# ashawkey/torch-ngp

Hardware: AMD Instinct MI355X
Metric: training samples/s (rays x steps), lego-shaped synthetic, fp16 autocast, full step incl. Adam (higher is better)
Workload: dtype f16

## Files before the change

### include/ngp_hip.h

```cpp
#ifndef NGP_HIP_H
#define NGP_HIP_H

#include <stddef.h>
#include <stdint.h>

#ifdef __cplusplus
extern "C" {
#endif

typedef void* ngp_stream_t;

enum {
    NGP_OK = 0,
    NGP_ERR_INVALID = 1,
    NGP_ERR_LAUNCH = 2,
    NGP_ERR_DEVICE = 3
};

enum { NGP_F32 = 0, NGP_F16 = 1, NGP_F64 = 2 };

#define NGP_MAX_LEVELS 32

const char* ngp_last_error(void);
int ngp_abi_version(void);
// ... 91 lines not shown
                                          const double* rgbs, const double* deltas, const int32_t* rays, const double* weights_sum,
                                          const double* image, uint32_t M, uint32_t N, float T_thresh, double* grad_sigmas,
                                          double* grad_rgbs, ngp_stream_t stream);
int ngp_composite_rays_f64(uint32_t n_alive, uint32_t n_step, float T_thresh, int32_t* rays_alive, double* rays_t,
                           const double* sigmas, const double* rgbs, const double* deltas, double* weights_sum, double* depth,
                           double* image, ngp_stream_t stream);

size_t ngp_compact_rays_workspace_bytes(uint32_t n_alive);
int ngp_compact_rays(const int32_t* rays_alive, uint32_t n_alive, int32_t* out_alive, int32_t* out_count,
                     void* workspace, ngp_stream_t stream);


int ngp_ffmlp_forward(const void* inputs, const void* weights, uint32_t B, uint32_t input_dim, uint32_t output_dim,
                      uint32_t hidden_dim, uint32_t num_layers, uint32_t activation, uint32_t output_activation,
                      void* forward_buffer, void* outputs, ngp_stream_t stream);
int ngp_ffmlp_inference(const void* inputs, const void* weights, uint32_t B, uint32_t input_dim,
                        uint32_t output_dim, uint32_t hidden_dim, uint32_t num_layers, uint32_t activation,
                        uint32_t output_activation, void* inference_buffer, void* outputs, ngp_stream_t stream);
int ngp_ffmlp_backward(const void* grad, const void* inputs, const void* weights, const void* forward_buffer,
                       uint32_t B, uint32_t input_dim, uint32_t output_dim, uint32_t hidden_dim, uint32_t num_layers,
                       uint32_t activation, uint32_t output_activation, int calc_grad_inputs, void* backward_buffer,
                       void* grad_inputs, void* grad_weights, ngp_stream_t stream);
int ngp_allocate_splitk(size_t size);
int ngp_free_splitk(void);

int ngp_grid_encode_forward_ex(const float* inputs, const void* embeddings, const int32_t* offsets, void* outputs,
                               uint32_t B, uint32_t D, uint32_t C, uint32_t L, float S, uint32_t H, void* dy_dx,
                               uint32_t gridtype, int align_corners, uint32_t interp, int dtype, float bound,
                               ngp_stream_t stream);
int ngp_grid_encode_backward_ex(const void* grad, const float* inputs, const void* embeddings, const int32_t* offsets,
                                void* grad_embeddings, uint32_t B, uint32_t D, uint32_t C, uint32_t L, float S,
                                uint32_t H, const void* dy_dx, void* grad_inputs, uint32_t gridtype, int align_corners,
                                uint32_t interp, int dtype, float bound, ngp_stream_t stream);
int ngp_grid_encode_forward_sched(const float* inputs, const void* embeddings, const int32_t* offsets, void* outputs,
                                  uint32_t B, uint32_t D, uint32_t C, uint32_t L, float S, uint32_t H, void* dy_dx,
                                  uint32_t gridtype, int align_corners, uint32_t interp, int dtype, float bound,
                                  const float* level_cost_host, ngp_stream_t stream);

int ngp_grid_encode_forward_sel(const float* inputs, const void* embeddings, const void* embeddings_alt, const float* parity,
                                const uint32_t* rows_dev, const int32_t* offsets, void* outputs, uint32_t B, uint32_t D, uint32_t C, uint32_t L,
                                float S, uint32_t H, uint32_t gridtype, int align_corners, uint32_t interp, int dtype, float bound,
                                const float* level_cost_host, ngp_stream_t stream);

uint32_t ngp_grid_forward_work_lists(uint32_t L, uint32_t tiles, const float* level_cost_host, uint16_t* level_out, uint32_t* tile0_out,
                                     uint32_t* end_out);

size_t ngp_grid_backward_workspace_bytes(const int32_t* offsets_host, uint32_t B, uint32_t D, uint32_t C, uint32_t L, float S, uint32_t H,
                                         uint32_t gridtype, int align_corners, int dtype);
int ngp_grid_encode_backward_checked(const void* grad, const float* inputs, const void* embeddings, const int32_t* offsets,
                                     void* grad_embeddings, uint32_t B, uint32_t D, uint32_t C, uint32_t L, float S, uint32_t H,
                                     const void* dy_dx, void* grad_inputs, uint32_t gridtype, int align_corners, uint32_t interp,
                                     int dtype, float bound, const int32_t* offsets_host, void* workspace, size_t workspace_bytes,
                                     float* found_inf, ngp_stream_t stream);

typedef struct ngp_table_adam {
    float* param[2]; float* exp_avg[2]; float* exp_avg_sq[2]; void* param_fp16[2];
    const float* state;
    float lr, beta1, beta2, eps;
} ngp_table_adam_t;
uint32_t ngp_grid_table_adam_prefix(const int32_t* offsets_host, uint32_t B, uint32_t D, uint32_t C, uint32_t L, float S, uint32_t H,
                                    uint32_t gridtype, int align_corners, int dtype);
typedef struct ngp_slab_sets {
    const void* slabs_a; uint32_t n_slabs_a, n_params_a; void* grad_weights_a;
    const void* slabs_b; uint32_t n_slabs_b, n_params_b; void* grad_weights_b;
    const float* ray_err; uint32_t n_rays; float* loss;
    uint32_t overwrite_table;
    const ngp_table_adam_t* table_adam;
} ngp_slab_sets_t;
int ngp_grid_encode_backward_checked_slabs(const void* grad, const float* inputs, const void* embeddings, const int32_t* offsets,
                                           void* grad_embeddings, uint32_t B, uint32_t D, uint32_t C, uint32_t L, float S, uint32_t H,
                                           const void* dy_dx, void* grad_inputs, uint32_t gridtype, int align_corners, uint32_t interp,
                                           int dtype, float bound, const int32_t* offsets_host, void* workspace, size_t workspace_bytes,
                                           float* found_inf, const ngp_slab_sets_t* slab_sets, ngp_stream_t stream);
int ngp_grid_encode_backward_ws(const void* grad, const float* inputs, const void* embeddings, const int32_t* offsets,
                                void* grad_embeddings, uint32_t B, uint32_t D, uint32_t C, uint32_t L, float S, uint32_t H,
                                const void* dy_dx, void* grad_inputs, uint32_t gridtype, int align_corners, uint32_t interp,
                                int dtype, float bound, const int32_t* offsets_host, void* workspace, size_t workspace_bytes,
                                ngp_stream_t stream);

size_t ngp_density_grid_update_workspace_bytes(uint32_t n_cells);
int ngp_density_grid_update(const float* sigmas, const int64_t* cells, uint32_t n, float density_scale, float decay, float* density_grid,
                            uint32_t n_cells, float* scratch, float density_thresh, float* mean_out, uint8_t* bitfield, void* workspace,
                            ngp_stream_t stream);

#define NGP_FF_INPUT_PLANAR 1u
#define NGP_FF_DX_PLANAR 2u
#define NGP_FF_LAYERED 4u
#define NGP_FF_SINGLE_WAVE 8u
#define NGP_FF_DEFER_REDUCE 16u
#define NGP_FF_RECOMPUTE 32u
#define NGP_FF_SERIAL_FLUSH 64u
int ngp_ffmlp_forward_ex(const void* inputs, const void* weights, uint32_t B, uint32_t input_dim, uint32_t output_dim,
                         uint32_t hidden_dim, uint32_t num_layers, uint32_t activation, uint32_t output_activation,
                         void* forward_buffer, void* outputs, uint32_t flags, ngp_stream_t stream);
int ngp_ffmlp_inference_ex(const void* inputs, const void* weights, uint32_t B, uint32_t input_dim,
                           uint32_t output_dim, uint32_t hidden_dim, uint32_t num_layers, uint32_t activation,
                           uint32_t output_activation, void* inference_buffer, void* outputs, uint32_t flags,
                           ngp_stream_t stream);
int ngp_ffmlp_backward_ex(const void* grad, const void* inputs, const void* weights, const void* forward_buffer,
                          uint32_t B, uint32_t input_dim, uint32_t output_dim, uint32_t hidden_dim, uint32_t num_layers,
                          uint32_t activation, uint32_t output_activation, int calc_grad_inputs, void* backward_buffer,
                          void* grad_inputs, void* grad_weights, uint32_t flags, ngp_stream_t stream);

size_t ngp_ffmlp_backward_workspace_bytes(uint32_t B, uint32_t input_dim, uint32_t hidden_dim, uint32_t num_layers);
int ngp_ffmlp_backward_ws(const void* grad, const void* inputs, const void* weights, const void* forward_buffer, uint32_t B,
                          uint32_t input_dim, uint32_t output_dim, uint32_t hidden_dim, uint32_t num_layers, uint32_t activation,
                          uint32_t output_activation, int calc_grad_inputs, void* backward_buffer, void* grad_inputs, void* grad_weights,
                          uint32_t flags, void* workspace, size_t workspace_bytes, ngp_stream_t stream);

size_t ngp_ffmlp_backward_backward_workspace_bytes(uint32_t B, uint32_t input_dim, uint32_t hidden_dim, uint32_t num_layers,
                                                   uint32_t activation);
int ngp_ffmlp_backward_backward(const void* grad, const void* inputs, const void* weights, const void* forward_buffer, const void* u,
                                uint32_t B, uint32_t input_dim, uint32_t output_dim, uint32_t hidden_dim, uint32_t num_layers,
                                uint32_t activation, void* grad_grad, void* grad_weights2, void* grad_inputs2, void* workspace,
                                size_t workspace_bytes, ngp_stream_t stream);

int ngp_network_forward(const void* enc, const float* dirs, uint32_t M, uint32_t M_valid, const void* w_sigma, const void* w_color,
                        uint32_t num_layers_sigma, uint32_t num_layers_color, float density_scale, int training,
                        void* forward_buffer_sigma, void* h16, float* sigma, void* color_in, void* forward_buffer_color, float* rgb,
                        uint32_t flags, ngp_stream_t stream);

int ngp_network_forward_rows(const void* enc, const float* dirs, uint32_t M, uint32_t M_valid, const void* w_sigma, const void* w_color,
                             uint32_t num_layers_sigma, uint32_t num_layers_color, float density_scale, int training,
                             void* forward_buffer_sigma, void* h16, float* sigma, void* color_in, void* forward_buffer_color, float* rgb,
                             uint32_t flags, const uint32_t* rows_dev, ngp_stream_t stream);

int ngp_network_backward_color(const void* grad_out16, const void* color_in, const void* w_color, const void* forward_buffer_color, uint32_t M,
                               uint32_t num_layers_color, void* backward_buffer, const float* grad_sigma, const void* h16,
                               float density_scale, void* grad_h16, void* grad_w_color, uint32_t flags, ngp_stream_t stream);
uint32_t ngp_ffmlp_backward_slab_count(uint32_t B, uint32_t input_dim, uint32_t hidden_dim, uint32_t num_layers);
int ngp_ffmlp_reduce_slabs_pair(const void* slabs_a, uint32_t n_slabs_a, uint32_t n_params_a, void* grad_weights_a, const void* slabs_b,
                                uint32_t n_slabs_b, uint32_t n_params_b, void* grad_weights_b, float* found_inf, ngp_stream_t stream);

int ngp_training_row_bound(const uint32_t* rows_dev);

int ngp_pipeline_mid_forward(const void* h16, const float* dirs, float* sigma, void* color_in, uint32_t M, uint32_t M_valid,
                             float density_scale, ngp_stream_t stream);
int ngp_pipeline_rgb_forward(const void* out16, float* rgb, uint32_t M, ngp_stream_t stream);
int ngp_pipeline_rgb_backward(const float* grad_rgb, const float* rgb, void* grad_out16, uint32_t M, ngp_stream_t stream);
int ngp_pipeline_mid_backward(const float* grad_sigma, const void* h16, const void* grad_color_in, void* grad_h16, uint32_t M,
                              float density_scale, ngp_stream_t stream);

int ngp_pipeline_mse_loss(const float* image, const float* target, uint32_t n, const float* loss_scale, float* loss,
                          float* grad_image, ngp_stream_t stream);

#define NGP_LINEAR_STACK_MAX 8
uint32_t ngp_linear_stack_flat_size(uint32_t depth, uint32_t n_in, uint32_t hidden, uint32_t n_out, int identity);
int ngp_linear_stack_pack(const float* const* weights, uint32_t depth, uint32_t n_in, uint32_t hidden, uint32_t n_out, int identity,
                          void* flat_fp16, ngp_stream_t stream);
int ngp_linear_stack_unpack_grad(const void* grad_flat_fp16, uint32_t depth, uint32_t n_in, uint32_t hidden, uint32_t n_out, int identity,
                                 float* const* grads, ngp_stream_t stream);

int ngp_pad_2d_fp16(const void* src, uint32_t src_rows, uint32_t src_cols, uint32_t src_row_stride, void* dst, uint32_t dst_rows,
                    uint32_t dst_cols, ngp_stream_t stream);

int ngp_rays_from_pixels(const float* poses, uint32_t B, float fx, float fy, float cx, float cy, uint32_t W, const int64_t* inds,
                         uint32_t inds_batch_stride, uint32_t N, float* rays_o, float* rays_d, ngp_stream_t stream);

#define NGP_MARCH_RESET_COUNTER 1u
#define NGP_MARCH_ZERO_TAIL 2u
#define NGP_MARCH_SCAN_LAUNCH 8u
#define NGP_MARCH_NOISE_FROM_SEED 4u
int ngp_march_rays_train_ex(const float* rays_o, const float* rays_d, const uint8_t* grid, float bound, float dt_gamma,
                            uint32_t max_steps, uint32_t N, uint32_t C, uint32_t H, uint32_t M, const float* nears,
                            const float* fars, float* xyzs, float* dirs, float* deltas, int32_t* rays, int32_t* counter,
                            const float* noises, void* workspace, uint32_t flags, ngp_stream_t stream);
int ngp_march_rays_train_aabb(const float* rays_o, const float* rays_d, const uint8_t* grid, float bound, float dt_gamma,
                              uint32_t max_steps, uint32_t N, uint32_t C, uint32_t H, uint32_t M, const float* aabb, float min_near,
                              float* nears, float* fars, float* xyzs, float* dirs, float* deltas, int32_t* rays, int32_t* counter,
                              const float* noises, void* workspace, uint32_t flags, ngp_stream_t stream);

int ngp_march_rays_ex(uint32_t n_alive, uint32_t n_step, const int32_t* rays_alive, const float* rays_t, const float* rays_o,
                      const float* rays_d, float bound, float dt_gamma, uint32_t max_steps, uint32_t C, uint32_t H,
                      const uint8_t* grid, const float* nears, const float* fars, float* xyzs, float* dirs, float* deltas,
                      const float* noises, uint32_t zero_rows, ngp_stream_t stream);

int ngp_march_rays_dev(const int32_t* state, uint32_t alive_bound, uint32_t n_total, uint32_t n_step_cap, const int32_t* rays_alive, const float* rays_t,
                       const float* rays_o, const float* rays_d, float bound, float dt_gamma, uint32_t max_steps, uint32_t C, uint32_t H,
                       const uint8_t* grid, const float* nears, const float* fars, float* xyzs, float* dirs, float* deltas,
                       const float* noises, uint32_t rows, ngp_stream_t stream);
int ngp_march_rays_dev_rows(const int32_t* state, uint32_t alive_bound, uint32_t n_total, uint32_t n_step_cap, const int32_t* rays_alive, const float* rays_t,
// ... 176 lines not shown
```

### torch-ngp_amd/_ngp_capi.py

```python
import ctypes
import os

import torch

_HERE = os.path.dirname(os.path.abspath(__file__))
LIB_PATH = os.environ.get('NGP_HIP_LIBRARY') or os.path.join(_HERE, 'libngp_hip.so')

NGP_F32, NGP_F16, NGP_F64 = 0, 1, 2
NGP_FF_INPUT_PLANAR, NGP_FF_DX_PLANAR, NGP_FF_LAYERED, NGP_FF_SINGLE_WAVE, NGP_FF_DEFER_REDUCE, NGP_FF_RECOMPUTE = 1, 2, 4, 8, 16, 32
NGP_FF_SERIAL_FLUSH = 64
NGP_MARCH_RESET_COUNTER, NGP_MARCH_ZERO_TAIL, NGP_MARCH_NOISE_FROM_SEED, NGP_MARCH_SCAN_LAUNCH = 1, 2, 4, 8
NGP_OPT_PHASE_CHECK, NGP_OPT_PHASE_UPDATE, NGP_OPT_PHASE_COMMIT, NGP_OPT_PHASE_FLIP = 1, 2, 4, 8
ABI_VERSION = 11

if not os.path.exists(LIB_PATH):
    raise ImportError(
        f"{LIB_PATH} is missing: build the HIP extension first (python __graft_entry__.py, or "
        f"make -C {os.path.join(_HERE, 'csrc')}).  There is no CPU fallback for these operators.")

lib = ctypes.CDLL(LIB_PATH)

_vp, _u32, _f32, _i32, _sz = ctypes.c_void_p, ctypes.c_uint32, ctypes.c_float, ctypes.c_int, ctypes.c_size_t

_SIGNATURES = {
    'ngp_grid_encode_forward': [_vp, _vp, _vp, _vp, _u32, _u32, _u32, _u32, _f32, _u32, _vp, _u32, _i32, _u32, _i32, _vp],
    'ngp_grid_encode_backward': [_vp, _vp, _vp, _vp, _vp, _u32, _u32, _u32, _u32, _f32, _u32, _vp, _vp, _u32, _i32, _u32, _i32, _vp],
    'ngp_grad_total_variation': [_vp, _vp, _vp, _vp, _f32, _u32, _u32, _u32, _u32, _f32, _u32, _u32, _i32, _i32, _vp],
    'ngp_grid_corner_indices': [_vp, _vp, _vp, _u32, _u32, _u32, _f32, _u32, _u32, _i32, _vp],
    'ngp_grid_level_table': [_u32, _f32, _u32, _vp, _vp],
    'ngp_grid_encode_backward_backward': [_vp, _vp, _vp, _vp, _vp, _vp, _vp, _vp, _u32, _u32, _u32, _u32, _f32, _u32, _u32, _i32, _u32, _i32, _vp,
                                          _sz, _vp],
    'ngp_grid_encode_backward_ordered': [_vp, _vp, _vp, _vp, _vp, _u32, _u32, _u32, _u32, _f32, _u32, _vp, _vp, _u32, _i32, _u32, _i32, _f32, _vp,
                                         _sz, _vp],
    'ngp_grid_encode_backward_backward_ordered': [_vp, _vp, _vp, _vp, _vp, _vp, _vp, _vp, _u32, _u32, _u32, _u32, _f32, _u32, _u32, _i32, _u32, _i32,
                                                  _vp, _sz, _vp],
    'ngp_grid_backward_is_reproducible': [_vp, _u32, _u32, _u32, _u32, _f32, _u32, _u32, _i32, _i32],
    'ngp_sh_encode_forward': [_vp, _vp, _u32, _u32, _u32, _vp, _i32, _vp],
    'ngp_sh_encode_backward': [_vp, _vp, _u32, _u32, _u32, _vp, _vp, _i32, _vp],
    'ngp_freq_encode_forward': [_vp, _u32, _u32, _u32, _u32, _vp, _vp],
    'ngp_freq_encode_backward': [_vp, _vp, _u32, _u32, _u32, _u32, _vp, _vp],
    'ngp_freq_encode_forward_f64': [_vp, _u32, _u32, _u32, _u32, _vp, _vp],
    'ngp_freq_encode_backward_f64': [_vp, _vp, _u32, _u32, _u32, _u32, _vp, _vp],
    'ngp_freq_encode_backward_backward': [_vp, _vp, _vp, _u32, _u32, _u32, _u32, _vp, _vp, _i32, _vp],
    'ngp_sh_encode_backward_backward': [_vp, _vp, _vp, _vp, _u32, _u32, _u32, _vp, _vp, _i32, _vp],
    'ngp_near_far_from_aabb': [_vp, _vp, _vp, _u32, _f32, _vp, _vp, _vp],
    'ngp_sph_from_ray': [_vp, _vp, _f32, _u32, _vp, _vp],
    'ngp_morton3D': [_vp, _u32, _vp, _vp],
    'ngp_morton3D_invert': [_vp, _u32, _vp, _vp],
    'ngp_packbits': [_vp, _u32, _f32, _vp, _vp],
    'ngp_packbits_ex': [_vp, _u32, _f32, _vp, _vp, _vp],
    'ngp_march_rays_train': [_vp, _vp, _vp, _f32, _f32, _u32, _u32, _u32, _u32, _u32, _vp, _vp, _vp, _vp, _vp, _vp, _vp, _vp, _vp, _vp],
    'ngp_composite_rays_train_forward': [_vp, _vp, _vp, _vp, _u32, _u32, _f32, _vp, _vp, _vp, _vp],
    'ngp_composite_rays_train_backward': [_vp, _vp, _vp, _vp, _vp, _vp, _vp, _vp, _u32, _u32, _f32, _vp, _vp, _vp],
    'ngp_march_rays': [_u32, _u32, _vp, _vp, _vp, _vp, _f32, _f32, _u32, _u32, _u32, _vp, _vp, _vp, _vp, _vp, _vp, _vp, _vp],
    'ngp_march_rays_ex': [_u32, _u32, _vp, _vp, _vp, _vp, _f32, _f32, _u32, _u32, _u32, _vp, _vp, _vp, _vp, _vp, _vp, _vp, _u32, _vp],
    'ngp_composite_rays': [_u32, _u32, _f32, _vp, _vp, _vp, _vp, _vp, _vp, _vp, _vp, _vp],
    'ngp_near_far_from_aabb_f64': [_vp, _vp, _vp, _u32, _f32, _vp, _vp, _vp],
    'ngp_sph_from_ray_f64': [_vp, _vp, _f32, _u32, _vp, _vp],
    'ngp_packbits_f64': [_vp, _u32, _f32, _vp, _vp],
    'ngp_composite_rays_train_forward_f64': [_vp, _vp, _vp, _vp, _u32, _u32, _f32, _vp, _vp, _vp, _vp],
    'ngp_composite_rays_train_backward_f64': [_vp, _vp, _vp, _vp, _vp, _vp, _vp, _vp, _u32, _u32, _f32, _vp, _vp, _vp],
    'ngp_composite_rays_f64': [_u32, _u32, _f32, _vp, _vp, _vp, _vp, _vp, _vp, _vp, _vp, _vp],
    'ngp_compact_rays': [_vp, _u32, _vp, _vp, _vp, _vp],
    'ngp_coarse_occupancy': [_vp, _u32, _u32, _vp, _vp],
    'ngp_cull_rays': [_vp, _vp, _vp, _vp, _u32, _f32, _u32, _u32, _vp, _vp, _vp],
    'ngp_march_rays_dev': [_vp, _u32, _u32, _u32, _vp, _vp, _vp, _vp, _f32, _f32, _u32, _u32, _u32, _vp, _vp, _vp, _vp, _vp, _vp, _vp, _u32, _vp],
    'ngp_composite_rays_dev': [_vp, _u32, _u32, _u32, _f32, _vp, _vp, _vp, _vp, _vp, _vp, _vp, _vp, _vp],
    'ngp_compact_rays_dev': [_vp, _u32, _u32, _u32, _u32, _vp, _vp, _vp, _vp, _vp],
    'ngp_render_iterations_dev': [_vp, _u32, _u32, _vp],
    'ngp_ffmlp_forward': [_vp, _vp, _u32, _u32, _u32, _u32, _u32, _u32, _u32, _vp, _vp, _vp],
    'ngp_ffmlp_inference': [_vp, _vp, _u32, _u32, _u32, _u32, _u32, _u32, _u32, _vp, _vp, _vp],
    'ngp_ffmlp_backward': [_vp, _vp, _vp, _vp, _u32, _u32, _u32, _u32, _u32, _u32, _u32, _i32, _vp, _vp, _vp, _vp],
    'ngp_grid_encode_forward_ex': [_vp, _vp, _vp, _vp, _u32, _u32, _u32, _u32, _f32, _u32, _vp, _u32, _i32, _u32, _i32, _f32, _vp],
    'ngp_grid_encode_forward_sched': [_vp, _vp, _vp, _vp, _u32, _u32, _u32, _u32, _f32, _u32, _vp, _u32, _i32, _u32, _i32, _f32, _vp, _vp],
    'ngp_grid_encode_forward_sel': [_vp, _vp, _vp, _vp, _vp, _vp, _vp, _u32, _u32, _u32, _u32, _f32, _u32, _u32, _i32, _u32, _i32, _f32, _vp, _vp],
    'ngp_grid_encode_backward_ex': [_vp, _vp, _vp, _vp, _vp, _u32, _u32, _u32, _u32, _f32, _u32, _vp, _vp, _u32, _i32, _u32, _i32, _f32, _vp],
    'ngp_grid_encode_backward_ws': [_vp, _vp, _vp, _vp, _vp, _u32, _u32, _u32, _u32, _f32, _u32, _vp, _vp, _u32, _i32, _u32, _i32, _f32, _vp, _vp,
                                    _sz, _vp],
    'ngp_grid_encode_backward_checked': [_vp, _vp, _vp, _vp, _vp, _u32, _u32, _u32, _u32, _f32, _u32, _vp, _vp, _u32, _i32, _u32, _i32, _f32, _vp,
                                         _vp, _sz, _vp, _vp],
    'ngp_grid_encode_backward_checked_slabs': [_vp, _vp, _vp, _vp, _vp, _u32, _u32, _u32, _u32, _f32, _u32, _vp, _vp, _u32, _i32, _u32, _i32, _f32,
                                               _vp, _vp, _sz, _vp, _vp, _vp],
    'ngp_density_grid_update': [_vp, _vp, _u32, _f32, _f32, _vp, _u32, _vp, _f32, _vp, _vp, _vp, _vp],
    'ngp_ffmlp_forward_ex': [_vp, _vp, _u32, _u32, _u32, _u32, _u32, _u32, _u32, _vp, _vp, _u32, _vp],
    'ngp_ffmlp_inference_ex': [_vp, _vp, _u32, _u32, _u32, _u32, _u32, _u32, _u32, _vp, _vp, _u32, _vp],
    'ngp_ffmlp_backward_ex': [_vp, _vp, _vp, _vp, _u32, _u32, _u32, _u32, _u32, _u32, _u32, _i32, _vp, _vp, _vp, _u32, _vp],
    'ngp_ffmlp_backward_ws': [_vp, _vp, _vp, _vp, _u32, _u32, _u32, _u32, _u32, _u32, _u32, _i32, _vp, _vp, _vp, _u32, _vp, _sz, _vp],
    'ngp_ffmlp_backward_backward': [_vp, _vp, _vp, _vp, _vp, _u32, _u32, _u32, _u32, _u32, _u32, _vp, _vp, _vp, _vp, _sz, _vp],
    'ngp_network_forward': [_vp, _vp, _u32, _u32, _vp, _vp, _u32, _u32, _f32, _i32, _vp, _vp, _vp, _vp, _vp, _vp, _u32, _vp],
    'ngp_network_forward_rows': [_vp, _vp, _u32, _u32, _vp, _vp, _u32, _u32, _f32, _i32, _vp, _vp, _vp, _vp, _vp, _vp, _u32, _vp, _vp],
    'ngp_march_rays_dev_rows': [_vp, _u32, _u32, _u32, _vp, _vp, _vp, _vp, _f32, _f32, _u32, _u32, _u32, _vp, _vp, _vp, _vp, _vp, _vp, _vp, _u32, _vp, _vp],
    'ngp_training_row_bound': [_vp],
    'ngp_pipeline_mid_forward': [_vp, _vp, _vp, _vp, _u32, _u32, _f32, _vp],
    'ngp_pipeline_rgb_forward': [_vp, _vp, _u32, _vp],
    'ngp_pipeline_rgb_backward': [_vp, _vp, _vp, _u32, _vp],
    'ngp_pipeline_mid_backward': [_vp, _vp, _vp, _vp, _u32, _f32, _vp],
    'ngp_pipeline_mse_loss': [_vp, _vp, _u32, _vp, _vp, _vp, _vp],
    'ngp_rays_from_pixels': [_vp, _u32, _f32, _f32, _f32, _f32, _u32, _vp, _u32, _u32, _vp, _vp, _vp],
    'ngp_march_rays_train_ex': [_vp, _vp, _vp, _f32, _f32, _u32, _u32, _u32, _u32, _u32, _vp, _vp, _vp, _vp, _vp, _vp, _vp, _vp, _vp, _u32, _vp],
    'ngp_march_rays_train_aabb': [_vp, _vp, _vp, _f32, _f32, _u32, _u32, _u32, _u32, _u32, _vp, _f32, _vp, _vp, _vp, _vp, _vp, _vp, _vp, _vp, _vp, _u32,
                                  _vp],
    'ngp_composite_rays_train_forward_ex': [_vp, _vp, _vp, _vp, _u32, _u32, _f32, _vp, _vp, _vp, _i32, _f32, _vp, _vp, _vp, _vp, _vp, _vp],
    'ngp_composite_rays_train_backward_ex': [_vp, _vp, _vp, _vp, _vp, _vp, _vp, _vp, _u32, _u32, _f32, _vp, _vp, _i32, _f32, _vp, _vp, _vp],
    'ngp_composite_rays_train_geo_forward': [_vp, _vp, _vp, _vp, _u32, _u32, _f32, _vp, _vp, _vp, _vp, _vp],
    'ngp_composite_rays_train_geo_backward': [_vp, _vp, _vp, _vp, _vp, _vp, _vp, _vp, _vp, _vp, _vp, _vp, _u32, _u32, _f32, _vp, _vp, _vp],
    'ngp_composite_rays_train_geo_forward_f64': [_vp, _vp, _vp, _vp, _u32, _u32, _f32, _vp, _vp, _vp, _vp, _vp],
    'ngp_composite_rays_train_geo_backward_f64': [_vp, _vp, _vp, _vp, _vp, _vp, _vp, _vp, _vp, _vp, _vp, _vp, _u32, _u32, _f32, _vp, _vp, _vp],
    'ngp_composite_rays_train_features_forward': [_vp, _vp, _vp, _vp, _u32, _u32, _u32, _f32, _i32, _vp, _vp],
    'ngp_composite_rays_train_features_backward': [_vp, _vp, _vp, _vp, _vp, _vp, _u32, _u32, _u32, _f32, _i32, _vp, _vp, _vp],
    'ngp_composite_rays_train_features_forward_f64': [_vp, _vp, _vp, _vp, _u32, _u32, _u32, _f32, _vp, _vp],
    'ngp_composite_rays_train_features_backward_f64': [_vp, _vp, _vp, _vp, _vp, _vp, _u32, _u32, _u32, _f32, _vp, _vp, _vp],
    'ngp_composite_rays_features': [_u32, _u32, _f32, _vp, _vp, _vp, _vp, _vp, _u32, _i32, _vp, _vp],
    'ngp_composite_rays_features_dev': [_vp, _u32, _u32, _u32, _f32, _vp, _vp, _vp, _vp, _vp, _u32, _i32, _vp, _vp],
    'ngp_composite_train_loss_backward': [_vp, _vp, _vp, _vp, _u32, _u32, _f32, _i32, _f32, _vp, _vp, _vp, _vp, _vp, _vp, _vp, _vp, _vp, _vp, _vp,
                                          _vp, _vp, _sz, _vp],
    'ngp_composite_train_geo_loss_backward': [_vp, _vp, _vp, _vp, _u32, _u32, _f32, _i32, _f32, _vp, _vp, _vp, _vp, _f32, _f32, _vp, _vp, _vp, _vp,
                                              _vp, _vp, _vp, _vp, _vp, _vp, _vp, _vp, _vp, _sz, _vp],
    'ngp_network_backward_color': [_vp, _vp, _vp, _vp, _u32, _u32, _vp, _vp, _vp, _f32, _vp, _vp, _u32, _vp],
    'ngp_ffmlp_reduce_slabs_pair': [_vp, _u32, _u32, _vp, _vp, _u32, _u32, _vp, _vp, _vp],
    'ngp_optim_adam_step': [_i32, _vp, _vp, _vp, _vp, _vp, _vp, _vp, _vp, _f32, _f32, _f32, _f32, _f32, _f32, _f32, _vp, _vp],
    'ngp_optim_adam_step_ex': [_i32, _vp, _vp, _vp, _vp, _vp, _vp, _vp, _vp, _f32, _f32, _f32, _f32, _f32, _f32, _f32, _vp, _vp, _f32, _u32, _vp],
    'ngp_optim_adam_small_commit': [_i32, _vp, _vp, _vp, _vp, _vp, _vp, _vp, _vp, _f32, _f32, _f32, _f32, _f32, _f32, _f32, _vp, _i32, _vp, _vp,
                                    ctypes.c_uint64, _vp],
    'ngp_optim_ema_update': [_i32, _vp, _vp, _vp, _f32, _vp],
    'ngp_optim_poison_shards': [_vp, _u32, ctypes.c_uint64, _vp, _vp],
    'ngp_optim_shard_verdict': [_vp, _vp, _vp, _u32, ctypes.c_uint64, _vp],
    'ngp_linear_stack_pack': [_vp, _u32, _u32, _u32, _u32, _i32, _vp, _vp],
    'ngp_linear_stack_unpack_grad': [_vp, _u32, _u32, _u32, _u32, _i32, _vp, _vp],
    'ngp_pad_2d_fp16': [_vp, _u32, _u32, _u32, _vp, _u32, _u32, _vp],
    'ngp_allocate_splitk': [_sz],
    'ngp_free_splitk': [],
    'ngp_cmdlist_create': [_vp],
    'ngp_cmdlist_begin': [_vp],
    'ngp_cmdlist_mark': [_vp, _u32, _i32],
    'ngp_cmdlist_end': [_vp],
    'ngp_cmdlist_count': [_vp, _vp],
    'ngp_cmdlist_entry_name': [_vp, _u32, _vp, _u32],
    'ngp_cmdlist_replay': [_vp, _vp],
    'ngp_cmdlist_wait_mark': [_vp, _u32, _vp],
    'ngp_cmdlist_destroy': [_vp],
    'ngp_ray_sample_ts': [_vp, _vp, _vp, _vp, _u32, _u32, _f32, _vp, _vp],
    'ngp_ray_sample_ts_f64': [_vp, _vp, _vp, _vp, _u32, _u32, _f32, _vp, _vp],
    'ngp_ray_points_forward': [_vp, _vp, _vp, _vp, _u32, _u32, _f32, _vp, _vp, _vp],
    'ngp_ray_points_forward_f64': [_vp, _vp, _vp, _vp, _u32, _u32, _f32, _vp, _vp, _vp],
    'ngp_ray_points_backward': [_vp, _vp, _vp, _vp, _vp, _vp, _vp, _u32, _u32, _f32, _vp, _vp, _vp],
    'ngp_ray_points_backward_f64': [_vp, _vp, _vp, _vp, _vp, _vp, _u32, _u32, _f32, _vp, _vp, _vp],
    'ngp_grid_input_gradient': [_vp, _vp, _vp, _vp, _u32, _u32, _u32, _u32, _f32, _u32, _u32, _i32, _u32, _i32, _f32, _vp, _vp],
    'ngp_rays_from_pixels_backward': [_vp, _vp, _u32, _f32, _f32, _f32, _f32, _u32, _vp, _u32, _u32, _vp, _vp],
    'ngp_error_map_draw': [_vp, _u32, _u32, _u32, _u32, _u32, _u32, _vp, _vp, _vp, _vp, _vp, _vp],
    'ngp_error_map_update': [_vp, _vp, _vp, _vp, _u32, _u32, _f32, _f32, _vp],
    'ngp_sdf_sigmas_forward': [_vp, _vp, _vp, _vp, _vp, _u32, _f32, _vp, _vp],
    'ngp_sdf_sigmas_backward': [_vp, _vp, _vp, _vp, _vp, _vp, _u32, _f32, _vp, _vp, _vp, _vp, _vp, _sz, _vp],
    'ngp_sdf_sigmas_forward_f64': [_vp, _vp, _vp, _vp, _vp, _u32, _f32, _vp, _vp],
    'ngp_sdf_sigmas_backward_f64': [_vp, _vp, _vp, _vp, _vp, _vp, _u32, _f32, _vp, _vp, _vp, _vp, _vp, _sz, _vp],
}
for _name, _args in _SIGNATURES.items():
    _fn = getattr(lib, _name)
    _fn.argtypes = _args
    _fn.restype = ctypes.c_int
lib.ngp_last_error.restype = ctypes.c_char_p
lib.ngp_target_arch.restype = ctypes.c_char_p
lib.ngp_abi_version.restype = ctypes.c_int
lib.ngp_ffmlp_backward_slab_count.argtypes = [_u32, _u32, _u32, _u32]
lib.ngp_ffmlp_backward_slab_count.restype = _u32
lib.ngp_march_rays_train_workspace_bytes.argtypes = [_u32]
lib.ngp_march_rays_train_workspace_bytes.restype = _sz
lib.ngp_compact_rays_workspace_bytes.argtypes = [_u32]
lib.ngp_ffmlp_backward_workspace_bytes.argtypes = [_u32, _u32, _u32, _u32]
lib.ngp_ffmlp_backward_workspace_bytes.restype = _sz
lib.ngp_ffmlp_backward_backward_workspace_bytes.argtypes = [_u32, _u32, _u32, _u32, _u32]
lib.ngp_ffmlp_backward_backward_workspace_bytes.restype = _sz
lib.ngp_grid_backward_workspace_bytes.argtypes = [_vp, _u32, _u32, _u32, _u32, _f32, _u32, _u32, _i32, _i32]
lib.ngp_grid_backward_workspace_bytes.restype = _sz
lib.ngp_grid_backward_backward_workspace_bytes.argtypes = [_vp, _u32, _u32, _u32, _u32, _i32]
lib.ngp_grid_backward_backward_workspace_bytes.restype = _sz
lib.ngp_compact_rays_workspace_bytes.restype = _sz
lib.ngp_grid_ordered_workspace_bytes.argtypes = [_u32, _u32, _u32, _i32]
lib.ngp_grid_ordered_workspace_bytes.restype = _sz
lib.ngp_grid_table_adam_prefix.argtypes = [_vp, _u32, _u32, _u32, _u32, _f32, _u32, _u32, _i32, _i32]
lib.ngp_grid_table_adam_prefix.restype = _u32
lib.ngp_coarse_occupancy_bytes.argtypes = [_u32, _u32]
lib.ngp_coarse_occupancy_bytes.restype = _sz
lib.ngp_grid_forward_work_lists.argtypes = [_u32, _u32, _vp, _vp, _vp, _vp]
lib.ngp_grid_forward_work_lists.restype = _u32
lib.ngp_density_grid_update_workspace_bytes.argtypes = [_u32]
lib.ngp_linear_stack_flat_size.argtypes = [_u32, _u32, _u32, _u32, _i32]
lib.ngp_linear_stack_flat_size.restype = _u32
lib.ngp_density_grid_update_workspace_bytes.restype = _sz
lib.ngp_sdf_sigmas_workspace_bytes.argtypes = [_u32]
lib.ngp_sdf_sigmas_workspace_bytes.restype = _sz

if lib.ngp_abi_version() != ABI_VERSION:
    raise ImportError(f"{LIB_PATH}: ABI version {lib.ngp_abi_version()} != expected {ABI_VERSION}; rebuild the extension")

EXPORTED = sorted(list(_SIGNATURES) + ['ngp_last_error', 'ngp_target_arch', 'ngp_abi_version',
                                       'ngp_march_rays_train_workspace_bytes', 'ngp_compact_rays_workspace_bytes',
                                       'ngp_grid_backward_workspace_bytes', 'ngp_ffmlp_backward_workspace_bytes',
                                       'ngp_ffmlp_backward_slab_count', 'ngp_density_grid_update_workspace_bytes', 'ngp_grid_forward_work_lists', 'ngp_coarse_occupancy_bytes',
                                       'ngp_grid_table_adam_prefix', 'ngp_linear_stack_flat_size',
                                       'ngp_grid_backward_backward_workspace_bytes', 'ngp_ffmlp_backward_backward_workspace_bytes',
                                       'ngp_grid_ordered_workspace_bytes', 'ngp_sdf_sigmas_workspace_bytes'])


def check(rc):
    if rc != 0:
        raise RuntimeError(lib.ngp_last_error().decode('utf-8', 'replace'))


class row_bound:

    def __init__(self, ws):
        self.ws = ws

    def __enter__(self):
        if self.ws is not None:
            check(lib.ngp_training_row_bound(self.ws.data_ptr()))
        return self

    def __exit__(self, *exc):
        if self.ws is not None:
            lib.ngp_training_row_bound(None)
        return False


class SlabSets(ctypes.Structure):
    _fields_ = [('slabs_a', ctypes.c_void_p), ('n_slabs_a', ctypes.c_uint32), ('n_params_a', ctypes.c_uint32), ('grad_weights_a', ctypes.c_void_p),
                ('slabs_b', ctypes.c_void_p), ('n_slabs_b', ctypes.c_uint32), ('n_params_b', ctypes.c_uint32), ('grad_weights_b', ctypes.c_void_p),
                ('ray_err', ctypes.c_void_p), ('n_rays', ctypes.c_uint32), ('loss', ctypes.c_void_p), ('overwrite_table', ctypes.c_uint32),
                ('table_adam', ctypes.c_void_p)]


class RenderLoop(ctypes.Structure):
    _fields_ = ([('state', ctypes.c_void_p), ('alive', ctypes.c_void_p * 2)] +
                [(n, ctypes.c_void_p) for n in ('rays_t', 'rays_o', 'rays_d', 'nears', 'fars', 'grid', 'noises', 'xyzs', 'dirs', 'deltas', 'enc', 'sigmas',
                                                'rgbs', 'embeddings', 'offsets', 'level_cost_host', 'w_sigma', 'w_color', 'weights_sum', 'depth', 'image',
                                                'compact_workspace', 'rows_used')] +
                [(n, ctypes.c_uint32) for n in ('lanes', 'rows', 'n_total', 'n_step_cap', 'max_steps', 'cascade', 'grid_size', 'L', 'H', 'gridtype',
                                                'interp', 'num_layers_sigma', 'num_layers_color')] +
                [('align_corners', ctypes.c_int32)] + [(n, ctypes.c_float) for n in ('bound', 'dt_gamma', 'T_thresh', 'S', 'density_scale')])


class TableAdam(ctypes.Structure):
    _fields_ = [('param', ctypes.c_void_p * 2), ('exp_avg', ctypes.c_void_p * 2), ('exp_avg_sq', ctypes.c_void_p * 2), ('param_fp16', ctypes.c_void_p * 2),
                ('state', ctypes.c_void_p), ('lr', ctypes.c_float), ('beta1', ctypes.c_float), ('beta2', ctypes.c_float), ('eps', ctypes.c_float)]


class CallerTensor:
    __slots__ = ('tensor',)

    def __init__(self, tensor):
        self.tensor = tensor


def ptr(t):
    return None if t is None else t.data_ptr()


def stream():
    return torch.cuda.current_stream().cuda_stream


def require_device(t, name):
    if not t.is_cuda:
        raise RuntimeError(f"{name} must be a CUDA tensor")


def require_contiguous(t, name):
    if not t.is_contiguous():
        raise RuntimeError(f"{name} must be a contiguous tensor")


def require_int32(t, name):
    if t.dtype != torch.int32:
        raise RuntimeError(f"{name} must be an int tensor")


def float_code(t, name):
    if t.dtype == torch.float16:
        return NGP_F16
    if t.dtype == torch.float32:
        return NGP_F32
    if t.dtype == torch.float64:
        return NGP_F64
    raise RuntimeError(f"{name} must be a floating tensor")
# ... 60 lines not shown
```

### torch-ngp_amd/csrc/ffmlp.hip

```cpp
#include "common.h"
#include "sh_poly.inc"

namespace ngp {

constexpr int FF_WAVES = 4;
constexpr int FF_THREADS = FF_WAVES * 64;
constexpr int FF_TILE = 32;

enum Act : uint32_t { ACT_RELU = 0, ACT_EXP = 1, ACT_SINE = 2, ACT_SIGMOID = 3, ACT_SQUAREPLUS = 4, ACT_SOFTPLUS = 5, ACT_NONE = 6 };
constexpr float K_ACT = 10.0f;

__device__ __forceinline__ float act_forward(uint32_t a, float x) {
    switch (a) {
        case ACT_RELU: return x > 0.0f ? x : 0.0f;
        case ACT_EXP: return __expf(x);
        case ACT_SINE: return __sinf(x);
        case ACT_SIGMOID: return 1.0f / (1.0f + __expf(-x));
        case ACT_SQUAREPLUS: { const float s = x * K_ACT; return 0.5f * (s + sqrtf(s * s + 4.0f)) / K_ACT; }
        case ACT_SOFTPLUS: return __logf(__expf(x * K_ACT) + 1.0f) / K_ACT;
        default: return x;
    }
}
__device__ __forceinline__ float act_backward_factor(uint32_t a, float y) {
    switch (a) {
// ... 123 lines not shown
template <int WIDTH>
__device__ void build_forward_image(half8_t* img, const half_t* __restrict__ w, uint32_t in_dim, uint32_t num_layers, uint32_t first_frag = 0,
                                    uint32_t n_frags = 0xFFFFFFFFu) {
    if (first_frag == 0u && n_frags == 0xFFFFFFFFu && (in_dim & 15u) == 0u) {
        build_forward_image_coalesced<WIDTH>(img, w, in_dim, num_layers);
        return;
    }
    const uint32_t all = fwd_frag_count<WIDTH>(in_dim, num_layers);
    const uint32_t total = (n_frags == 0xFFFFFFFFu ? all : n_frags) * 64;
    const uint32_t shift = first_frag * 64;
    for (uint32_t e0 = threadIdx.x; e0 < total; e0 += IMG_BATCH * blockDim.x) {
        half4_t lo[IMG_BATCH], hi[IMG_BATCH];
        bool real[IMG_BATCH];
#pragma unroll
        for (int b = 0; b < IMG_BATCH; b++) {
            const uint32_t e = e0 + b * blockDim.x;
            const half_t *pl = nullptr, *ph = nullptr;
            if (e < total) forward_fragment_source<WIDTH>(e + shift, w, in_dim, num_layers, pl, ph);
            real[b] = pl != nullptr;
            lo[b] = *reinterpret_cast<const half4_t*>(pl ? pl : w);
            hi[b] = *reinterpret_cast<const half4_t*>(ph ? ph : w);
        }
#pragma unroll
        for (int b = 0; b < IMG_BATCH; b++) {
            const uint32_t e = e0 + b * blockDim.x;
            if (e < total) {
                const half4_t z = {(half_t)0.0f, (half_t)0.0f, (half_t)0.0f, (half_t)0.0f};
                const half4_t l4 = real[b] ? lo[b] : z, h4 = real[b] ? hi[b] : z;
                img[e] = half8_t{l4.x, l4.y, l4.z, l4.w, h4.x, h4.y, h4.z, h4.w};
            }
        }
    }
}

template <int WIDTH>
__device__ __forceinline__ void pack_hidden(const float16_t (&acc)[Shape<WIDTH>::NIB], half8_t (&frag)[Shape<WIDTH>::NKB]) {
#pragma unroll
    for (int kb = 0; kb < Shape<WIDTH>::NKB; kb++) {
#pragma unroll
        for (int j = 0; j < 8; j++) frag[kb][j] = (half_t)acc[kb >> 1][(kb & 1) * 8 + j];
    }
}

__device__ __forceinline__ uint32_t relu_pack2(float a, float b) {
    typedef float f32x2 __attribute__((ext_vector_type(2)));
    typedef short i16x2 __attribute__((ext_vector_type(2)));
    const half2_t hv = __builtin_convertvector(f32x2{a, b}, half2_t);
    return __builtin_bit_cast(uint32_t, __builtin_elementwise_max(__builtin_bit_cast(i16x2, hv), i16x2{0, 0}));
}
template <int WIDTH>
__device__ __forceinline__ void pack_hidden_relu(const float16_t (&acc)[Shape<WIDTH>::NIB], half8_t (&frag)[Shape<WIDTH>::NKB]) {
    typedef uint32_t u32x4 __attribute__((ext_vector_type(4)));
#pragma unroll
    for (int kb = 0; kb < Shape<WIDTH>::NKB; kb++) {
        u32x4 w;
#pragma unroll
        for (int q = 0; q < 4; q++) w[q] = relu_pack2(acc[kb >> 1][(kb & 1) * 8 + 2 * q], acc[kb >> 1][(kb & 1) * 8 + 2 * q + 1]);
        frag[kb] = __builtin_bit_cast(half8_t, w);
    }
}


__device__ __forceinline__ half8_t load_features8(const half_t* __restrict__ inputs, bool planar, size_t rows, size_t s, uint32_t in_dim,
                                                  uint32_t f0) {
    if (!planar) return *reinterpret_cast<const half8_t*>(inputs + s * in_dim + f0);
    half8_t v;
#pragma unroll
    for (int q = 0; q < 4; q++) {
        const half2_t t = *reinterpret_cast<const half2_t*>(inputs + ((size_t)(f0 / 2 + q) * rows + s) * 2);
        v[2 * q] = t.x;
        v[2 * q + 1] = t.y;
    }
    return v;
}

template <typename V>
__device__ __forceinline__ void stream_store(V* dst, V v) {
    __builtin_nontemporal_store(v, dst);
}

template <int WIDTH, bool TRAIN, bool PLAIN >
__device__ __forceinline__ void ffmlp_forward_body(const half_t* __restrict__ inputs, const half_t* __restrict__ weights,
                                                   half_t* __restrict__ forward_buffer, half_t* __restrict__ outputs, uint32_t n_tiles,
                                                   uint32_t in_dim, uint32_t num_layers, uint32_t act, uint32_t out_act, bool in_planar) {
    constexpr int NIB = Shape<WIDTH>::NIB, NKB = Shape<WIDTH>::NKB;
    extern __shared__ __attribute__((aligned(16))) unsigned char smem[];
    half8_t* img = reinterpret_cast<half8_t*>(smem);
    build_forward_image<WIDTH>(img, weights, in_dim, num_layers);
    const size_t rows = (size_t)n_tiles * FF_TILE;
    __syncthreads();

    const int lane = threadIdx.x & 63, wid = threadIdx.x >> 6;
    const int n = lane & 31, h = lane >> 5;
    const uint32_t in_kb = in_dim / 16;
    const half8_t* img_l0 = img + lane;
    const half8_t* img_hid = img_l0 + (size_t)NIB * in_kb * 64;
    const half8_t* img_out = img_hid + (size_t)(num_layers - 1) * NIB * NKB * 64;
    const size_t layer_stride = (size_t)n_tiles * NKB * 64;

    for (uint32_t tile = blockIdx.x * FF_WAVES + wid; tile < n_tiles; tile += gridDim.x * FF_WAVES) {
        const size_t srow = (size_t)tile * FF_TILE + n;
        float16_t acc[NIB];
#pragma unroll
        for (int ib = 0; ib < NIB; ib++) acc[ib] = zero16();
        for (uint32_t kb = 0; kb < in_kb; kb++) {
            const half8_t x = load_features8(inputs, in_planar, rows, srow, in_dim, 16 * kb + 8 * h);
#pragma unroll
            for (int ib = 0; ib < NIB; ib++) acc[ib] = mfma(img_l0[(ib * in_kb + kb) * 64], x, acc[ib]);
        }
        half8_t hid[NKB];
        for (uint32_t l = 0;; l++) {
            if (PLAIN || act == ACT_RELU) {
                pack_hidden_relu<WIDTH>(acc, hid);
            } else {
                if (act != ACT_NONE) {
#pragma unroll
                    for (int ib = 0; ib < NIB; ib++)
#pragma unroll
                        for (int r = 0; r < 16; r++) acc[ib][r] = act_forward(act, acc[ib][r]);
                }
                pack_hidden<WIDTH>(acc, hid);
            }
            if (TRAIN) {
                half8_t* dst = reinterpret_cast<half8_t*>(forward_buffer) + l * layer_stride + (size_t)tile * NKB * 64 + lane;
#pragma unroll
                for (int kb = 0; kb < NKB; kb++) stream_store(dst + kb * 64, hid[kb]);
            }
            if (l + 1 == num_layers) break;
            const half8_t* wl = img_hid + (size_t)l * NIB * NKB * 64;
#pragma unroll
            for (int ib = 0; ib < NIB; ib++) {
                acc[ib] = zero16();
#pragma unroll
                for (int kb = 0; kb < NKB; kb++) acc[ib] = mfma(wl[(ib * NKB + kb) * 64], hid[kb], acc[ib]);
            }
        }
        float16_t o = zero16();
#pragma unroll
        for (int kb = 0; kb < NKB; kb++) o = mfma(img_out[kb * 64], hid[kb], o);
        half4_t lo, hi;
#pragma unroll
        for (int c = 0; c < 4; c++) {
            lo[c] = (half_t)(PLAIN ? o[c] : act_forward(out_act, o[c]));
            hi[c] = (half_t)(PLAIN ? o[4 + c] : act_forward(out_act, o[4 + c]));
        }
        half_t* orow = outputs + ((size_t)tile * FF_TILE + n) * 16 + 4 * h;
        *reinterpret_cast<half4_t*>(orow) = lo;
        *reinterpret_cast<half4_t*>(orow + 8) = hi;
    }
}

template <int WIDTH, bool TRAIN, bool PLAIN>
__global__ __launch_bounds__(FF_THREADS) __attribute__((amdgpu_waves_per_eu(4, 4))) void k_ffmlp_forward(
    const half_t* __restrict__ inputs, const half_t* __restrict__ weights, half_t* __restrict__ forward_buffer, half_t* __restrict__ outputs,
    uint32_t n_tiles, uint32_t in_dim, uint32_t num_layers, uint32_t act, uint32_t out_act, bool in_planar) {
    ffmlp_forward_body<WIDTH, TRAIN, PLAIN>(inputs, weights, forward_buffer, outputs, n_tiles, in_dim, num_layers, act, out_act, in_planar);
}
template <int WIDTH, bool TRAIN, bool PLAIN>
__global__ __launch_bounds__(FF_THREADS) __attribute__((amdgpu_waves_per_eu(2, 2))) void k_ffmlp_forward_wide(
    const half_t* __restrict__ inputs, const half_t* __restrict__ weights, half_t* __restrict__ forward_buffer, half_t* __restrict__ outputs,
    uint32_t n_tiles, uint32_t in_dim, uint32_t num_layers, uint32_t act, uint32_t out_act, bool in_planar) {
    ffmlp_forward_body<WIDTH, TRAIN, PLAIN>(inputs, weights, forward_buffer, outputs, n_tiles, in_dim, num_layers, act, out_act, in_planar);
}


template <bool TRAIN, int NT>
__device__ __forceinline__ void relu_network_tail(float16_t (&acc)[NT][2], float16_t (&o)[NT], const half8_t* __restrict__ hid_img,
                                                  const half8_t* __restrict__ out_img, uint32_t nl, half_t* __restrict__ fb, size_t layer_stride,
                                                  const uint32_t (&tile)[NT], const bool (&live)[NT], int lane) {
    constexpr int WIDTH = 64, NIB = 2, NKB = 4;
    half8_t hid[NT][NKB];
    for (uint32_t l = 0;; l++) {
#pragma unroll
        for (int t = 0; t < NT; t++) {
            pack_hidden_relu<WIDTH>(acc[t], hid[t]);
            if (TRAIN && fb && live[t]) {
                half8_t* dst = reinterpret_cast<half8_t*>(fb) + l * layer_stride + (size_t)tile[t] * NKB * 64 + lane;
#pragma unroll
                for (int kb = 0; kb < NKB; kb++) stream_store(dst + kb * 64, hid[t][kb]);
            }
        }
        if (l + 1 == nl) break;
        const half8_t* wl = hid_img + (size_t)l * NIB * NKB * 64;
#pragma unroll
        for (int ib = 0; ib < NIB; ib++) {
#pragma unroll
            for (int t = 0; t < NT; t++) acc[t][ib] = zero16();
#pragma unroll
            for (int kb = 0; kb < NKB; kb++) {
                const half8_t a = wl[(ib * NKB + kb) * 64];
#pragma unroll
                for (int t = 0; t < NT; t++) acc[t][ib] = mfma(a, hid[t][kb], acc[t][ib]);
            }
        }
    }
#pragma unroll
    for (int t = 0; t < NT; t++) o[t] = zero16();
#pragma unroll
    for (int kb = 0; kb < NKB; kb++) {
        const half8_t a = out_img[kb * 64];
#pragma unroll
        for (int t = 0; t < NT; t++) o[t] = mfma(a, hid[t][kb], o[t]);
    }
}

template <bool TRAIN, int WAVES , int NT >
__global__ __launch_bounds__(WAVES * 64) __attribute__((amdgpu_waves_per_eu(NT == 1 ? 4 : 2, NT == 1 ? 4 : 3))) void k_network_forward(
    const half_t* __restrict__ enc, bool enc_planar, const float* __restrict__ dirs, uint32_t M_valid, const half_t* __restrict__ w_sigma,
    const half_t* __restrict__ w_color, half_t* __restrict__ fb_s, half_t* __restrict__ h16, float* __restrict__ sigma,
    half_t* __restrict__ color_in, half_t* __restrict__ fb_c, float* __restrict__ rgb, uint32_t n_tiles_cap, uint32_t nl_s, uint32_t nl_c,
    float density_scale, const uint32_t* __restrict__ rows_dev, bool rows_live) {
    constexpr int WIDTH = 64, NIB = 2, NKB = 4;
    constexpr uint32_t in_kb = 2;
    const uint32_t n_tiles = !rows_dev ? n_tiles_cap
                             : rows_live ? live_rows(n_tiles_cap * (uint32_t)FF_TILE, rows_dev[0]) / (uint32_t)FF_TILE
                                         : min(n_tiles_cap, (rows_dev[0] + (uint32_t)FF_TILE - 1u) / (uint32_t)FF_TILE);
    extern __shared__ __attribute__((aligned(16))) unsigned char smem[];
    half8_t* img_s = reinterpret_cast<half8_t*>(smem);
    const uint32_t frags_s = NIB * in_kb + (nl_s - 1) * NIB * NKB + NKB;
    half8_t* img_c = img_s + (size_t)frags_s * 64;
    const size_t rows = (size_t)n_tiles_cap * FF_TILE;
    const int lane = threadIdx.x & 63, wid = threadIdx.x >> 6;
    const int n = lane & 31, h = lane >> 5;
    const uint32_t n_groups = (n_tiles + NT - 1) / NT;
    half8_t x_next[NT][in_kb];
    float dir_next[NT][3];
#pragma unroll
    for (int t = 0; t < NT; t++) dir_next[t][0] = dir_next[t][1] = dir_next[t][2] = 0.0f;
    auto request = [&](uint32_t group) {
        if (group < n_groups) {
#pragma unroll
            for (int t = 0; t < NT; t++) {
                const uint32_t tl = group * NT + t < n_tiles ? group * NT + t : n_tiles - 1;
                const size_t srow = (size_t)tl * FF_TILE + n;
#pragma unroll
                for (uint32_t kb = 0; kb < in_kb; kb++) x_next[t][kb] = load_features8(enc, enc_planar, rows, srow, 32, 16 * kb + 8 * h);
                dir_next[t][0] = dir_next[t][1] = dir_next[t][2] = 0.0f;
                if (srow < M_valid) { dir_next[t][0] = dirs[srow * 3]; dir_next[t][1] = dirs[srow * 3 + 1]; dir_next[t][2] = dirs[srow * 3 + 2]; }
            }
        }
    };
    request(blockIdx.x * WAVES + wid);
    build_forward_image<WIDTH>(img_s, w_sigma, 32, nl_s);
    build_forward_image<WIDTH>(img_c, w_color, 32, nl_c);
    __syncthreads();
// ... 1214 lines not shown
        }
    }
}

__global__ __launch_bounds__(RS_PARAMS * RS_GROUPS) void k_ffmlp_reduce_slabs_pair(SlabSets sets, float* __restrict__ found_inf) {
    __shared__ float part[RS_GROUPS][RS_PARAMS];
    slab_reduce_block(sets, blockIdx.x, part, found_inf);
}

struct DeviceInfo {
    int cus = 0;
    bool ok = false;
};
static DeviceInfo device_info() {
    static thread_local DeviceInfo info;
    if (!info.ok) {
        int dev = 0;
        if (hipGetDevice(&dev) == hipSuccess) {
            hipDeviceProp_t p;
            if (hipGetDeviceProperties(&p, dev) == hipSuccess) {
                info.cus = p.multiProcessorCount;
                info.ok = true;
            }
        }
        if (!info.ok) info.cus = 256;
    }
    return info;
}

static int check_ff_args(const char* fn, uint32_t B, uint32_t in_dim, uint32_t out_dim, uint32_t hidden, uint32_t num_layers) {
    NGP_REQUIRE(hidden == 16 || hidden == 32 || hidden == 64 || hidden == 128 || hidden == 256, NGP_ERR_INVALID,
                "%s: hidden_dim should in [16, 32, 64, 128, 256], but got %u", fn, hidden);
    NGP_REQUIRE(in_dim > 0 && in_dim % 16 == 0, NGP_ERR_INVALID, "%s: input_dim should be 16 * m (m > 0), but got %u", fn, in_dim);
    NGP_REQUIRE(out_dim == 16, NGP_ERR_INVALID, "%s: output_dim must be padded to 16 by the caller (got %u)", fn, out_dim);
    NGP_REQUIRE(num_layers >= 2, NGP_ERR_INVALID, "%s: num_layers should be larger than 2 (3 matmuls), but got %u", fn, num_layers);
    NGP_REQUIRE(B % 128 == 0, NGP_ERR_INVALID, "%s: batch size must be 128 * m, but got %u", fn, B);
    return NGP_OK;
}

static int raise_lds(const void* kern, size_t lds, const char* what) {
    if (lds > 64 * 1024) {
        hipError_t e = hipFuncSetAttribute(kern, hipFuncAttributeMaxDynamicSharedMemorySize, (int)lds);
        NGP_REQUIRE(e == hipSuccess, NGP_ERR_LAUNCH, "%s: cannot raise the dynamic LDS limit: %s", what, hipGetErrorString(e));
    }
    return NGP_OK;
}

static int reduce_slabs(const void* slabs, uint32_t n_slabs, uint32_t n_params, void* grad_weights, hipStream_t st, const char* what) {
    SlabSets sets = {};
    const uint32_t blocks = slab_set(sets, 0, slabs, n_slabs, n_params, grad_weights, false);
    NGP_LAUNCH(k_ffmlp_reduce_slabs_pair, dim3(blocks), dim3(RS_PARAMS * RS_GROUPS), 0, st, sets, (float*)nullptr);
    return check_launch(what);
}

template <int WIDTH>
static size_t forward_image_bytes(uint32_t in_dim, uint32_t num_layers) {
    return (size_t)fwd_frag_count<WIDTH>(in_dim, num_layers) * 1024;
}

template <int WIDTH, bool TRAIN>
static int launch_forward_layered(const void* inputs, const void* weights, uint32_t B, uint32_t in_dim, uint32_t num_layers, uint32_t act,
                                  uint32_t out_act, void* buffer, void* outputs, uint32_t flags, hipStream_t st) {
    constexpr int NIB = Shape<WIDTH>::NIB, NKB = Shape<WIDTH>::NKB;
    const uint32_t n_tiles = B / FF_TILE;
    uint32_t frags = NIB * (in_dim / 16);
    if (frags < (uint32_t)(NIB * NKB)) frags = NIB * NKB;
    const size_t lds = (size_t)frags * 1024;
    NGP_REQUIRE(lds <= 152 * 1024, NGP_ERR_INVALID, "ffmlp: one %u x %u layer (%zu B) exceeds the LDS of a CU", (unsigned)WIDTH, in_dim, lds);
    NGP_REQUIRE(buffer, NGP_ERR_INVALID, "ffmlp: this network shape needs the %s the reference passes", TRAIN ? "forward_buffer" : "inference_buffer [B, hidden]");
    auto kern = k_ffmlp_forward_layered<WIDTH, TRAIN>;
    int rc = raise_lds(reinterpret_cast<const void*>(kern), lds, "ffmlp");
    if (rc) return rc;
    const uint32_t per_cu = (uint32_t)((160 * 1024) / (lds + 1024));
    uint32_t blocks = (uint32_t)device_info().cus * (per_cu < 1 ? 1 : (per_cu > 2 ? 2 : per_cu));
    const uint32_t need = cdiv(n_tiles, FF_WAVES);
    if (blocks > need) blocks = need;
    NGP_LAUNCH(kern, dim3(blocks), dim3(FF_THREADS), lds, st, (const half_t*)inputs, (const half_t*)weights, (half_t*)buffer,
                       (half_t*)outputs, n_tiles, in_dim, num_layers, act, out_act, (flags & NGP_FF_INPUT_PLANAR) != 0);
    return check_launch(TRAIN ? "ffmlp_forward(layered)" : "ffmlp_inference(layered)");
}

template <int WIDTH, bool TRAIN>
static int launch_forward(const void* inputs, const void* weights, uint32_t B, uint32_t in_dim, uint32_t num_layers, uint32_t act,
                          uint32_t out_act, void* fwd, void* outputs, uint32_t flags, hipStream_t st) {
    const uint32_t n_tiles = B / FF_TILE;
    const size_t lds = forward_image_bytes<WIDTH>(in_dim, num_layers);
    if (WIDTH > 128 || lds > 152 * 1024 || (flags & NGP_FF_LAYERED))
        return launch_forward_layered<WIDTH, TRAIN>(inputs, weights, B, in_dim, num_layers, act, out_act, fwd, outputs, flags, st);
    if constexpr (WIDTH > 128) {
        return NGP_ERR_INVALID;
    } else {
    const bool plain = act == ACT_RELU && out_act == ACT_NONE;
    using forward_kernel_t = void (*)(const half_t*, const half_t*, half_t*, half_t*, uint32_t, uint32_t, uint32_t, uint32_t, uint32_t, bool);
    forward_kernel_t kern;
    if constexpr (WIDTH > 64) kern = plain ? k_ffmlp_forward_wide<WIDTH, TRAIN, true> : k_ffmlp_forward_wide<WIDTH, TRAIN, false>;
    else kern = plain ? k_ffmlp_forward<WIDTH, TRAIN, true> : k_ffmlp_forward<WIDTH, TRAIN, false>;
    int rc = raise_lds(reinterpret_cast<const void*>(kern), lds, "ffmlp");
    if (rc) return rc;
    const uint32_t per_cu = (uint32_t)((160 * 1024) / (lds + 1024));
    uint32_t blocks = (uint32_t)device_info().cus * (per_cu < 1 ? 1 : (per_cu > 4 ? 4 : per_cu));
    const uint32_t need = cdiv(n_tiles, FF_WAVES);
    if (blocks > need) blocks = need;
    const hipError_t e = NGP_LAUNCH_STATUS(kern, dim3(blocks), dim3(FF_THREADS), lds, st, (const half_t*)inputs, (const half_t*)weights, (half_t*)fwd,
                                           (half_t*)outputs, n_tiles, in_dim, num_layers, act, out_act, (flags & NGP_FF_INPUT_PLANAR) != 0);
    NGP_REQUIRE(e == hipSuccess, NGP_ERR_LAUNCH, "ffmlp: kernel launch failed: %s", hipGetErrorString(e));
    return check_launch(TRAIN ? "ffmlp_forward" : "ffmlp_inference");
    }
}

constexpr uint32_t WG_MAX_CHUNKS = 64;

template <int WIDTH>
static int launch_backward_layered(const void* grad, const void* inputs, const void* weights, const void* fwd, uint32_t B, uint32_t in_dim,
                                   uint32_t num_layers, uint32_t act, bool with_dx, void* backward_buffer, void* grad_inputs,
                                   void* grad_weights, uint32_t flags, void* workspace, size_t workspace_bytes, hipStream_t st) {
    constexpr int NIB = Shape<WIDTH>::NIB, NKB = Shape<WIDTH>::NKB;
    const bool in_planar = (flags & NGP_FF_INPUT_PLANAR) != 0, dx_planar = (flags & NGP_FF_DX_PLANAR) != 0;
    const uint32_t n_tiles = B / FF_TILE;
    const uint32_t in_jb = (in_dim + 31) / 32;
    uint32_t frags = NIB * NKB;
    if (with_dx && frags < in_jb * NKB) frags = in_jb * NKB;
    const size_t lds = (size_t)frags * 1024;
    NGP_REQUIRE(lds <= 152 * 1024, NGP_ERR_INVALID, "ffmlp_backward: one %u x %u layer (%zu B) exceeds the LDS of a CU", (unsigned)WIDTH, in_dim, lds);
    const void* dk = act == ACT_RELU ? reinterpret_cast<const void*>(k_ffmlp_dgrad_layered<WIDTH, true>)
                                     : reinterpret_cast<const void*>(k_ffmlp_dgrad_layered<WIDTH, false>);
    int rc = raise_lds(dk, lds, "ffmlp_backward");
    if (rc) return rc;
    const uint32_t per_cu = (uint32_t)((160 * 1024) / (lds + 1024));
    uint32_t blocks = (uint32_t)device_info().cus * (per_cu < 1 ? 1 : (per_cu > 2 ? 2 : per_cu));
    const uint32_t need = cdiv(n_tiles, FF_WAVES);
    if (blocks > need) blocks = need;
    if (act == ACT_RELU)
        NGP_LAUNCH((k_ffmlp_dgrad_layered<WIDTH, true>), dim3(blocks), dim3(FF_THREADS), lds, st, (const half_t*)grad, (const half_t*)weights,
                           (const half_t*)fwd, (half_t*)backward_buffer, n_tiles, in_dim, num_layers, act, with_dx, (half_t*)grad_inputs, dx_planar);
    else
        NGP_LAUNCH((k_ffmlp_dgrad_layered<WIDTH, false>), dim3(blocks), dim3(FF_THREADS), lds, st, (const half_t*)grad, (const half_t*)weights,
                           (const half_t*)fwd, (half_t*)backward_buffer, n_tiles, in_dim, num_layers, act, with_dx, (half_t*)grad_inputs, dx_planar);
    rc = check_launch("ffmlp_backward(dgrad)");
    if (rc) return rc;
    const uint32_t n_params = ff_param_count(in_dim, WIDTH, num_layers);
    const uint32_t jobs = wgrad_jobs_of(NIB, in_jb) + (num_layers - 1) * wgrad_jobs_of(NIB, NIB) + wgrad_jobs_of(1, NIB);
    uint32_t chunks = 1;
    if (workspace) {
        chunks = (uint32_t)(workspace_bytes / ((size_t)n_params * 4));
        const uint32_t want = cdiv((uint32_t)device_info().cus * 4u, jobs);
        if (chunks > want) chunks = want;
        if (chunks > WG_MAX_CHUNKS) chunks = WG_MAX_CHUNKS;
        const uint32_t by_tiles = cdiv(n_tiles, 2 * FF_WAVES);
        if (chunks > by_tiles) chunks = by_tiles;
        if (chunks < 1) chunks = 1;
    }
    const uint32_t tiles_per_chunk = cdiv(n_tiles, chunks);
    chunks = cdiv(n_tiles, tiles_per_chunk);
    const bool direct = chunks == 1;
    NGP_LAUNCH(k_ffmlp_wgrad<WIDTH>, dim3(chunks, jobs), dim3(FF_THREADS), 0, st, (const half_t*)grad, (const half_t*)inputs, (const half_t*)fwd,
                       (const half_t*)backward_buffer, n_tiles, in_dim, num_layers, in_planar, tiles_per_chunk, direct ? (float*)nullptr : (float*)workspace,
                       direct ? (half_t*)grad_weights : (half_t*)nullptr);
    rc = check_launch("ffmlp_backward(wgrad)");
    if (rc || direct) return rc;
    return reduce_slabs(workspace, chunks, n_params, grad_weights, st, "ffmlp_backward(reduce)");
}

static bool ff_register_resident(uint32_t in_dim, uint32_t hidden, uint32_t num_layers) {
    return (hidden == 32 || hidden == 64) && num_layers <= 4 && in_dim <= 64;
}
static bool ff_leaves_slabs(uint32_t in_dim, uint32_t hidden, uint32_t num_layers) {
    return ff_register_resident(in_dim, hidden, num_layers) && num_layers >= 2 && num_layers <= 3;
}

template <int WIDTH>
static uint32_t backward_slab_count(uint32_t B, uint32_t in_dim, uint32_t num_layers) {
    const uint32_t n_params = SlabLayout{WIDTH, in_dim, num_layers}.n_params();
    const size_t buf_bytes = (size_t)num_layers * B * WIDTH * sizeof(half_t);
    uint32_t blocks = (uint32_t)device_info().cus;
    const uint32_t need = cdiv(B / FF_TILE, FF_WAVES);
    if (blocks > need) blocks = need;
    const size_t fit = buf_bytes / ((size_t)n_params * 4);
    if (blocks > fit) blocks = (uint32_t)fit;
    return blocks;
}

struct BackwardLds {
    size_t image, tile;
    uint32_t pf_depth;
    size_t stage, total;
};
template <int WIDTH, int IN_JB, int NHM>
// ... 43 lines not shown
    const bool defer = (flags & NGP_FF_DEFER_REDUCE) != 0, serial = (flags & NGP_FF_SERIAL_FLUSH) != 0;
    const MidEpilogue mid = mid_in ? *mid_in : MidEpilogue{nullptr, nullptr, nullptr, 0.0f};
    const uint32_t n_tiles = B / FF_TILE;
    const uint32_t n_params = SlabLayout{WIDTH, in_dim, num_layers}.n_params();
    const BackwardLds lds = backward_lds_plan<WIDTH, IN_JB, NHM>(in_dim, num_layers, with_dx, flags, false);
    NGP_REQUIRE(lds.total <= 160 * 1024, NGP_ERR_INVALID, "ffmlp_backward: LDS need (%zu B) exceeds 160 KiB", lds.total);
    const uint32_t blocks = backward_slab_count<WIDTH>(B, in_dim, num_layers);
    const half_t *g = (const half_t*)grad, *x = (const half_t*)inputs, *w = (const half_t*)weights;
    if (flags & NGP_FF_RECOMPUTE) {
        if constexpr (WIDTH == 64 && IN_JB == 1 && RELU && (NHM == 1 || NHM == 2)) {
            NGP_REQUIRE(in_dim == 32 && !(flags & NGP_FF_SINGLE_WAVE), NGP_ERR_INVALID, "ffmlp_backward: NGP_FF_RECOMPUTE needs input_dim 32 and the paired kernel");
            const BackwardLds lds_r = backward_lds_plan<WIDTH, IN_JB, NHM>(in_dim, num_layers, with_dx, flags, true);
            NGP_REQUIRE(lds_r.total <= 160 * 1024, NGP_ERR_INVALID, "ffmlp_backward: LDS need (%zu B) exceeds 160 KiB", lds_r.total);
            auto pk = k_ffmlp_backward_paired<WIDTH, IN_JB, NHM, RELU, true>;
            return launch_and_reduce(reinterpret_cast<const void*>(pk), lds_r.total, blocks, defer, backward_buffer, grad_weights, n_params, st,
                                     [&](dim3 grid, float* slabs, half_t* direct) {
                NGP_LAUNCH(pk, grid, dim3(FP_THREADS), lds_r.total, st, g, x, w, (const half_t*)nullptr, n_tiles, in_dim, num_layers, act, with_dx,
                                   (half_t*)grad_inputs, slabs, direct, in_planar, dx_planar, lds_r.pf_depth, mid, (uint32_t)lds_r.total, serial, rows_dev);
            });
        } else {
            NGP_REQUIRE(false, NGP_ERR_INVALID, "ffmlp_backward: NGP_FF_RECOMPUTE serves 64-wide ReLU networks with 32 inputs and 2 or 3 layers");
        }
    }
    if constexpr (NHM == 1 || NHM == 2) {
        if (!(flags & NGP_FF_SINGLE_WAVE)) {
            auto pk = k_ffmlp_backward_paired<WIDTH, IN_JB, NHM, RELU>;
            return launch_and_reduce(reinterpret_cast<const void*>(pk), lds.total, blocks, defer, backward_buffer, grad_weights, n_params, st,
                                     [&](dim3 grid, float* slabs, half_t* direct) {
                NGP_LAUNCH(pk, grid, dim3(FP_THREADS), lds.total, st, g, x, w, (const half_t*)fwd, n_tiles, in_dim, num_layers, act, with_dx,
                                   (half_t*)grad_inputs, slabs, direct, in_planar, dx_planar, lds.pf_depth, mid, (uint32_t)lds.total, serial, rows_dev);
            });
        }
    }
    NGP_REQUIRE(!mid.grad_sigma && !defer && !rows_dev, NGP_ERR_INVALID, "ffmlp_backward: this extension needs the paired kernel (2 or 3 layers)");
    auto kern = k_ffmlp_backward<WIDTH, IN_JB, NHM, RELU>;
    return launch_and_reduce(reinterpret_cast<const void*>(kern), lds.total, blocks, false, backward_buffer, grad_weights, n_params, st,
                             [&](dim3 grid, float* slabs, half_t* direct) {
        NGP_LAUNCH(kern, grid, dim3(FF_THREADS), lds.total, st, g, x, w, (const half_t*)fwd, n_tiles, in_dim, num_layers, act, with_dx,
                           (half_t*)grad_inputs, slabs, direct, in_planar, dx_planar, lds.pf_depth, (uint32_t)lds.total, serial);
    });
}

template <int WIDTH, int IN_JB, int NHM>
static int launch_backward(const void* grad, const void* inputs, const void* weights, const void* fwd, uint32_t B, uint32_t in_dim,
                           uint32_t num_layers, uint32_t act, bool with_dx, void* backward_buffer, void* grad_inputs,
                           void* grad_weights, uint32_t flags, hipStream_t st, const MidEpilogue* mid = nullptr,
                           const uint32_t* rows_dev = nullptr ) {
    if (act == ACT_RELU)
        return launch_backward_t<WIDTH, IN_JB, NHM, true>(grad, inputs, weights, fwd, B, in_dim, num_layers, act, with_dx, backward_buffer,
                                                          grad_inputs, grad_weights, flags, st, mid, rows_dev);
    return launch_backward_t<WIDTH, IN_JB, NHM, false>(grad, inputs, weights, fwd, B, in_dim, num_layers, act, with_dx, backward_buffer,
                                                       grad_inputs, grad_weights, flags, st, mid, rows_dev);
}

}

using namespace ngp;

#define FF_WIDTHS(CALL)                  \
    switch (hidden_dim) {                \
        case 16: return CALL(16);        \
        case 32: return CALL(32);        \
        case 64: return CALL(64);        \
        case 128: return CALL(128);      \
        default: return CALL(256);       \
    }

extern "C" int ngp_ffmlp_forward_ex(const void* inputs, const void* weights, uint32_t B, uint32_t input_dim, uint32_t output_dim,
                                    uint32_t hidden_dim, uint32_t num_layers, uint32_t activation, uint32_t output_activation,
                                    void* forward_buffer, void* outputs, uint32_t flags, ngp_stream_t stream) {
    int rc = check_ff_args("ffmlp_forward", B, input_dim, output_dim, hidden_dim, num_layers);
    if (rc) return rc;
    if (B == 0) return NGP_OK;
    NGP_REQUIRE(inputs && weights && forward_buffer && outputs, NGP_ERR_INVALID, "ffmlp_forward: NULL tensor");
    hipStream_t st = as_stream(stream);
#define FF_FWD(W) launch_forward<W, true>(inputs, weights, B, input_dim, num_layers, activation, output_activation, forward_buffer, outputs, flags, st)
    FF_WIDTHS(FF_FWD)
#undef FF_FWD
}

extern "C" int ngp_ffmlp_inference_ex(const void* inputs, const void* weights, uint32_t B, uint32_t input_dim, uint32_t output_dim,
                                      uint32_t hidden_dim, uint32_t num_layers, uint32_t activation, uint32_t output_activation,
                                      void* inference_buffer, void* outputs, uint32_t flags, ngp_stream_t stream) {
    int rc = check_ff_args("ffmlp_inference", B, input_dim, output_dim, hidden_dim, num_layers);
    if (rc) return rc;
    if (B == 0) return NGP_OK;
    NGP_REQUIRE(inputs && weights && outputs, NGP_ERR_INVALID, "ffmlp_inference: NULL tensor");
    hipStream_t st = as_stream(stream);
#define FF_INF(W) launch_forward<W, false>(inputs, weights, B, input_dim, num_layers, activation, output_activation, inference_buffer, outputs, flags, st)
    FF_WIDTHS(FF_INF)
#undef FF_INF
}

extern "C" size_t ngp_ffmlp_backward_workspace_bytes(uint32_t B, uint32_t input_dim, uint32_t hidden_dim, uint32_t num_layers) {
    if (ff_register_resident(input_dim, hidden_dim, num_layers) || B == 0) return 0;
    return (size_t)WG_MAX_CHUNKS * SlabLayout{hidden_dim, input_dim, num_layers}.n_params() * sizeof(float);
}

static int ffmlp_backward_impl(const void* grad, const void* inputs, const void* weights, const void* forward_buffer, uint32_t B,
                               uint32_t input_dim, uint32_t output_dim, uint32_t hidden_dim, uint32_t num_layers, uint32_t activation,
                               int calc_grad_inputs, void* backward_buffer, void* grad_inputs, void* grad_weights, uint32_t flags, void* workspace,
                               size_t workspace_bytes, const uint32_t* rows_dev, ngp_stream_t stream) {
    int rc = check_ff_args("ffmlp_backward", B, input_dim, output_dim, hidden_dim, num_layers);
    if (rc) return rc;
    NGP_REQUIRE(!rows_dev || (ff_register_resident(input_dim, hidden_dim, num_layers) && num_layers <= 3 &&
                              !(flags & (NGP_FF_LAYERED | NGP_FF_SINGLE_WAVE))),
                NGP_ERR_INVALID, "ffmlp_backward: the row bound needs the paired kernel (a register-resident network of 2 or 3 layers, neither "
                                 "NGP_FF_LAYERED nor NGP_FF_SINGLE_WAVE)");
    if (B == 0) {
        if (grad_weights && !(flags & NGP_FF_DEFER_REDUCE)) {
            const size_t n_w = (size_t)hidden_dim * ((size_t)input_dim + (size_t)hidden_dim * (num_layers - 1) + (size_t)output_dim);
            hipError_t e = ::ngp::memset_async(grad_weights, 0, n_w * sizeof(half_t), as_stream(stream));
            NGP_REQUIRE(e == hipSuccess, NGP_ERR_LAUNCH, "ffmlp_backward: hipMemsetAsync failed: %s", hipGetErrorString(e));
        }
        return NGP_OK;
    }
    NGP_REQUIRE(grad && inputs && weights && (forward_buffer || (flags & NGP_FF_RECOMPUTE)) && backward_buffer && grad_weights, NGP_ERR_INVALID,
                "ffmlp_backward: NULL tensor");
    NGP_REQUIRE(!calc_grad_inputs || grad_inputs, NGP_ERR_INVALID, "ffmlp_backward: grad_inputs is NULL but calc_grad_inputs is set");
    hipStream_t st = as_stream(stream);
    const bool dx = calc_grad_inputs != 0;
    const bool fast = ff_register_resident(input_dim, hidden_dim, num_layers) && !(flags & NGP_FF_LAYERED);
    NGP_REQUIRE(fast || !(flags & NGP_FF_RECOMPUTE), NGP_ERR_INVALID, "ffmlp_backward: NGP_FF_RECOMPUTE serves 64-wide ReLU networks with 32 inputs and 2 or 3 layers");
    NGP_REQUIRE(fast || !(flags & NGP_FF_DEFER_REDUCE), NGP_ERR_INVALID, "ffmlp_backward: NGP_FF_DEFER_REDUCE needs a 2- or 3-layer network of width 32 / 64");
    if (!fast) {
#define FF_LAY(W) launch_backward_layered<W>(grad, inputs, weights, forward_buffer, B, input_dim, num_layers, activation, dx, backward_buffer, grad_inputs, grad_weights, flags, workspace, workspace_bytes, st)
        FF_WIDTHS(FF_LAY)
#undef FF_LAY
    }
    const uint32_t in_jb = (input_dim + 31) / 32;
#define FF_BWD(W, J, N) \
    return launch_backward<W, J, N>(grad, inputs, weights, forward_buffer, B, input_dim, num_layers, activation, dx, backward_buffer, grad_inputs, grad_weights, flags, st, nullptr, rows_dev)
#define FF_BWD_N(W, J)                      \
    switch (num_layers - 1) {               \
        case 1: FF_BWD(W, J, 1);            \
        case 2: FF_BWD(W, J, 2);            \
        default: FF_BWD(W, J, 3);           \
    }
    if (hidden_dim == 64) {
        if (in_jb == 1) { FF_BWD_N(64, 1) }
        FF_BWD_N(64, 2)
    }
    if (in_jb == 1) { FF_BWD_N(32, 1) }
    FF_BWD_N(32, 2)
#undef FF_BWD_N
#undef FF_BWD
}

extern "C" int ngp_ffmlp_backward_ws(const void* grad, const void* inputs, const void* weights, const void* forward_buffer, uint32_t B,
                                     uint32_t input_dim, uint32_t output_dim, uint32_t hidden_dim, uint32_t num_layers, uint32_t activation,
                                     uint32_t output_activation, int calc_grad_inputs, void* backward_buffer, void* grad_inputs,
                                     void* grad_weights, uint32_t flags, void* workspace, size_t workspace_bytes, ngp_stream_t stream) {
    (void)output_activation;
    return ffmlp_backward_impl(grad, inputs, weights, forward_buffer, B, input_dim, output_dim, hidden_dim, num_layers, activation, calc_grad_inputs,
                               backward_buffer, grad_inputs, grad_weights, flags, workspace, workspace_bytes, nullptr, stream);
}

extern "C" int ngp_ffmlp_backward_ex(const void* grad, const void* inputs, const void* weights, const void* forward_buffer, uint32_t B,
                                     uint32_t input_dim, uint32_t output_dim, uint32_t hidden_dim, uint32_t num_layers, uint32_t activation,
                                     uint32_t output_activation, int calc_grad_inputs, void* backward_buffer, void* grad_inputs,
                                     void* grad_weights, uint32_t flags, ngp_stream_t stream) {
    (void)output_activation;
    return ffmlp_backward_impl(grad, inputs, weights, forward_buffer, B, input_dim, output_dim, hidden_dim, num_layers, activation, calc_grad_inputs,
                               backward_buffer, grad_inputs, grad_weights, flags, nullptr, 0, armed_row_bound(), stream);
}


extern "C" uint32_t ngp_ffmlp_backward_slab_count(uint32_t B, uint32_t input_dim, uint32_t hidden_dim, uint32_t num_layers) {
    if (!ff_leaves_slabs(input_dim, hidden_dim, num_layers) || B == 0) return 0;
    const uint32_t blocks = hidden_dim == 64 ? backward_slab_count<64>(B, input_dim, num_layers) : backward_slab_count<32>(B, input_dim, num_layers);
    return blocks <= 1 ? 0u : blocks;
}
// ... 144 lines not shown
```

### torch-ngp_amd/csrc/raymarching.hip

```cpp
#include "common.h"
#include <math.h>
#include <float.h>

namespace ngp {

constexpr int RM_THREADS = 256;

__device__ __forceinline__ void near_far_from_aabb(float ox, float oy, float oz, float dx, float dy, float dz, const float* __restrict__ aabb,
                                                   float min_near, float& near_out, float& far_out) {
    const float rdx = 1.0f / dx, rdy = 1.0f / dy, rdz = 1.0f / dz;
    float near = (aabb[0] - ox) * rdx, far = (aabb[3] - ox) * rdx, t;
    near_out = far_out = FLT_MAX;
    if (near > far) { t = near; near = far; far = t; }
    float ny = (aabb[1] - oy) * rdy, fy = (aabb[4] - oy) * rdy;
    if (ny > fy) { t = ny; ny = fy; fy = t; }
    if (near > fy || ny > far) return;
    if (ny > near) near = ny;
    if (fy < far) far = fy;
    float nz = (aabb[2] - oz) * rdz, fz = (aabb[5] - oz) * rdz;
    if (nz > fz) { t = nz; nz = fz; fz = t; }
    if (near > fz || nz > far) return;
    if (nz > near) near = nz;
    if (fz < far) far = fz;
    if (near < min_near) near = min_near;
// ... 8 lines not shown
    if (n >= N) return;
    float near, far;
    near_far_from_aabb(rays_o[n * 3], rays_o[n * 3 + 1], rays_o[n * 3 + 2], rays_d[n * 3], rays_d[n * 3 + 1], rays_d[n * 3 + 2], aabb, min_near,
                       near, far);
    nears[n] = near;
    fars[n] = far;
}

__global__ void k_sph_from_ray(const float* __restrict__ rays_o, const float* __restrict__ rays_d, float radius, uint32_t N,
                               float* __restrict__ coords) {
    const uint32_t n = blockIdx.x * blockDim.x + threadIdx.x;
    if (n >= N) return;
    const float ox = rays_o[n * 3], oy = rays_o[n * 3 + 1], oz = rays_o[n * 3 + 2];
    const float dx = rays_d[n * 3], dy = rays_d[n * 3 + 1], dz = rays_d[n * 3 + 2];
    const float A = dx * dx + dy * dy + dz * dz;
    const float Bh = ox * dx + oy * dy + oz * dz;
    const float Cc = ox * ox + oy * oy + oz * oz - radius * radius;
    const float t = (-Bh + sqrtf(Bh * Bh - A * Cc)) / A;
    const float x = ox + t * dx, y = oy + t * dy, z = oz + t * dz;
    const float theta = atan2f(sqrtf(x * x + z * z), y);
    const float phi = atan2f(z, x);
    const float RPI = 0.3183098861837907f;
    coords[n * 2] = 2.0f * theta * RPI - 1.0f;
    coords[n * 2 + 1] = phi * RPI;
}

__device__ __forceinline__ uint32_t expand_bits(uint32_t v) {
    v = (v * 0x00010001u) & 0xFF0000FFu;
    v = (v * 0x00000101u) & 0x0F00F00Fu;
    v = (v * 0x00000011u) & 0xC30C30C3u;
    v = (v * 0x00000005u) & 0x49249249u;
    return v;
}
__device__ __forceinline__ uint32_t morton3D_1(uint32_t x, uint32_t y, uint32_t z) {
    return expand_bits(x) | (expand_bits(y) << 1) | (expand_bits(z) << 2);
}
__device__ __forceinline__ uint32_t compact_bits(uint32_t x) {
    x &= 0x49249249u;
    x = (x | (x >> 2)) & 0xc30c30c3u;
    x = (x | (x >> 4)) & 0x0f00f00fu;
    x = (x | (x >> 8)) & 0xff0000ffu;
    x = (x | (x >> 16)) & 0x0000ffffu;
    return x;
}
__global__ void k_morton3D(const int32_t* __restrict__ coords, uint32_t N, int32_t* __restrict__ indices) {
    const uint32_t n = blockIdx.x * blockDim.x + threadIdx.x;
    if (n >= N) return;
    indices[n] = (int32_t)morton3D_1((uint32_t)coords[n * 3], (uint32_t)coords[n * 3 + 1], (uint32_t)coords[n * 3 + 2]);
}
__global__ void k_morton3D_invert(const int32_t* __restrict__ indices, uint32_t N, int32_t* __restrict__ coords) {
    const uint32_t n = blockIdx.x * blockDim.x + threadIdx.x;
    if (n >= N) return;
    const int32_t ind = indices[n];
    coords[n * 3 + 0] = (int32_t)compact_bits((uint32_t)(ind >> 0));
    coords[n * 3 + 1] = (int32_t)compact_bits((uint32_t)(ind >> 1));
    coords[n * 3 + 2] = (int32_t)compact_bits((uint32_t)(ind >> 2));
}

__global__ void k_packbits(const float* __restrict__ grid, uint32_t N, float thresh, const float* __restrict__ thresh_cap,
                           uint8_t* __restrict__ bitfield) {
    const uint32_t n = blockIdx.x * blockDim.x + threadIdx.x;
    if (n >= N) return;
    if (thresh_cap) thresh = fminf(thresh, thresh_cap[0]);
    const float4_t a = *reinterpret_cast<const float4_t*>(grid + (size_t)n * 8);
    const float4_t b = *reinterpret_cast<const float4_t*>(grid + (size_t)n * 8 + 4);
    uint32_t bits = 0;
    bits |= (a.x > thresh) ? 1u : 0u;
    bits |= (a.y > thresh) ? 2u : 0u;
    bits |= (a.z > thresh) ? 4u : 0u;
    bits |= (a.w > thresh) ? 8u : 0u;
    bits |= (b.x > thresh) ? 16u : 0u;
    bits |= (b.y > thresh) ? 32u : 0u;
    bits |= (b.z > thresh) ? 64u : 0u;
    bits |= (b.w > thresh) ? 128u : 0u;
    bitfield[n] = (uint8_t)bits;
}

__global__ __launch_bounds__(RM_THREADS) void k_density_scatter(const float* __restrict__ sigmas, const int64_t* __restrict__ cells, uint32_t n,
                                                                  float scale, float* __restrict__ scratch, uint32_t n_cells) {
    const uint32_t i = blockIdx.x * RM_THREADS + threadIdx.x;
    if (i >= n) return;
    const uint64_t c = (uint64_t)cells[i];
    if (c < n_cells) scratch[c] = sigmas[i] * scale;
}

constexpr int DM_THREADS = 256, DM_PER_THREAD = 32;
__global__ __launch_bounds__(DM_THREADS) void k_density_apply_mean(float* __restrict__ grid, float* __restrict__ scratch, uint32_t n_cells, float decay,
                                                                     double* __restrict__ partials, uint32_t* __restrict__ ticket,
                                                                     float* __restrict__ mean_out) {
    const uint32_t base = blockIdx.x * (DM_THREADS * DM_PER_THREAD);
    double acc = 0.0;
    auto one = [&](float g, float f, bool& touched) {
        touched = !(f == -1.0f);
        if (f >= 0.0f && g >= 0.0f) g = fmaxf(g * decay, f);
        acc += (double)fmaxf(g, 0.0f);
        return g;
    };
#pragma unroll 2
    for (int k = 0; k < DM_PER_THREAD / 4; k++) {
        const uint32_t i = base + (uint32_t)(k * DM_THREADS + threadIdx.x) * 4u;
        if (i < n_cells) {
            float4_t g = *reinterpret_cast<const float4_t*>(grid + i);
            const float4_t f = *reinterpret_cast<const float4_t*>(scratch + i);
            bool t0, t1, t2, t3;
            g.x = one(g.x, f.x, t0); g.y = one(g.y, f.y, t1); g.z = one(g.z, f.z, t2); g.w = one(g.w, f.w, t3);
            if (t0 || t1 || t2 || t3) {
                *reinterpret_cast<float4_t*>(grid + i) = g;
                *reinterpret_cast<float4_t*>(scratch + i) = float4_t{-1.0f, -1.0f, -1.0f, -1.0f};
            }
        }
    }
    __shared__ double part[DM_THREADS / 64];
    __shared__ bool last;
#pragma unroll
    for (int o = 32; o > 0; o >>= 1) acc += __shfl_xor(acc, o, 64);
    if ((threadIdx.x & 63) == 0) part[threadIdx.x >> 6] = acc;
    __syncthreads();
    if (threadIdx.x == 0) {
        double b = 0.0;
#pragma unroll
        for (int w = 0; w < DM_THREADS / 64; w++) b += part[w];
        __hip_atomic_store(&partials[blockIdx.x], b, __ATOMIC_RELAXED, __HIP_MEMORY_SCOPE_AGENT);
        asm volatile("s_waitcnt vmcnt(0)" ::: "memory");
        last = __hip_atomic_fetch_add(ticket, 1u, __ATOMIC_RELAXED, __HIP_MEMORY_SCOPE_AGENT) == gridDim.x - 1u;
    }
    __syncthreads();
    if (!last) return;
    double t = 0.0;
    for (uint32_t b = threadIdx.x; b < gridDim.x; b += DM_THREADS) t += __hip_atomic_load(&partials[b], __ATOMIC_RELAXED, __HIP_MEMORY_SCOPE_AGENT);
#pragma unroll
    for (int o = 32; o > 0; o >>= 1) t += __shfl_xor(t, o, 64);
    __syncthreads();
    if ((threadIdx.x & 63) == 0) part[threadIdx.x >> 6] = t;
    __syncthreads();
    if (threadIdx.x == 0) {
        double sum = 0.0;
#pragma unroll
        for (int w = 0; w < DM_THREADS / 64; w++) sum += part[w];
        mean_out[0] = (float)(sum / (double)n_cells);
        __hip_atomic_store(ticket, 0u, __ATOMIC_RELAXED, __HIP_MEMORY_SCOPE_AGENT);
    }
}

struct Ray {
    float ox, oy, oz, dx, dy, dz, rdx, rdy, rdz;
};
struct MarchParams {
    float bound, rbound, dt_gamma, dt_min, dt_max, Hf, rH, H3f, Hm1, Cm1;
    uint32_t H3;
    const uint8_t* grid;
};

__device__ __forceinline__ MarchParams make_params(float bound, float dt_gamma, uint32_t max_steps, uint32_t C, uint32_t H,
                                                   const uint8_t* grid) {
    MarchParams p;
    const float SQRT3 = 1.7320508075688772f;
    p.bound = bound;
    p.dt_gamma = dt_gamma;
    p.Hf = (float)H;
    p.rH = 1.0f / p.Hf;
    p.H3f = (float)(H * H * H);
    p.H3 = H * H * H;
    p.rbound = 1.0f / bound;
    p.Hm1 = (float)(H - 1);
    p.Cm1 = (float)C - 1.0f;
    p.dt_min = 2.0f * SQRT3 / (float)max_steps;
// ... 1317 lines not shown
                }
            }
        } else {
            const uint32_t npass = (nl + spp - 1u) >> (6u - lp);
            for (uint32_t p0 = 0; p0 < npass; p0 += CF_UNROLL) {
                float f[CF_UNROLL];
#pragma unroll
                for (int u = 0; u < CF_UNROLL; u++) {
                    const uint32_t i = (p0 + u) * spp + j;
                    f[u] = (c < C && i < nl) ? (float)row[i * C + c] : 0.0f;
                }
#pragma unroll
                for (int u = 0; u < CF_UNROLL; u++) {
                    const uint32_t p = p0 + u, i = p * spp + j;
                    const float wi = __shfl(w, (int)(i & 63u), 64);
                    if (c < C && i < nl) store_feat(grow + i * C + c, wi * g[0]);
                    const float qs = seg_sum(g[0] * f[u], lp, lane);
                    const float got = __shfl(qs, (int)(((uint32_t)lane & (spp - 1u)) << lp), 64);
                    q = ((uint32_t)lane >> (6u - lp)) == p ? got : q;
                }
            }
        }
        const float sa = carry + wave_incl_sum(w * q, lane);
        if (live) grad_sigmas[offset + s] = d0 * (T_after * q - (Q - sa));
        T = T * lane63(pin);
        carry = lane63(sa);
        if (T < T_thresh) break;
    }
}

}

using namespace ngp;

#define RM_LAUNCH_1D(kernel, count, st, ...) NGP_LAUNCH(kernel, dim3(cdiv((count), RM_THREADS)), dim3(RM_THREADS), 0, st, __VA_ARGS__)

extern "C" int ngp_near_far_from_aabb(const float* rays_o, const float* rays_d, const float* aabb, uint32_t N, float min_near,
                                      float* nears, float* fars, ngp_stream_t stream) {
    if (N == 0) return NGP_OK;
    NGP_REQUIRE(rays_o && rays_d && aabb && nears && fars, NGP_ERR_INVALID, "near_far_from_aabb: NULL tensor");
    RM_LAUNCH_1D(k_near_far_from_aabb, N, as_stream(stream), rays_o, rays_d, aabb, N, min_near, nears, fars);
    return check_launch("near_far_from_aabb");
}

extern "C" int ngp_sph_from_ray(const float* rays_o, const float* rays_d, float radius, uint32_t N, float* coords,
                                ngp_stream_t stream) {
    if (N == 0) return NGP_OK;
    NGP_REQUIRE(rays_o && rays_d && coords, NGP_ERR_INVALID, "sph_from_ray: NULL tensor");
    RM_LAUNCH_1D(k_sph_from_ray, N, as_stream(stream), rays_o, rays_d, radius, N, coords);
    return check_launch("sph_from_ray");
}

extern "C" int ngp_morton3D(const int32_t* coords, uint32_t N, int32_t* indices, ngp_stream_t stream) {
    if (N == 0) return NGP_OK;
    NGP_REQUIRE(coords && indices, NGP_ERR_INVALID, "morton3D: NULL tensor");
    RM_LAUNCH_1D(k_morton3D, N, as_stream(stream), coords, N, indices);
    return check_launch("morton3D");
}

extern "C" int ngp_morton3D_invert(const int32_t* indices, uint32_t N, int32_t* coords, ngp_stream_t stream) {
    if (N == 0) return NGP_OK;
    NGP_REQUIRE(coords && indices, NGP_ERR_INVALID, "morton3D_invert: NULL tensor");
    RM_LAUNCH_1D(k_morton3D_invert, N, as_stream(stream), indices, N, coords);
    return check_launch("morton3D_invert");
}

extern "C" int ngp_packbits_ex(const float* grid, uint32_t N, float density_thresh, const float* thresh_cap, uint8_t* bitfield,
                               ngp_stream_t stream) {
    if (N == 0) return NGP_OK;
    NGP_REQUIRE(grid && bitfield, NGP_ERR_INVALID, "packbits: NULL tensor");
    NGP_REQUIRE((reinterpret_cast<uintptr_t>(grid) & 15) == 0, NGP_ERR_INVALID, "packbits: grid must be 16-byte aligned");
    RM_LAUNCH_1D(k_packbits, N, as_stream(stream), grid, N, density_thresh, thresh_cap, bitfield);
    return check_launch("packbits");
}

extern "C" int ngp_packbits(const float* grid, uint32_t N, float density_thresh, uint8_t* bitfield, ngp_stream_t stream) {
    return ngp_packbits_ex(grid, N, density_thresh, nullptr, bitfield, stream);
}

extern "C" size_t ngp_density_grid_update_workspace_bytes(uint32_t n_cells) {
    return sizeof(double) * (size_t)cdiv(n_cells, DM_THREADS * DM_PER_THREAD) + 64;
}

extern "C" int ngp_density_grid_update(const float* sigmas, const int64_t* cells, uint32_t n, float density_scale, float decay, float* density_grid,
                                       uint32_t n_cells, float* scratch, float density_thresh, float* mean_out, uint8_t* bitfield, void* workspace,
                                       ngp_stream_t stream) {
    NGP_REQUIRE(density_grid && scratch && mean_out && bitfield && workspace, NGP_ERR_INVALID, "density_grid_update: NULL tensor");
    NGP_REQUIRE(n_cells >= 8 && n_cells % 8 == 0, NGP_ERR_INVALID, "density_grid_update: the grid must hold a multiple of 8 cells (got %u)", n_cells);
    NGP_REQUIRE(((reinterpret_cast<uintptr_t>(density_grid) | reinterpret_cast<uintptr_t>(scratch)) & 15) == 0, NGP_ERR_INVALID,
                "density_grid_update: grid and scratch must be 16-byte aligned");
    hipStream_t st = as_stream(stream);
    if (n) {
        NGP_REQUIRE(sigmas && cells, NGP_ERR_INVALID, "density_grid_update: NULL tensor");
        RM_LAUNCH_1D(k_density_scatter, n, st, sigmas, cells, n, density_scale, scratch, n_cells);
    }
    const uint32_t blocks = cdiv(n_cells, DM_THREADS * DM_PER_THREAD);
    double* partials = reinterpret_cast<double*>(workspace);
    uint32_t* ticket = reinterpret_cast<uint32_t*>(partials + blocks);
    NGP_LAUNCH(k_density_apply_mean, dim3(blocks), dim3(DM_THREADS), 0, st, density_grid, scratch, n_cells, decay, partials, ticket, mean_out);
    RM_LAUNCH_1D(k_packbits, n_cells / 8, st, (const float*)density_grid, n_cells / 8, density_thresh, (const float*)mean_out, bitfield);
    return check_launch("density_grid_update");
}

extern "C" size_t ngp_march_rays_train_workspace_bytes(uint32_t N) {
    return sizeof(uint32_t) * (march_ws_ticket_word(N) + (size_t)CT_GROUPS * CT_GROUP_STRIDE);
}

static int check_march_args(const char* fn, uint32_t C, uint32_t H, uint32_t max_steps) {
    NGP_REQUIRE(C >= 1 && C <= 8, NGP_ERR_INVALID, "%s: cascade count C must be in [1, 8] (got %u)", fn, C);
    NGP_REQUIRE(H >= 2 && H <= 1024, NGP_ERR_INVALID, "%s: grid size H must be in [2, 1024] (got %u)", fn, H);
    NGP_REQUIRE(max_steps >= 1, NGP_ERR_INVALID, "%s: max_steps must be positive", fn);
    return NGP_OK;
}

static int march_rays_train_impl(const float* rays_o, const float* rays_d, const uint8_t* grid_in, float bound, float dt_gamma,
                                 uint32_t max_steps, uint32_t N, uint32_t C, uint32_t H, uint32_t M, const float* aabb, float min_near,
                                 float* nears, float* fars, float* xyzs, float* dirs, float* deltas, int32_t* rays, int32_t* counter,
                                 const float* noises, void* workspace, uint32_t flags, ngp_stream_t stream) {
    int rc = check_march_args("march_rays_train", C, H, max_steps);
    if (rc) return rc;
    if (N == 0) return NGP_OK;
    NGP_REQUIRE(rays_o && rays_d && grid_in && nears && fars && xyzs && dirs && deltas && rays && counter && noises && workspace,
                NGP_ERR_INVALID, "march_rays_train: NULL tensor");
    hipStream_t st = as_stream(stream);
    uint32_t* ws = reinterpret_cast<uint32_t*>(workspace);
    const uint32_t ray_blocks = cdiv(N, MW_WAVES);
    const bool zero_tail = (flags & NGP_MARCH_ZERO_TAIL) && M > 0;
    const bool self_scan = (flags & NGP_MARCH_RESET_COUNTER) && !(flags & NGP_MARCH_SCAN_LAUNCH) && N <= 8192u;
    const uint32_t extra = zero_tail ? 16u : (self_scan ? 1u : 0u);
    const dim3 block(MW_WAVES * 64);
    const bool const_dt = dt_gamma == 0.0f;
#define MARCH_WAVE(WRITE, CDT)                                                                                                              \
    NGP_LAUNCH((k_march_train_wave<WRITE, CDT>), dim3(ray_blocks + ((WRITE) ? extra : 0u)), block, 0, st, rays_o, rays_d, grid_bits,   \
                       bound, dt_gamma, max_steps, N, C, H, M, nears, fars, xyzs, dirs, deltas, rays, noises, ws_windows, ws_masks,              \
                       (flags & NGP_MARCH_NOISE_FROM_SEED) != 0, aabb, min_near, ws, ray_blocks, self_scan ? counter : (int32_t*)nullptr,       \
                       zero_tail)
    const uint8_t* grid_bits = grid_in;
    uint32_t* ws_windows = ws + 2;
    uint64_t* ws_masks = reinterpret_cast<uint64_t*>(ws + 2 + ((N + 1u) & ~1u));
    if (const_dt) MARCH_WAVE(false, true); else MARCH_WAVE(false, false);
    rc = check_launch("march_rays_train(count)");
    if (rc) return rc;
    if (!self_scan) {
        NGP_LAUNCH(k_march_train_scan, dim3(1), dim3(SCAN_THREADS), 0, st, rays, counter, N, M, (int)((flags & NGP_MARCH_RESET_COUNTER) != 0), ws);
        rc = check_launch("march_rays_train(scan)");
        if (rc) return rc;
    }
    if (const_dt) MARCH_WAVE(true, true); else MARCH_WAVE(true, false);
#undef MARCH_WAVE
    return check_launch("march_rays_train(write)");
}

extern "C" int ngp_march_rays_train_ex(const float* rays_o, const float* rays_d, const uint8_t* grid_in, float bound, float dt_gamma,
                                       uint32_t max_steps, uint32_t N, uint32_t C, uint32_t H, uint32_t M, const float* nears,
                                       const float* fars, float* xyzs, float* dirs, float* deltas, int32_t* rays, int32_t* counter,
                                       const float* noises, void* workspace, uint32_t flags, ngp_stream_t stream) {
    return march_rays_train_impl(rays_o, rays_d, grid_in, bound, dt_gamma, max_steps, N, C, H, M, nullptr, 0.0f, const_cast<float*>(nears),
                                 const_cast<float*>(fars), xyzs, dirs, deltas, rays, counter, noises, workspace, flags, stream);
}

extern "C" int ngp_march_rays_train_aabb(const float* rays_o, const float* rays_d, const uint8_t* grid_in, float bound, float dt_gamma,
                                         uint32_t max_steps, uint32_t N, uint32_t C, uint32_t H, uint32_t M, const float* aabb, float min_near,
                                         float* nears, float* fars, float* xyzs, float* dirs, float* deltas, int32_t* rays, int32_t* counter,
                                         const float* noises, void* workspace, uint32_t flags, ngp_stream_t stream) {
    NGP_REQUIRE(aabb || N == 0, NGP_ERR_INVALID, "march_rays_train_aabb: NULL box");
    return march_rays_train_impl(rays_o, rays_d, grid_in, bound, dt_gamma, max_steps, N, C, H, M, aabb, min_near, nears, fars, xyzs, dirs, deltas,
                                 rays, counter, noises, workspace, flags, stream);
}

extern "C" int ngp_march_rays_train(const float* rays_o, const float* rays_d, const uint8_t* grid_in, float bound, float dt_gamma,
                                    uint32_t max_steps, uint32_t N, uint32_t C, uint32_t H, uint32_t M, const float* nears,
                                    const float* fars, float* xyzs, float* dirs, float* deltas, int32_t* rays, int32_t* counter,
                                    const float* noises, void* workspace, ngp_stream_t stream) {
    return ngp_march_rays_train_ex(rays_o, rays_d, grid_in, bound, dt_gamma, max_steps, N, C, H, M, nears, fars, xyzs, dirs, deltas, rays,
                                   counter, noises, workspace, 0u, stream);
}

static int make_finish(const char* fn, int bg_mode, float bg_scalar, const float* bg, const float* nears, const float* fars, float* image_out,
                       float* depth_out, bool forward, Finish* fin) {
    NGP_REQUIRE(bg_mode >= 0 && bg_mode <= 2, NGP_ERR_INVALID, "%s: bg_mode must be 0, 1 or 2", fn);
    NGP_REQUIRE(bg_mode != 2 || bg, NGP_ERR_INVALID, "%s: bg_mode 2 needs a per-ray background tensor", fn);
    NGP_REQUIRE(bg_mode == 0 || !forward || (nears && fars && image_out && depth_out), NGP_ERR_INVALID, "%s: NULL finishing tensor", fn);
    *fin = Finish{bg_mode, bg_scalar, bg, nears, fars, image_out, depth_out};
    return NGP_OK;
// ... 353 lines not shown
```

### torch-ngp_amd/fused.py

```python
import ctypes
import os
from collections import namedtuple

import numpy as np
import torch
from torch.autograd import Function

import _ngp_capi as capi
from optim import announce_overwrite, clean_deposits, resync_stale_shadows

_PLANAR_IN = capi.NGP_FF_INPUT_PLANAR
_PLANAR_DX = capi.NGP_FF_DX_PLANAR

NetCfg = namedtuple('NetCfg', 'bound L S H gridtype align interp nl_sigma nl_color training')
RenderCfg = namedtuple('RenderCfg', 'cascade grid_size min_near capacity perturb dt_gamma max_steps T_thresh density_scale bg_scalar')
Marched = namedtuple('Marched', 'xyzs dirs deltas rays nears fars ws')
Saved = namedtuple('Saved', 'xyzs offsets enc ws16 wc16 fb_s fb_c h16 color_in rgb sigma deltas rays weights_sum image_raw bg march_ws')
Bufs = namedtuple('Bufs', 'emb16 ws16 wc16 g_emb g_ws g_wc')


class GeoLoss(namedtuple('GeoLoss', 'lambda_distortion lambda_depth target_depth depth_weight', defaults=(0.0, 0.0, None, None))):
    __slots__ = ()

    def __new__(cls, lambda_distortion=0.0, lambda_depth=0.0, target_depth=None, depth_weight=None):
        lams = []
        for name, v in (('lambda_distortion', lambda_distortion), ('lambda_depth', lambda_depth)):
            if isinstance(v, bool) or not isinstance(v, (int, float)):
                raise TypeError(f'GeoLoss: {name} must be a host float, got {type(v).__name__}')
            v = float(v)
            if not (0.0 <= v < float('inf')):
                raise ValueError(f'GeoLoss: {name} must be finite and >= 0, got {v}')
            lams.append(v)
        if lams[1] > 0 and target_depth is None:
            raise ValueError('GeoLoss: lambda_depth > 0 needs target_depth')
        for name, t in (('target_depth', target_depth), ('depth_weight', depth_weight)):
            if t is not None and not (torch.is_tensor(t) and t.dtype == torch.float32 and t.dim() == 1 and t.is_contiguous()):
                raise ValueError(f'GeoLoss: {name} must be a contiguous [N] float32 tensor')
        return super().__new__(cls, lams[0], lams[1], target_depth, depth_weight)


def _grid_forward(x, emb16, offsets, enc, M, L, S, H, gridtype, align, interp, bound, costs, st):
    sel = getattr(emb16, '_ngp_sel', None)
    if sel is not None:
        capi.check(capi.lib.ngp_grid_encode_forward_sel(x.data_ptr(), emb16.data_ptr(), sel[0].data_ptr(), sel[1].data_ptr(), None, offsets.data_ptr(),
                                                         enc.data_ptr(), M, 3, 2, L, S, H, gridtype, align, interp, capi.NGP_F16, float(bound), costs, st))
    else:
        capi.check(capi.lib.ngp_grid_encode_forward_sched(x.data_ptr(), emb16.data_ptr(), offsets.data_ptr(), enc.data_ptr(), M, 3, 2, L, S, H,
                                                           None, gridtype, align, interp, capi.NGP_F16, float(bound), costs, st))


class _fused_ngp(Function):
    @staticmethod
    def forward(ctx, x, d, embeddings, w_sigma, w_color, offsets, cfg, bufs, density_scale=1.0):
        M = x.shape[0]
        dev = x.device
        st = capi.stream()
        x = x.contiguous()
        d = d.contiguous()
        half = dict(device=dev, dtype=torch.half)

        enc = torch.empty(cfg.L, M, 2, **half)
        costs = capi.ray_level_costs(cfg.L, cfg.S, cfg.H, 3.0 ** 0.5 / (1024.0 * max(float(cfg.bound), 1e-6))) if USE_BALANCED_FORWARD else None
        _grid_forward(x, bufs.emb16, offsets, enc, M, cfg.L, cfg.S, cfg.H, cfg.gridtype, cfg.align, cfg.interp, cfg.bound, costs, st)
        h16 = torch.empty(M, 16, **half)
        color_in = torch.empty(M, 32, **half)
        out16 = torch.empty(M, 16, **half)
        sigma = torch.empty(M, device=dev, dtype=torch.float32)
        rgb = torch.empty(M, 3, device=dev, dtype=torch.float32)
        d_valid = d.shape[0]
        if cfg.training:
            fb_s = torch.empty(cfg.nl_sigma, M, 64, **half)
            fb_c = torch.empty(cfg.nl_color, M, 64, **half)
        else:
            fb_s = fb_c = None
        assert not cfg.training or density_scale == 1.0, 'the backward of _fused_ngp knows no density scale (the fused training render folds it itself)'
        _network_forward(enc, d, d_valid, bufs.ws16, bufs.wc16, cfg.nl_sigma, cfg.nl_color, float(density_scale), cfg.training, fb_s, h16, sigma,
                         color_in, fb_c, out16, rgb, M, st)
        if cfg.training:
            ctx.save_for_backward(x, offsets, enc, bufs.ws16, bufs.wc16, fb_s, fb_c, h16, color_in, rgb)
            ctx.cfg = cfg
            ctx.n_emb = embeddings.shape[0]
            ctx.bufs = bufs
        return sigma, rgb

    @staticmethod
    def backward(ctx, grad_sigma, grad_rgb):
        x, offsets, enc, ws16, wc16, fb_s, fb_c, h16, color_in, rgb = ctx.saved_tensors
        cfg = ctx.cfg
        nl_sigma, nl_color = cfg.nl_sigma, cfg.nl_color
        M = x.shape[0]
        dev = x.device
        st = capi.stream()
        half = dict(device=dev, dtype=torch.half)
        grad_sigma = torch.zeros(M, device=dev) if grad_sigma is None else grad_sigma.contiguous().float()
        grad_rgb = torch.zeros(M, 3, device=dev) if grad_rgb is None else grad_rgb.contiguous().float()

        g_out16 = torch.empty(M, 16, **half)
        capi.check(capi.lib.ngp_pipeline_rgb_backward(grad_rgb.data_ptr(), rgb.data_ptr(), g_out16.data_ptr(), M, st))
        g_color_in = torch.empty(M, 32, **half)
        g_emb, g_ws, g_wc, deposited = _grad_targets(ctx.bufs, ctx.n_emb, dev)
        scratch_c = torch.empty(nl_color, M, 64, **half)
        capi.check(capi.lib.ngp_ffmlp_backward_ex(g_out16.data_ptr(), color_in.data_ptr(), wc16.data_ptr(), fb_c.data_ptr(), M, 32, 16, 64,
                                                   nl_color, 0, 6, 1, scratch_c.data_ptr(), g_color_in.data_ptr(), g_wc.data_ptr(), 0, st))
        g_h16 = g_out16
        capi.check(capi.lib.ngp_pipeline_mid_backward(grad_sigma.data_ptr(), h16.data_ptr(), g_color_in.data_ptr(), g_h16.data_ptr(), M, 1.0, st))
        g_enc = torch.empty(cfg.L, M, 2, **half)
        scratch_s = scratch_c[:nl_sigma]
        capi.check(capi.lib.ngp_ffmlp_backward_ex(g_h16.data_ptr(), enc.data_ptr(), ws16.data_ptr(), fb_s.data_ptr(), M, 32, 16, 64, nl_sigma,
                                                   0, 6, 1, scratch_s.data_ptr(), g_enc.data_ptr(), g_ws.data_ptr(), _PLANAR_IN | _PLANAR_DX, st))
        _grid_backward(g_enc, x, offsets, g_emb, M, cfg.L, cfg.S, cfg.H, cfg.gridtype, cfg.align, cfg.interp, cfg.bound, st)
        if deposited:
            return None, None, None, None, None, None, None, None, None
        return None, None, g_emb, g_ws, g_wc, None, None, None, None


USE_FUSED_NETWORK = True


def _network_forward(enc, dirs, d_valid, ws16, wc16, nl_sigma, nl_color, density_scale, training, fb_s, h16, sigma, color_in, fb_c, out16, rgb, M, st):
    if USE_FUSED_NETWORK:
        capi.check(capi.lib.ngp_network_forward(enc.data_ptr(), dirs.data_ptr(), M, d_valid, ws16.data_ptr(), wc16.data_ptr(), nl_sigma, nl_color,
                                                 float(density_scale), 1 if training else 0, capi.ptr(fb_s), capi.ptr(h16) if training else None,
                                                 sigma.data_ptr(), capi.ptr(color_in) if training else None, capi.ptr(fb_c), rgb.data_ptr(), _PLANAR_IN, st))
        return
    if training:
        capi.check(capi.lib.ngp_ffmlp_forward_ex(enc.data_ptr(), ws16.data_ptr(), M, 32, 16, 64, nl_sigma, 0, 6, fb_s.data_ptr(), h16.data_ptr(),
                                                  _PLANAR_IN, st))
# ... 343 lines not shown
        image, depth, weights_sum, saved = _render_train_network(marched, bufs, bg_t, offsets, cfg, rcfg)
        loss = torch.empty(1, device=image.device, dtype=torch.float32)
        grad_image = torch.empty_like(image)
        capi.check(capi.lib.ngp_pipeline_mse_loss(image.data_ptr(), target.data_ptr(), image.numel(), capi.ptr(loss_scale), loss.data_ptr(),
                                                   grad_image.data_ptr(), capi.stream()))
        _render_train_backward(saved, cfg, rcfg, grad_image, None, g_emb, g_ws, g_wc, found_inf, overwrite)
        return loss, image, depth, weights_sum
    s = _render_train_network(marched, bufs, bg_t, offsets, cfg, rcfg, composite=False)
    N, M, dev = s.rays.shape[0], s.xyzs.shape[0], s.xyzs.device
    f32 = dict(device=dev, dtype=torch.float32)
    weights_sum, image, depth = torch.empty(N, **f32), torch.empty(N, 3, **f32), torch.empty(N, **f32)
    loss, ray_err = torch.empty(1, **f32), torch.empty(N, **f32)
    g_sigma = torch.empty(M, **f32)
    g_out16 = torch.empty(M, 16, device=dev, dtype=torch.half)
    defer = _carries_reductions(cfg.nl_sigma, cfg.nl_color)
    if geo_loss is not None:
        for name in ('target_depth', 'depth_weight'):
            t = getattr(geo_loss, name)
            if t is not None and (t.shape[0] != N or t.device != dev):
                raise RuntimeError(f'fused: geo_loss.{name} must be [{N}] float32 on {dev}')
        depth_raw, distortion = torch.empty(N, **f32), torch.empty(N, **f32)
        capi.check(capi.lib.ngp_composite_train_geo_loss_backward(s.sigma.data_ptr(), s.rgb.data_ptr(), s.deltas.data_ptr(), s.rays.data_ptr(), M, N,
                                                                   float(rcfg.T_thresh), 2 if s.bg is not None else 1, float(rcfg.bg_scalar),
                                                                   capi.ptr(s.bg), marched.nears.data_ptr(), marched.fars.data_ptr(),
                                                                   target.data_ptr(), geo_loss.lambda_distortion, geo_loss.lambda_depth,
                                                                   capi.ptr(geo_loss.target_depth), capi.ptr(geo_loss.depth_weight),
                                                                   capi.ptr(loss_scale), weights_sum.data_ptr(), image.data_ptr(), depth.data_ptr(),
                                                                   depth_raw.data_ptr(), distortion.data_ptr(),
                                                                   None if defer else loss.data_ptr(), ray_err.data_ptr(), g_sigma.data_ptr(),
                                                                   g_out16.data_ptr(), s.march_ws.data_ptr(),
                                                                   s.march_ws.numel() * s.march_ws.element_size(), capi.stream()))
        _network_backward(s, cfg, rcfg, g_sigma, g_out16, g_emb, g_ws, g_wc, found_inf, loss_job=(ray_err, loss) if defer else None,
                          overwrite=overwrite, table_adam=table_adam)
        return loss, image, depth, weights_sum, depth_raw, distortion
    capi.check(capi.lib.ngp_composite_train_loss_backward(s.sigma.data_ptr(), s.rgb.data_ptr(), s.deltas.data_ptr(), s.rays.data_ptr(), M, N,
                                                           float(rcfg.T_thresh), 2 if s.bg is not None else 1, float(rcfg.bg_scalar), capi.ptr(s.bg),
                                                           marched.nears.data_ptr(), marched.fars.data_ptr(), target.data_ptr(),
                                                           capi.ptr(loss_scale), weights_sum.data_ptr(), image.data_ptr(), depth.data_ptr(),
                                                           None if defer else loss.data_ptr(), ray_err.data_ptr(), g_sigma.data_ptr(),
                                                           g_out16.data_ptr(), s.march_ws.data_ptr(),
                                                           s.march_ws.numel() * s.march_ws.element_size(), capi.stream()))
    _network_backward(s, cfg, rcfg, g_sigma, g_out16, g_emb, g_ws, g_wc, found_inf, loss_job=(ray_err, loss) if defer else None,
                      overwrite=overwrite, table_adam=table_adam)
    return loss, image, depth, weights_sum


@torch.no_grad()
def fused_train_iteration_split(model, rays_o, rays_d, target, box, counter, capacity, loss_scale, bg_color=1, perturb=False, dt_gamma=0,
                                max_steps=1024, T_thresh=1e-4, noise_seed=None, found_inf=None, overwrite_table=False, table_adam=None,
                                geo_loss=None):
    cfg = network_cfg(model.encoder, model.sigma_net, model.color_net, model.bound, True)
    bg_t, rcfg = _render_cfg(model, capacity, bg_color, perturb, dt_gamma, max_steps, T_thresh)
    bufs = _operands((model.encoder.embeddings, model.sigma_net.weights, model.color_net.weights), True, overwrite_table)
    if bufs.g_emb is None:
        raise RuntimeError('fused_train_iteration: the parameters are not managed by optim.NGPAdam(deposit=True)')
    rays_o = rays_o.contiguous().view(-1, 3)
    rays_d = rays_d.contiguous().view(-1, 3)
    target = target.contiguous().view(-1, 3)
    if target.shape[0] != rays_o.shape[0] or target.dtype != torch.float32:
        raise RuntimeError('fused_train_iteration: target must be [N,3] float32')
    if geo_loss is not None and not isinstance(geo_loss, GeoLoss):
        raise TypeError('fused_train_iteration: geo_loss must be a fused.GeoLoss')
    box_ = {}

    def march():
        box_['m'] = _render_train_march(rays_o, rays_d, model.density_bitfield, box, counter, cfg, rcfg, noise_seed, into=box_.get('m'))

    def rest():
        ta = _table_adam_of(table_adam, model)
        with capi.row_bound(_row_bound(box_['m'], cfg)):
            out = _train_iteration_rest(box_['m'], bufs, bg_t, model.encoder.offsets, target, loss_scale, cfg, rcfg, found_inf, overwrite_table, ta,
                                        geo_loss)
        if overwrite_table:
            announce_overwrite(model.encoder.embeddings, None if ta is None else _table_adam_prefix(model, cfg, capacity))
        return out
    return march, rest


density_point_spacing = None


@torch.no_grad()
def fused_density(x, encoder, sigma_net, bound):
    M = x.shape[0]
    dev = x.device
    st = capi.stream()
    emb16, w16 = _half_weights((encoder.embeddings, sigma_net.weights))
    L = int(encoder.num_levels)
    enc = torch.empty(L, M, 2, device=dev, dtype=torch.half)
    S, H = float(np.log2(encoder.per_level_scale)), int(encoder.base_resolution)
    costs = None if density_point_spacing is None else capi.ray_level_costs(L, S, H, float(density_point_spacing))
    _grid_forward(x.contiguous(), emb16, encoder.offsets, enc, M, L, S, H, int(encoder.gridtype_id), int(bool(encoder.align_corners)),
                  int(encoder.interp_id), bound, costs, st)
    h16 = torch.empty(M, 16, device=dev, dtype=torch.half)
    capi.check(capi.lib.ngp_ffmlp_inference_ex(enc.data_ptr(), w16.data_ptr(), M, 32, 16, 64, int(sigma_net.num_layers), 0, 6, None, h16.data_ptr(),
                                                _PLANAR_IN, st))
    return torch.exp(h16[:, 0].float()), h16[:, 1:]


def inference_weights(model, x):
    enc, sn, cn = getattr(model, 'encoder', None), getattr(model, 'sigma_net', None), getattr(model, 'color_net', None)
    if enc is None or sn is None or cn is None or torch.is_grad_enabled():
        return None
    probe = torch.empty(128, 3, device=x.device, dtype=torch.float32)
    if not getattr(model, '_fused_ok', lambda *_: False)(probe, probe):
        return None
    emb16, ws16, wc16 = _half_weights((enc.embeddings, sn.weights, cn.weights), cast=False)
    if emb16 is None or ws16 is None or wc16 is None or getattr(emb16, '_ngp_sel', None) is not None:
        return None
    return emb16, ws16, wc16, network_cfg(enc, sn, cn, model.bound, False)


class pinned_half_weights:

    def __init__(self, model):
        enc, sn, cn = getattr(model, 'encoder', None), getattr(model, 'sigma_net', None), getattr(model, 'color_net', None)
        self.params = [getattr(enc, 'embeddings', None), getattr(sn, 'weights', None), getattr(cn, 'weights', None)]

    def __enter__(self):
        if all(p is not None and p.is_cuda for p in self.params) and not torch.is_grad_enabled():
            for p in self.params:
                fn = getattr(p, '_ngp_materialize', None)
                if fn is not None:
                    fn()
                buf = getattr(p, '_ngp_fp16_pinbuf', None)
                if buf is None or buf.shape != p.shape or buf.device != p.device:
                    buf = torch.empty_like(p, dtype=torch.half)
                    p._ngp_fp16_pinbuf = buf
                buf.copy_(p.detach())
                p._ngp_fp16_pin = buf
        return self

    def __exit__(self, *exc):
        for p in self.params:
            if p is not None and hasattr(p, '_ngp_fp16_pin'):
                del p._ngp_fp16_pin
        return False
```

### torch-ngp_amd/graph.py

```python
import contextlib
import dataclasses
import operator
import os
import typing
from collections import namedtuple

import torch


def _capture_into(g, **kw):
    import torch.distributed as dist
    if dist.is_available() and dist.is_initialized():
        kw.setdefault('capture_error_mode', 'thread_local')
    return torch.cuda.graph(g, **kw)


MARCH_MARKS = {'boundary': None, 'net': ('k_network_forward', 1), 'composite': ('k_composite_train', 1), 'sigma': ('k_grid_backward_bin', 0),
               'sort': ('k_grid_backward_accumulate', 0)}
MARCH_MARK_ID = 1


_LaSet = namedtuple('_LaSet', 'march_graph rest_graph loss image march rest', defaults=(None, None))

_Refresh = namedtuple('_Refresh', 'graph mean sampling samples', defaults=(None, None))
# ... 515 lines not shown
            kernel, behind = MARCH_MARKS[self.march_at]
            for cl in rec.lists:
                at = [i for i, n in enumerate(cl.names()) if kernel in n]
                if not at:
                    raise RuntimeError(f'GraphedTrainStep: NGP_STEP_MARCH_AT={self.march_at}: no {kernel} launch in the recorded chain')
                cl.mark(MARCH_MARK_ID, max(at) + behind)
        rec.used_direct, rec.replay = True, GraphedTrainStep._replay_lookahead

    def _replay_lookahead(self, rays_o, rays_d, target, next_rays):
        m, rec = self.model, self.active
        p = self.la_cur
        q = 1 - p
        cur = rec.la[p]
        self.image = cur.image
        main = torch.cuda.current_stream()
        ready, self.la_ready[p] = self.la_ready[p], None
        if ready is not None:
            main.wait_event(self.la_event[p])
        if ready is not None and ready.holds_rays(rays_o, rays_d, self.occupancy_epoch):
            if not ready.holds_target(target):
                self.la_target[p].copy_(target, non_blocking=True)
            self.la_hits += 1
        else:
            torch._foreach_copy_([self.la_rays_o[p], self.la_rays_d[p], self.la_target[p]],
                                 [rays_o.view_as(self.la_rays_o[p]), rays_d.view_as(self.la_rays_d[p]), target], non_blocking=True)
            self.la_seed[p:p + 1].fill_(self.global_step)
            cur.march_graph.replay()
            self._count_to_ring(p)
            if self.la_slot_event is None:
                self.la_slot_event = torch.cuda.Event()
            self.la_slot_event.record(main)
        ahead = next_rays is not None and (self.global_step + 1) % self.update_interval != 0
        cl = rec.lists[p] if rec.lists else None
        early = ahead and cl is not None and MARCH_MARKS[self.march_at] is not None
        if early:
            self._replay_rest(cur.rest_graph, cl)
        if ahead:
            side = self.la_side
            if early:
                cl.wait_mark(MARCH_MARK_ID, side.cuda_stream)
            else:
                side.wait_stream(main)
            with torch.cuda.stream(side):
                no, nd, *nt = next_rays
                dst, src = [self.la_rays_o[q], self.la_rays_d[q]], [no.view_as(self.la_rays_o[q]), nd.view_as(self.la_rays_d[q])]
                torch._foreach_copy_(dst + [self.la_target[q]] * len(nt), src + nt, non_blocking=True)
                self.la_seed[q:q + 1].fill_(self.global_step + 1)
                rec.la[q].march_graph.replay()
                self._count_to_ring(q, ahead=1)
                self.la_event[q].record(side)
            self.la_ready[q] = _Announced.of(no, nd, *nt, epoch=self.occupancy_epoch)
        elif (self.global_step + 1) % self.update_interval == 0 and self.graph_updates and self.update_capture_error is None:
            full = m.iter_density < 16
            entry = self.update_graphs.get(full)
            if entry is not None and entry.sampling is not None:
                side = self.la_side
                side.wait_stream(main)
                with torch.cuda.stream(side):
                    entry.sampling.replay()
                    self.la_sample_event.record(side)
                self.la_presampled = full
        if rec.la_apply is not None:
            opt = self.optimizer
            opt.wait_shadows()
            cur.rest_graph.replay()
            opt.reduce_gradients()
            rec.la_apply.replay()
            opt.gather_shadows()
        elif not early:
            self._replay_rest(cur.rest_graph, cl)
        self.la_cur = q
        return cur.loss

    def _capture_update(self, full):
        if full in self.update_graphs:
            return True
        if self.update_capture_error is not None or self.graphs is None:
            return False
        try:
            import gc
            gc.collect()
            torch.cuda.synchronize()
            m = self.model
            if getattr(m, 'fused_refresh', True) and getattr(m, 'density_grid', None) is not None and m.density_grid.is_cuda:
                import raymarching
                raymarching.density_grid_state(m.density_grid, m.__dict__.setdefault('_refresh_state', {}))
            if self.la is not None and hasattr(m, 'refresh_sample'):
                gs, ga = torch.cuda.CUDAGraph(), torch.cuda.CUDAGraph()
                if self._sample_pool is None:
                    self._sample_pool = torch.cuda.graph_pool_handle()
                with _capture_into(gs, pool=self._sample_pool):
                    samples = m.refresh_sample(full=full)
                with _capture_into(ga, pool=self.active.rest_pool):
                    with torch.autocast('cuda', dtype=self.autocast_dtype):
                        mean = m.refresh_apply(samples)
                self.update_graphs[full] = _Refresh(ga, mean, gs, samples)
            else:
                g = torch.cuda.CUDAGraph()
                first, *_ = self.graphs
                with _capture_into(g, pool=first.pool()):
                    with torch.autocast('cuda', dtype=self.autocast_dtype):
                        mean = m.refresh_occupancy(full=full)
                self.update_graphs[full] = _Refresh(g, mean)
            self.n_update_captures += 1
            return True
        except Exception as e:
            self.update_capture_error = repr(e)
            torch.cuda.synchronize()
            return False

    def _update_extra_state(self):
        m = self.model
        refresh = getattr(m, 'refresh_occupancy', None)
        if refresh is None or not getattr(m, 'cuda_ray', False):
            with torch.autocast('cuda', dtype=self.autocast_dtype):
                m.update_extra_state()
            return
        full = m.iter_density < 16
        use_graph = self.graph_updates and self.graphs is not None and self.update_capture_error is None
        if use_graph and full not in self.update_graphs:
            use_graph = self._capture_update(full)
        mean_count = None
        if use_graph and self.la is not None and m.local_step > 0:
            used = min(16, m.local_step)
            with torch.cuda.stream(self.la_side):
                if self.la_slot_event is not None:
                    self.la_side.wait_event(self.la_slot_event)
                mean_count = int(m.step_counter[:used, 0].sum().item() / used)
        if use_graph:
            entry = self.update_graphs[full]
            mean = entry.mean
            if entry.sampling is not None:
                if self.la_presampled == full:
                    torch.cuda.current_stream().wait_event(self.la_sample_event)
                    self.la_presample_hits += 1
                else:
                    entry.sampling.replay()
                self.la_presampled = None
            entry.graph.replay()
        else:
            with torch.autocast('cuda', dtype=self.autocast_dtype):
                mean = refresh(full=full)
        m.finish_update(mean, mean_count=mean_count)

    def _eager(self, rays_o, rays_d, target):
        self.optimizer.zero_grad(set_to_none=True)
        geo = self.geo_loss
        with torch.autocast('cuda', dtype=self.autocast_dtype):
            if geo is None:
                out = self.model.render(rays_o, rays_d, **self.render_kwargs)
                loss = self.loss_fn(out, target)
            else:
                out = self.model.render(rays_o, rays_d, **dict(self.render_kwargs, geo=True))
                loss = self.loss_fn(out, target) + geo.lambda_distortion * out['distortion'].float().mean()
        self.image = self._image_of(out)
        self._scaled(loss).backward()
        if self.averager is not None and not getattr(self.optimizer, 'shard', False):
            self.averager.all_reduce()
        self._iteration_back()
        return loss.detach()

    def _ready_for(self, cap):
        if self._fits(cap):
            return True
        pick = self._pick_captured(cap)
        if pick is None:
            return self._try_capture(cap)
        if pick != self.captured_capacity:
            self._activate(pick)
# ... 25 lines not shown
```

### torch-ngp_amd/nerf/network_ff.py

```python
import torch

from activation import trunc_exp
from encoding import get_encoder
from ffmlp import FFMLP
from fused import fused_density, fused_ngp
from gridencoder import GridEncoder
from shencoder import SHEncoder

from .renderer import NeRFRenderer


class NeRFNetwork(NeRFRenderer):
    def __init__(self, encoding="hashgrid", encoding_dir="sphere_harmonics", num_layers=2, hidden_dim=64, geo_feat_dim=15,
                 num_layers_color=3, hidden_dim_color=64, bound=1, **kwargs):
        super().__init__(bound, **kwargs)
        self.num_layers = num_layers
        self.hidden_dim = hidden_dim
        self.geo_feat_dim = geo_feat_dim
        self.encoder, self.in_dim = get_encoder(encoding, desired_resolution=2048 * bound)
        self.sigma_net = FFMLP(input_dim=self.in_dim, output_dim=1 + geo_feat_dim, hidden_dim=hidden_dim, num_layers=num_layers)

        self.num_layers_color = num_layers_color
        self.hidden_dim_color = hidden_dim_color
        self.encoder_dir, dir_dim = get_encoder(encoding_dir)
        self.in_dim_color = dir_dim + geo_feat_dim + 1
        self.color_net = FFMLP(input_dim=self.in_dim_color, output_dim=3, hidden_dim=hidden_dim_color, num_layers=num_layers_color)
        self.fused = True

    def _fused_ok(self, x, d):
        return (self.fused and x.is_cuda and x.dtype == torch.float32 and d.dtype == torch.float32 and x.dim() == 2
                and x.shape[0] > 0 and x.shape[0] % 128 == 0 and d.shape[0] == x.shape[0]
                and torch.is_autocast_enabled('cuda') and torch.get_autocast_dtype('cuda') == torch.float16
                and isinstance(self.encoder, GridEncoder) and self.encoder.input_dim == 3 and self.encoder.level_dim == 2
                and self.encoder.output_dim == 32 and isinstance(self.encoder_dir, SHEncoder) and self.encoder_dir.degree == 4
                and self.hidden_dim == 64 and self.hidden_dim_color == 64 and self.geo_feat_dim == 15
                and 2 <= self.num_layers <= 4 and 2 <= self.num_layers_color <= 4
                and not (x.requires_grad or d.requires_grad))

    def _density_head(self, x):
        h = self.sigma_net(self.encoder(x, bound=self.bound))
        return trunc_exp(h[..., 0]), h[..., 1:]

    def _color_head(self, d, geo_feat):
        code = self.encoder_dir(d)
        pad = torch.zeros_like(geo_feat[..., :1])
        return torch.sigmoid(self.color_net(torch.cat([code, geo_feat, pad], dim=-1)))

    def forward(self, x, d):
        if self._fused_ok(x, d):
            return fused_ngp(x, d, self.encoder, self.sigma_net, self.color_net, self.bound, self.training and torch.is_grad_enabled())
        sigma, geo_feat = self._density_head(x)
        return sigma, self._color_head(d, geo_feat)

    def forward_scaled(self, x, d, density_scale):
        if not torch.is_grad_enabled() and self._fused_ok(x, d):
            return fused_ngp(x, d, self.encoder, self.sigma_net, self.color_net, self.bound, False, density_scale)
        sigma, rgb = self(x, d)
        return density_scale * sigma, rgb

    def density(self, x):
        if not torch.is_grad_enabled() and x.dim() == 2 and self._fused_ok(x, x):
            sigma, geo_feat = fused_density(x, self.encoder, self.sigma_net, self.bound)
            return {'sigma': sigma, 'geo_feat': geo_feat}
        sigma, geo_feat = self._density_head(x)
        return {'sigma': sigma, 'geo_feat': geo_feat}

    def color(self, x, d, mask=None, geo_feat=None, **kwargs):
        if mask is None:
            return self._color_head(d, geo_feat)
        rgbs = torch.zeros(mask.shape[0], 3, dtype=x.dtype, device=x.device)
        if mask.any():
            rgbs[mask] = self._color_head(d[mask], geo_feat[mask]).to(rgbs.dtype)
        return rgbs

    def get_params(self, lr):
        groups = [{'params': m.parameters(), 'lr': lr} for m in (self.encoder, self.sigma_net, self.encoder_dir, self.color_net)]
        if self.bg_radius > 0:
            groups += [{'params': self.encoder_bg.parameters(), 'lr': lr}, {'params': self.bg_net.parameters(), 'lr': lr}]
        return groups
```

### torch-ngp_amd/nerf/renderer.py

```python
import math

import numpy as np
import torch
import torch.nn as nn

import raymarching


def _meshgrid(*axes):
    return torch.meshgrid(*axes, indexing='ij')


def sample_pdf(bins, weights, n_samples, det=False):
    pdf = weights + 1e-5
    pdf = pdf / pdf.sum(-1, keepdim=True)
    cdf = torch.cat([torch.zeros_like(pdf[..., :1]), torch.cumsum(pdf, -1)], -1)
    if det:
        u = torch.linspace(0.5 / n_samples, 1.0 - 0.5 / n_samples, steps=n_samples, device=weights.device)
        u = u.expand(*cdf.shape[:-1], n_samples)
    else:
        u = torch.rand(*cdf.shape[:-1], n_samples, device=weights.device)
    u = u.contiguous()
    hi = torch.searchsorted(cdf, u, right=True)
    lo = (hi - 1).clamp(min=0)
    hi = hi.clamp(max=cdf.shape[-1] - 1)
    cdf_lo, cdf_hi = torch.gather(cdf, -1, lo), torch.gather(cdf, -1, hi)
    bin_lo, bin_hi = torch.gather(bins, -1, lo), torch.gather(bins, -1, hi)
    width = cdf_hi - cdf_lo
    width = torch.where(width < 1e-5, torch.ones_like(width), width)
    return bin_lo + (u - cdf_lo) / width * (bin_hi - bin_lo)


def _alpha_weights(z_vals, sample_dist, sigma, density_scale):
    deltas = torch.cat([z_vals[..., 1:] - z_vals[..., :-1], sample_dist * torch.ones_like(z_vals[..., :1])], -1)
    alphas = 1 - torch.exp(-deltas * density_scale * sigma)
    trans = torch.cumprod(torch.cat([torch.ones_like(alphas[..., :1]), 1 - alphas + 1e-15], -1), -1)[..., :-1]
    return deltas, alphas * trans


class NeRFRenderer(nn.Module):
    def __init__(self, bound=1, cuda_ray=False, density_scale=1, min_near=0.2, density_thresh=0.01, bg_radius=-1):
        super().__init__()
        self.bound = bound
        self.cascade = 1 + math.ceil(math.log2(bound))
        self.grid_size = 128
        self.density_scale = density_scale
        self.min_near = min_near
        self.density_thresh = density_thresh
        self.bg_radius = bg_radius

        box = torch.FloatTensor([-bound, -bound, -bound, bound, bound, bound])
        self.register_buffer('aabb_train', box)
        self.register_buffer('aabb_infer', box.clone())

        self.cuda_ray = cuda_ray
        if cuda_ray:
            cells = self.grid_size ** 3
            self.register_buffer('density_grid', torch.zeros(self.cascade, cells))
            self.register_buffer('density_bitfield', torch.zeros(self.cascade * cells // 8, dtype=torch.uint8))
            self.register_buffer('step_counter', torch.zeros(16, 2, dtype=torch.int32))
            self._mean_density, self._mean_density_dev = 0.0, None
            self.iter_density = 0
            self.mean_count = 0
            self.local_step = 0

    def forward(self, x, d):
        raise NotImplementedError()

    def density(self, x):
        raise NotImplementedError()

    def color(self, x, d, mask=None, **kwargs):
        raise NotImplementedError()

    def reset_extra_state(self):
        if not self.cuda_ray:
            return
        self.density_grid.zero_()
        self.step_counter.zero_()
        self.mean_density = 0
        self.iter_density = 0
        self.mean_count = 0
        self.local_step = 0

    def run(self, rays_o, rays_d, num_steps=128, upsample_steps=128, bg_color=None, perturb=False, **kwargs):
        lead = rays_o.shape[:-1]
        rays_o = rays_o.contiguous().view(-1, 3)
        rays_d = rays_d.contiguous().view(-1, 3)
        n_rays, dev = rays_o.shape[0], rays_o.device
        box = self.aabb_train if self.training else self.aabb_infer
        nears, fars = raymarching.near_far_from_aabb(rays_o, rays_d, box, self.min_near)
        nears, fars = nears.unsqueeze(-1), fars.unsqueeze(-1)
        span = fars - nears
        z_vals = nears + span * torch.linspace(0.0, 1.0, num_steps, device=dev).unsqueeze(0).expand(n_rays, num_steps)
        sample_dist = span / num_steps
        if perturb:
            z_vals = z_vals + (torch.rand(z_vals.shape, device=dev) - 0.5) * sample_dist

        def points(z):
            p = rays_o.unsqueeze(-2) + rays_d.unsqueeze(-2) * z.unsqueeze(-1)
            return torch.min(torch.max(p, box[:3]), box[3:])

        xyzs = points(z_vals)
        dens = {k: v.view(n_rays, num_steps, -1) for k, v in self.density(xyzs.reshape(-1, 3)).items()}
        if upsample_steps > 0:
            with torch.no_grad():
                deltas, weights = _alpha_weights(z_vals, sample_dist, dens['sigma'].squeeze(-1), self.density_scale)
                mids = z_vals[..., :-1] + 0.5 * deltas[..., :-1]
                new_z = sample_pdf(mids, weights[:, 1:-1], upsample_steps, det=not self.training).detach()
                new_xyzs = points(new_z)
            new_dens = {k: v.view(n_rays, upsample_steps, -1) for k, v in self.density(new_xyzs.reshape(-1, 3)).items()}
            z_vals, order = torch.sort(torch.cat([z_vals, new_z], 1), dim=1)
            xyzs = torch.cat([xyzs, new_xyzs], 1)
            xyzs = torch.gather(xyzs, 1, order.unsqueeze(-1).expand_as(xyzs))
            for k in dens:
                both = torch.cat([dens[k], new_dens[k]], 1)
                dens[k] = torch.gather(both, 1, order.unsqueeze(-1).expand_as(both))
        _, weights = _alpha_weights(z_vals, sample_dist, dens['sigma'].squeeze(-1), self.density_scale)
        dirs = rays_d.view(-1, 1, 3).expand_as(xyzs)
        flat = {k: v.reshape(-1, v.shape[-1]) for k, v in dens.items()}
# ... 145 lines not shown

        results['depth'] = depth
        results['image'] = image
        return results

    @staticmethod
    def _aux_infer_feats(fn, frame, xyzs, dirs, sigmas, rgbs, n_rays):
        with torch.no_grad():
            feats = fn(xyzs, dirs, sigmas, rgbs)
        if not torch.is_tensor(feats) or feats.dim() != 2 or feats.shape[0] != xyzs.shape[0] or not 1 <= feats.shape[1] <= 256:
            raise ValueError(f"render(aux_infer=...): the callable must return a [{xyzs.shape[0]}, C] tensor with 1 <= C <= 256 (got "
                             f"{tuple(feats.shape) if torch.is_tensor(feats) else type(feats).__name__})")
        if feats.dtype not in (torch.float32, torch.float16):
            raise ValueError(f"render(aux_infer=...): the callable must return float32 or float16 (got {feats.dtype})")
        if frame['out'] is None:
            frame['out'] = torch.zeros(n_rays, feats.shape[1], dtype=torch.float32, device=xyzs.device)
            frame['dtype'] = feats.dtype
        elif feats.shape[1] != frame['out'].shape[1] or feats.dtype != frame['dtype']:
            raise ValueError(f"render(aux_infer=...): every call of a frame must return the same C and dtype (first call: C = "
                             f"{frame['out'].shape[1]}, {frame['dtype']}; this call: C = {feats.shape[1]}, {feats.dtype})")
        return feats.detach().contiguous()

    def _render_loop_on_device(self, rays_o, rays_d, nears, fars, rays_t, weights_sum, depth, image, perturb, dt_gamma, max_steps, T_thresh,
                               sync_every=8, aux_infer=None, aux_frame=None):
        from .render_loop import FrameLoop
        FrameLoop(self, (rays_o, rays_d, nears, fars, rays_t, weights_sum, depth, image), perturb, dt_gamma, max_steps, T_thresh, sync_every,
                  aux_infer, aux_frame).run()

    def _cascade_points(self, coords, cas):
        unit = 2 * coords.float() / (self.grid_size - 1) - 1
        bound = min(2 ** cas, self.bound)
        half_cell = bound / self.grid_size
        pts = unit * (bound - half_cell)
        pts += (torch.rand_like(pts) * 2 - 1) * half_cell
        return pts

    def _query_sigma(self, pts):
        return self.density(pts)['sigma'].reshape(-1).detach() * self.density_scale

    @torch.no_grad()
    def mark_untrained_grid(self, poses, intrinsic, S=64):
        if not self.cuda_ray:
            return
        if isinstance(poses, np.ndarray):
            poses = torch.from_numpy(poses)
        dev = self.density_bitfield.device
        poses = poses.to(dev)
        fx, fy, cx, cy = intrinsic
        n_views = poses.shape[0]
        axis = torch.arange(self.grid_size, dtype=torch.int32, device=dev).split(S)
        count = torch.zeros_like(self.density_grid)
        for xs in axis:
            for ys in axis:
                for zs in axis:
                    xx, yy, zz = _meshgrid(xs, ys, zs)
                    coords = torch.stack([xx.reshape(-1), yy.reshape(-1), zz.reshape(-1)], -1)
                    cell_ids = raymarching.morton3D(coords).long()
                    unit = (2 * coords.float() / (self.grid_size - 1) - 1).unsqueeze(0)
                    for cas in range(self.cascade):
                        bound = min(2 ** cas, self.bound)
                        half_cell = bound / self.grid_size
                        world = unit * (bound - half_cell)
                        for head in range(0, n_views, S):
                            cam = poses[head:head + S]
                            local = (world - cam[:, :3, 3].unsqueeze(1)) @ cam[:, :3, :3]
                            z = local[:, :, 2]
                            seen = (z > 0) & (local[:, :, 0].abs() < cx / fx * z + half_cell * 2) \
                                & (local[:, :, 1].abs() < cy / fy * z + half_cell * 2)
                            count[cas, cell_ids] += seen.sum(0).reshape(-1)
        self.density_grid[count == 0] = -1

    @property
    def mean_density(self):
        if self._mean_density_dev is not None:
            self._mean_density = float(self._mean_density_dev.item())
            self._mean_density_dev = None
        return self._mean_density

    @mean_density.setter
    def mean_density(self, value):
        self._mean_density, self._mean_density_dev = float(value), None

    @torch.no_grad()
    def refresh_sample(self, S=128, full=None):
        dev = self.density_bitfield.device
        full = (self.iter_density < 16) if full is None else full
        samples = []
        if full:
            axis = torch.arange(self.grid_size, dtype=torch.int32, device=dev).split(S)
            for xs in axis:
                for ys in axis:
                    for zs in axis:
                        xx, yy, zz = _meshgrid(xs, ys, zs)
                        coords = torch.stack([xx.reshape(-1), yy.reshape(-1), zz.reshape(-1)], -1)
                        cell_ids = raymarching.morton3D(coords).long()
                        for cas in range(self.cascade):
                            samples.append((cas, cell_ids, self._cascade_points(coords, cas)))
        else:
            n = self.grid_size ** 3 // 4
            cells = self.grid_size ** 3

            def sorted_uniform(count):
                e = -torch.log(torch.rand(count + 1, device=dev, dtype=torch.float64).clamp_(min=1e-300))
                c = torch.cumsum(e, 0)
                return (c[:count] / c[count]).clamp_(max=1.0 - 2.0 ** -40)
            for cas in range(self.cascade):
                rand_ids = (sorted_uniform(n) * cells).long().clamp_(max=cells - 1)
                rand_coords = raymarching.morton3D_invert(rand_ids)
                occupied = torch.cumsum(self.density_grid[cas] > 0, 0, dtype=torch.int32)
                pick = (sorted_uniform(n) * occupied[-1]).to(torch.int32).clamp_(max=occupied[-1] - 1).clamp_(min=0)
                occ_ids = torch.searchsorted(occupied, pick + 1).clamp_(max=occupied.shape[0] - 1)
                occ_coords = raymarching.morton3D_invert(occ_ids)
                cell_ids = torch.cat([rand_ids, occ_ids], 0)
                coords = torch.cat([rand_coords, occ_coords], 0)
                samples.append((cas, cell_ids, self._cascade_points(coords, cas)))
        return samples

    @torch.no_grad()
    def refresh_apply(self, samples, decay=0.95):
        cells = self.grid_size ** 3
        if getattr(self, 'fused_refresh', True) and self.density_grid.is_cuda and self.density_grid.is_contiguous():
            if len(samples) == 1 and samples[0][0] == 0:
                ids, pts = samples[0][1], samples[0][2]
            else:
                ids = torch.cat([cell_ids + cas * cells for cas, cell_ids, _ in samples], 0)
                pts = torch.cat([p for _, _, p in samples], 0)
            import fused as _fused
            _fused.density_point_spacing = 1.6 / self.grid_size if len(samples) == self.cascade and len(samples[0][1]) < cells else None
            try:
                chunk = int(getattr(self, 'refresh_chunk', 1 << 22))
                if pts.shape[0] <= chunk:
                    sigma = self.density(pts)['sigma'].reshape(-1).detach()
                else:
                    sigma = torch.cat([self.density(pts[i:i + chunk])['sigma'].reshape(-1).detach() for i in range(0, pts.shape[0], chunk)], 0)
            finally:
                _fused.density_point_spacing = None
            state = self.__dict__.setdefault('_refresh_state', {})
            return raymarching.update_density_grid(sigma, ids, self.density_scale, decay, self.density_grid, self.density_thresh,
                                                   self.density_bitfield, state).reshape(())
        fresh = -torch.ones_like(self.density_grid)
        for cas, cell_ids, pts in samples:
            fresh[cas, cell_ids] = self._query_sigma(pts)
        both = (self.density_grid >= 0) & (fresh >= 0)
        self.density_grid.copy_(torch.where(both, torch.maximum(self.density_grid * decay, fresh), self.density_grid))
        mean = torch.mean(self.density_grid.clamp(min=0))
        raymarching.packbits_capped(self.density_grid, self.density_thresh, mean, self.density_bitfield)
        return mean

    @torch.no_grad()
    def refresh_occupancy(self, decay=0.95, S=128, full=None):
        return self.refresh_apply(self.refresh_sample(S, full), decay)

    def finish_update(self, mean, mean_count=None):
        self._mean_density_dev = mean.detach().reshape(())
        self.iter_density += 1
        used = min(16, self.local_step)
        if used > 0:
            self.mean_count = int(self.step_counter[:used, 0].sum().item() / used) if mean_count is None else int(mean_count)
        self.local_step = 0

    @torch.no_grad()
    def update_extra_state(self, decay=0.95, S=128):
        if not self.cuda_ray:
            return
        self.finish_update(self.refresh_occupancy(decay, S))

    def render(self, rays_o, rays_d, staged=False, max_ray_batch=4096, **kwargs):
        if kwargs.get('aux') is not None and (staged or not self.cuda_ray):
            raise NotImplementedError("render(aux=...): the 'aux' channels need the cuda_ray training render; the staged / non-cuda_ray path "
                                      "does not composite them")
        if kwargs.get('aux_infer') is not None and not self.cuda_ray:
            raise NotImplementedError("render(aux_infer=...): the 'aux' channels of an eval frame are composited by the cuda_ray inference loop; "
                                      "the non-cuda_ray path does not composite them")
        if self.cuda_ray:
            return self.run_cuda(rays_o, rays_d, **kwargs)
        if not staged:
            return self.run(rays_o, rays_d, **kwargs)
        B, N = rays_o.shape[:2]
        depth = torch.empty(B, N, device=rays_o.device)
        image = torch.empty(B, N, 3, device=rays_o.device)
        for b in range(B):
            for head in range(0, N, max_ray_batch):
                tail = min(head + max_ray_batch, N)
                part = self.run(rays_o[b:b + 1, head:tail], rays_d[b:b + 1, head:tail], **kwargs)
                depth[b:b + 1, head:tail] = part['depth']
                image[b:b + 1, head:tail] = part['image']
        return {'depth': depth, 'image': image}
```

### torch-ngp_amd/raymarching/backend.py

```python
import types

import torch

import _ngp_capi as capi


def _f32(t, name):
    capi.dense(t, name)
    if t.dtype != torch.float32:
        raise RuntimeError(f"{name} must be a float32 tensor (the reference wrappers cast with custom_fwd(cast_inputs=float32))")
    return t


def _f64(pairs):
    if not capi.float64_call(*pairs):
        return False
    for t, n in pairs:
        capi.dense(t, n)
    return True


def _f32_call(pairs, fn):
    for t, n in pairs:
        _f32(t, n)
    return fn


def _i32(t, name):
    capi.dense(t, name)
    capi.require_int32(t, name)
    return t


def near_far_from_aabb(rays_o, rays_d, aabb, N, min_near, nears, fars):
    floats = ((rays_o, 'rays_o'), (rays_d, 'rays_d'), (aabb, 'aabb'), (nears, 'nears'), (fars, 'fars'))
    fn = capi.lib.ngp_near_far_from_aabb_f64 if _f64(floats) else _f32_call(floats, capi.lib.ngp_near_far_from_aabb)
    capi.check(fn(capi.ptr(rays_o), capi.ptr(rays_d), capi.ptr(aabb), N, float(min_near), capi.ptr(nears), capi.ptr(fars), capi.stream()))


def sph_from_ray(rays_o, rays_d, radius, N, coords):
    floats = ((rays_o, 'rays_o'), (rays_d, 'rays_d'), (coords, 'coords'))
    fn = capi.lib.ngp_sph_from_ray_f64 if _f64(floats) else _f32_call(floats, capi.lib.ngp_sph_from_ray)
    capi.check(fn(capi.ptr(rays_o), capi.ptr(rays_d), float(radius), N, capi.ptr(coords), capi.stream()))


def morton3D(coords, N, indices):
    _i32(coords, 'coords'); _i32(indices, 'indices')
    capi.check(capi.lib.ngp_morton3D(capi.ptr(coords), N, capi.ptr(indices), capi.stream()))


def morton3D_invert(indices, N, coords):
    _i32(coords, 'coords'); _i32(indices, 'indices')
    capi.check(capi.lib.ngp_morton3D_invert(capi.ptr(indices), N, capi.ptr(coords), capi.stream()))


def packbits(grid, N, density_thresh, bitfield):
    floats = ((grid, 'grid'),)
    fn = capi.lib.ngp_packbits_f64 if _f64(floats) else _f32_call(floats, capi.lib.ngp_packbits)
    capi.dense(bitfield, 'bitfield')
    if bitfield.dtype != torch.uint8:
        raise RuntimeError("bitfield must be a uint8 tensor")
    capi.check(fn(capi.ptr(grid), N, float(density_thresh), capi.ptr(bitfield), capi.stream()))


def packbits_capped(grid, N, density_thresh, thresh_cap, bitfield):
    capi.check(capi.lib.ngp_packbits_ex(capi.ptr(grid), N, float(density_thresh), capi.ptr(thresh_cap), capi.ptr(bitfield), capi.stream()))


def density_grid_update(sigmas, cells, n, density_scale, decay, density_grid, n_cells, scratch, density_thresh, mean_out, bitfield, workspace):
    _f32(sigmas, 'sigmas'); _f32(density_grid, 'density_grid'); _f32(scratch, 'scratch'); _f32(mean_out, 'mean_out')
    capi.dense(cells, 'cells')
    if cells.dtype != torch.int64:
        raise RuntimeError("cells must be an int64 tensor")
    capi.check(capi.lib.ngp_density_grid_update(capi.ptr(sigmas), capi.ptr(cells), n, float(density_scale), float(decay), capi.ptr(density_grid),
                                                n_cells, capi.ptr(scratch), float(density_thresh), capi.ptr(mean_out), capi.ptr(bitfield),
                                                capi.ptr(workspace), capi.stream()))


def density_grid_update_workspace_bytes(n_cells):
    return int(capi.lib.ngp_density_grid_update_workspace_bytes(n_cells))


def march_rays_train(rays_o, rays_d, grid, bound, dt_gamma, max_steps, N, C, H, M, nears, fars, xyzs, dirs, deltas, rays,
                     counter, noises):
    for t, n in ((rays_o, 'rays_o'), (rays_d, 'rays_d'), (nears, 'nears'), (fars, 'fars'), (xyzs, 'xyzs'), (dirs, 'dirs'),
                 (deltas, 'deltas'), (noises, 'noises')):
        _f32(t, n)
    _i32(rays, 'rays'); _i32(counter, 'counter')
    capi.dense(grid, 'grid')
    ws = torch.empty(capi.lib.ngp_march_rays_train_workspace_bytes(N), dtype=torch.uint8, device=rays_o.device)
    capi.check(capi.lib.ngp_march_rays_train(
        capi.ptr(rays_o), capi.ptr(rays_d), capi.ptr(grid), float(bound), float(dt_gamma), max_steps, N, C, H, M,
        capi.ptr(nears), capi.ptr(fars), capi.ptr(xyzs), capi.ptr(dirs), capi.ptr(deltas), capi.ptr(rays), capi.ptr(counter),
        capi.ptr(noises), capi.ptr(ws), capi.stream()))


def composite_rays_train_forward(sigmas, rgbs, deltas, rays, M, N, T_thresh, weights_sum, depth, image):
    floats = ((sigmas, 'sigmas'), (rgbs, 'rgbs'), (deltas, 'deltas'), (weights_sum, 'weights_sum'), (depth, 'depth'), (image, 'image'))
    fn = capi.lib.ngp_composite_rays_train_forward_f64 if _f64(floats) else _f32_call(floats, capi.lib.ngp_composite_rays_train_forward)
    _i32(rays, 'rays')
    capi.check(fn(capi.ptr(sigmas), capi.ptr(rgbs), capi.ptr(deltas), capi.ptr(rays), M, N, float(T_thresh), capi.ptr(weights_sum), capi.ptr(depth),
                  capi.ptr(image), capi.stream()))


def composite_rays_train_backward(grad_weights_sum, grad_image, sigmas, rgbs, deltas, rays, weights_sum, image, M, N, T_thresh,
                                  grad_sigmas, grad_rgbs):
    floats = ((grad_weights_sum, 'grad_weights_sum'), (grad_image, 'grad_image'), (sigmas, 'sigmas'), (rgbs, 'rgbs'), (deltas, 'deltas'),
              (weights_sum, 'weights_sum'), (image, 'image'), (grad_sigmas, 'grad_sigmas'), (grad_rgbs, 'grad_rgbs'))
    fn = capi.lib.ngp_composite_rays_train_backward_f64 if _f64(floats) else _f32_call(floats, capi.lib.ngp_composite_rays_train_backward)
    _i32(rays, 'rays')
    capi.check(fn(
        capi.ptr(grad_weights_sum), capi.ptr(grad_image), capi.ptr(sigmas), capi.ptr(rgbs), capi.ptr(deltas), capi.ptr(rays),
        capi.ptr(weights_sum), capi.ptr(image), M, N, float(T_thresh), capi.ptr(grad_sigmas), capi.ptr(grad_rgbs), capi.stream()))


def composite_rays_train_geo_forward(sigmas, rgbs, deltas, rays, M, N, T_thresh, weights_sum, depth, image, distortion):
    floats = ((sigmas, 'sigmas'), (rgbs, 'rgbs'), (deltas, 'deltas'), (weights_sum, 'weights_sum'), (depth, 'depth'), (image, 'image'),
              (distortion, 'distortion'))
    fn = capi.lib.ngp_composite_rays_train_geo_forward_f64 if _f64(floats) else _f32_call(floats, capi.lib.ngp_composite_rays_train_geo_forward)
    _i32(rays, 'rays')
    capi.check(fn(capi.ptr(sigmas), capi.ptr(rgbs), capi.ptr(deltas), capi.ptr(rays), M, N, float(T_thresh), capi.ptr(weights_sum), capi.ptr(depth),
                  capi.ptr(image), capi.ptr(distortion), capi.stream()))


def composite_rays_train_geo_backward(grad_weights_sum, grad_depth, grad_image, grad_distortion, sigmas, rgbs, deltas, rays, weights_sum, depth,
                                      image, distortion, M, N, T_thresh, grad_sigmas, grad_rgbs):
    floats = tuple((t, n) for t, n in (
        (grad_weights_sum, 'grad_weights_sum'), (grad_depth, 'grad_depth'), (grad_image, 'grad_image'), (grad_distortion, 'grad_distortion'),
        (sigmas, 'sigmas'), (rgbs, 'rgbs'), (deltas, 'deltas'), (weights_sum, 'weights_sum'), (depth, 'depth'), (image, 'image'),
        (distortion, 'distortion'), (grad_sigmas, 'grad_sigmas'), (grad_rgbs, 'grad_rgbs')) if t is not None)
    fn = capi.lib.ngp_composite_rays_train_geo_backward_f64 if _f64(floats) else _f32_call(floats, capi.lib.ngp_composite_rays_train_geo_backward)
    _i32(rays, 'rays')
    capi.check(fn(
        capi.ptr(grad_weights_sum), capi.ptr(grad_depth), capi.ptr(grad_image), capi.ptr(grad_distortion), capi.ptr(sigmas), capi.ptr(rgbs),
        capi.ptr(deltas), capi.ptr(rays), capi.ptr(weights_sum), capi.ptr(depth), capi.ptr(image), capi.ptr(distortion), M, N, float(T_thresh),
        capi.ptr(grad_sigmas), capi.ptr(grad_rgbs), capi.stream()))


def composite_rays_train_features_forward(sigmas, feats, deltas, rays, M, N, C, T_thresh, out):
    _i32(rays, 'rays')
    if _f64(((sigmas, 'sigmas'), (feats, 'feats'), (deltas, 'deltas'), (out, 'out'))):
        capi.check(capi.lib.ngp_composite_rays_train_features_forward_f64(capi.ptr(sigmas), capi.ptr(feats), capi.ptr(deltas), capi.ptr(rays), M, N, C,
                                                                          float(T_thresh), capi.ptr(out), capi.stream()))
        return
    for t, n in ((sigmas, 'sigmas'), (deltas, 'deltas'), (out, 'out')):
        _f32(t, n)
    capi.check(capi.lib.ngp_composite_rays_train_features_forward(capi.ptr(sigmas), capi.ptr(capi.dense(feats, 'feats')), capi.ptr(deltas),
                                                                  capi.ptr(rays), M, N, C, float(T_thresh), _feat_code(feats, 'feats'), capi.ptr(out),
                                                                  capi.stream()))


def composite_rays_train_features_backward(grad_out, sigmas, feats, deltas, rays, out, M, N, C, T_thresh, grad_sigmas, grad_feats):
    _i32(rays, 'rays')
    if _f64(((grad_out, 'grad_out'), (sigmas, 'sigmas'), (feats, 'feats'), (deltas, 'deltas'), (out, 'out'), (grad_sigmas, 'grad_sigmas'),
             (grad_feats, 'grad_feats'))):
        capi.check(capi.lib.ngp_composite_rays_train_features_backward_f64(
            capi.ptr(grad_out), capi.ptr(sigmas), capi.ptr(feats), capi.ptr(deltas), capi.ptr(rays), capi.ptr(out), M, N, C, float(T_thresh),
            capi.ptr(grad_sigmas), capi.ptr(grad_feats), capi.stream()))
        return
    for t, n in ((grad_out, 'grad_out'), (sigmas, 'sigmas'), (deltas, 'deltas'), (out, 'out'), (grad_sigmas, 'grad_sigmas')):
        _f32(t, n)
    capi.dense(feats, 'feats'); capi.dense(grad_feats, 'grad_feats')
    if grad_feats.dtype != feats.dtype:
# ... 202 lines not shown
```

### torch-ngp_amd/raymarching/raymarching.py

```python
import torch
from torch.autograd import Function
from torch.amp import custom_bwd, custom_fwd

try:
    import os as _os
    if _os.environ.get('NGP_HIP_LIBRARY'):
        raise ImportError('NGP_HIP_LIBRARY is set')
    import _raymarching as _backend
except ImportError:
    from .backend import _backend
from . import backend as _geo

__all__ = ['near_far_from_aabb', 'sph_from_ray', 'morton3D', 'morton3D_invert', 'packbits', 'packbits_capped', 'march_rays_train',
           'composite_rays_train', 'composite_rays_train_geo', 'composite_rays_train_features', 'sample_ts', 'ray_points', 'march_rays', 'composite_rays', 'composite_rays_features', 'compact_rays', 'update_density_grid', 'density_grid_state',
           'sdf_sigmas']

_f32_fwd = custom_fwd(device_type='cuda', cast_inputs=torch.float32)


def _rays(t):
    t = t if t.is_cuda else t.cuda()
    return t.contiguous().view(-1, 3)


def _round_up_strict(count, align):
    return count + (align - count % align) if align > 0 else count


class _near_far_from_aabb(Function):
    @staticmethod
    @_f32_fwd
    def forward(ctx, rays_o, rays_d, aabb, min_near=0.2):
        rays_o, rays_d = _rays(rays_o), _rays(rays_d)
        n_rays = rays_o.shape[0]
        nears = torch.empty(n_rays, dtype=rays_o.dtype, device=rays_o.device)
        fars = torch.empty_like(nears)
        _backend.near_far_from_aabb(rays_o, rays_d, aabb.contiguous(), n_rays, min_near, nears, fars)
        return nears, fars


near_far_from_aabb = _near_far_from_aabb.apply


class _sph_from_ray(Function):
    @staticmethod
    @_f32_fwd
    def forward(ctx, rays_o, rays_d, radius):
        rays_o, rays_d = _rays(rays_o), _rays(rays_d)
        n_rays = rays_o.shape[0]
        coords = torch.empty(n_rays, 2, dtype=rays_o.dtype, device=rays_o.device)
        _backend.sph_from_ray(rays_o, rays_d, radius, n_rays, coords)
        return coords


sph_from_ray = _sph_from_ray.apply


class _morton3D(Function):
    @staticmethod
    def forward(ctx, coords):
        coords = coords if coords.is_cuda else coords.cuda()
        n = coords.shape[0]
        indices = torch.empty(n, dtype=torch.int32, device=coords.device)
        _backend.morton3D(coords.int().contiguous(), n, indices)
        return indices


morton3D = _morton3D.apply


class _morton3D_invert(Function):
    @staticmethod
    def forward(ctx, indices):
        indices = indices if indices.is_cuda else indices.cuda()
        n = indices.shape[0]
        coords = torch.empty(n, 3, dtype=torch.int32, device=indices.device)
        _backend.morton3D_invert(indices.int().contiguous(), n, coords)
        return coords


morton3D_invert = _morton3D_invert.apply


class _packbits(Function):
    @staticmethod
    @_f32_fwd
    def forward(ctx, grid, thresh, bitfield=None):
        grid = (grid if grid.is_cuda else grid.cuda()).contiguous()
        n_bytes = grid.shape[0] * grid.shape[1] // 8
        if bitfield is None:
            bitfield = torch.empty(n_bytes, dtype=torch.uint8, device=grid.device)
        _backend.packbits(grid, n_bytes, thresh, bitfield)
        return bitfield


packbits = _packbits.apply


def packbits_capped(grid, thresh, thresh_cap, bitfield):
    grid = grid.contiguous()
    n_bytes = grid.shape[0] * grid.shape[1] // 8
    _backend.packbits_capped(grid, n_bytes, float(thresh), thresh_cap.reshape(1).float().contiguous(), bitfield)
    return bitfield


def density_grid_state(density_grid, state):
    n_cells, dev = density_grid.numel(), density_grid.device
    if state.get('n_cells') != n_cells or state.get('device') != dev:
        if density_grid.is_cuda and torch.cuda.is_current_stream_capturing():
            raise RuntimeError('density_grid_state: the refresh scratch must be created outside stream capture (call '
                               'raymarching.density_grid_state(model.density_grid, state) -- or run one refresh eagerly -- before capturing)')
        state.update(n_cells=n_cells, device=dev, scratch=torch.full((n_cells,), -1.0, dtype=torch.float32, device=dev),
                     workspace=torch.zeros(int(_backend.density_grid_update_workspace_bytes(n_cells)), dtype=torch.uint8, device=dev),
                     mean=torch.zeros(1, dtype=torch.float32, device=dev))
    return state


def update_density_grid(sigmas, cells, density_scale, decay, density_grid, density_thresh, bitfield, state):
    n_cells = density_grid.numel()
    density_grid_state(density_grid, state)
    sigmas = sigmas.reshape(-1).float().contiguous()
    cells = cells.reshape(-1).contiguous()
    _backend.density_grid_update(sigmas, cells, sigmas.numel(), float(density_scale), float(decay), density_grid, n_cells, state['scratch'],
                                 float(density_thresh), state['mean'], bitfield, state['workspace'])
    return state['mean']


class _march_rays_train(Function):
    @staticmethod
    @_f32_fwd
    def forward(ctx, rays_o, rays_d, bound, density_bitfield, C, H, nears, fars, step_counter=None, mean_count=-1, perturb=False,
                align=-1, force_all_rays=False, dt_gamma=0, max_steps=1024):
        rays_o, rays_d = _rays(rays_o), _rays(rays_d)
        bitfield = (density_bitfield if density_bitfield.is_cuda else density_bitfield.cuda()).contiguous()
        dev, n_rays = rays_o.device, rays_o.shape[0]

        estimated = (not force_all_rays) and mean_count > 0
        capacity = _round_up_strict(mean_count, align) if estimated else n_rays * max_steps

        xyzs = torch.zeros(capacity, 3, dtype=torch.float32, device=dev)
        dirs = torch.zeros(capacity, 3, dtype=torch.float32, device=dev)
        deltas = torch.zeros(capacity, 2, dtype=torch.float32, device=dev)
        rays = torch.empty(n_rays, 3, dtype=torch.int32, device=dev)
        if step_counter is None:
            step_counter = torch.zeros(2, dtype=torch.int32, device=dev)
        noises = torch.rand(n_rays, dtype=torch.float32, device=dev) if perturb else torch.zeros(n_rays, dtype=torch.float32, device=dev)

        _backend.march_rays_train(rays_o, rays_d, bitfield, bound, dt_gamma, max_steps, n_rays, C, H, capacity, nears, fars, xyzs,
                                  dirs, deltas, rays, step_counter, noises)

        if not estimated:
            used = _round_up_strict(int(step_counter[0].item()), align)
            xyzs, dirs, deltas = xyzs[:used], dirs[:used], deltas[:used]
        return xyzs, dirs, deltas, rays


march_rays_train = _march_rays_train.apply


class _composite_rays_train(Function):
    @staticmethod
    @_f32_fwd
    def forward(ctx, sigmas, rgbs, deltas, rays, T_thresh=1e-4):
        sigmas, rgbs, deltas = sigmas.contiguous(), rgbs.contiguous(), deltas.contiguous()
        n_samples, n_rays = sigmas.shape[0], rays.shape[0]
        weights_sum = torch.empty(n_rays, dtype=sigmas.dtype, device=sigmas.device)
        depth = torch.empty_like(weights_sum)
        image = torch.empty(n_rays, 3, dtype=sigmas.dtype, device=sigmas.device)
        _backend.composite_rays_train_forward(sigmas, rgbs, deltas, rays, n_samples, n_rays, T_thresh, weights_sum, depth, image)
        ctx.save_for_backward(sigmas, rgbs, deltas, rays, weights_sum, image)
        ctx.sizes = (n_samples, n_rays, T_thresh)
        return weights_sum, depth, image

    @staticmethod
    @custom_bwd(device_type='cuda')
    def backward(ctx, grad_weights_sum, grad_depth, grad_image):
        sigmas, rgbs, deltas, rays, weights_sum, image = ctx.saved_tensors
        n_samples, n_rays, T_thresh = ctx.sizes
        grad_sigmas = torch.zeros_like(sigmas)
        grad_rgbs = torch.zeros_like(rgbs)
        _backend.composite_rays_train_backward(grad_weights_sum.contiguous(), grad_image.contiguous(), sigmas, rgbs, deltas, rays,
                                               weights_sum, image, n_samples, n_rays, T_thresh, grad_sigmas, grad_rgbs)
        return grad_sigmas, grad_rgbs, None, None, None


composite_rays_train = _composite_rays_train.apply


class _composite_rays_train_geo(Function):

    @staticmethod
    @_f32_fwd
    def forward(ctx, sigmas, rgbs, deltas, rays, T_thresh=1e-4):
        sigmas, rgbs, deltas = sigmas.contiguous(), rgbs.contiguous(), deltas.contiguous()
        n_samples, n_rays = sigmas.shape[0], rays.shape[0]
        weights_sum = torch.empty(n_rays, dtype=sigmas.dtype, device=sigmas.device)
        depth = torch.empty_like(weights_sum)
        distortion = torch.empty_like(weights_sum)
        image = torch.empty(n_rays, 3, dtype=sigmas.dtype, device=sigmas.device)
        _geo.composite_rays_train_geo_forward(sigmas, rgbs, deltas, rays, n_samples, n_rays, T_thresh, weights_sum, depth, image, distortion)
        ctx.save_for_backward(sigmas, rgbs, deltas, rays, weights_sum, depth, image, distortion)
        ctx.sizes = (n_samples, n_rays, T_thresh)
        ctx.set_materialize_grads(False)
        return weights_sum, depth, image, distortion

    @staticmethod
    @custom_bwd(device_type='cuda')
    def backward(ctx, grad_weights_sum, grad_depth, grad_image, grad_distortion):
# ... 209 lines not shown
```

Measured before the change: 673.8 million.

## Deduplicate density-refresh samples on device and bound MLP inference by live row count

Adds a device-side selection pass that drops duplicate cell ids within and across paired runs of refresh samples and compacts them, producing a live-row count held on the device. The MLP inference kernel and the density scatter kernel read this count so they only process live tiles and rows, with no host sync. This is meant to cut redundant density evaluations in the occupancy-grid refresh. It adds an extra selection kernel with a last-block scan, and the row-bounded path only works with the register-resident forward kernel.

```diff
diff --git a/include/ngp_hip.h b/include/ngp_hip.h
--- a/include/ngp_hip.h
+++ b/include/ngp_hip.h
@@ -197,6 +197,14 @@
 int ngp_density_grid_update(const float* sigmas, const int64_t* cells, uint32_t n, float density_scale, float decay, float* density_grid,
                             uint32_t n_cells, float* scratch, float density_thresh, float* mean_out, uint8_t* bitfield, void* workspace,
                             ngp_stream_t stream);
+int ngp_density_grid_update_rows(const float* sigmas, const void* h16, uint32_t h16_stride, const int64_t* cells, uint32_t n,
+                                 const uint32_t* rows_dev, float density_scale, float decay, float* density_grid, uint32_t n_cells,
+                                 float* scratch, float density_thresh, float* mean_out, uint8_t* bitfield, void* workspace,
+                                 ngp_stream_t stream);
+
+size_t ngp_refresh_select_workspace_bytes(uint32_t T);
+int ngp_refresh_select(const int64_t* ids, const float* pts, uint32_t run_len, uint32_t n_runs, int64_t* ids_out, float* pts_out,
+                       uint32_t* live_out, void* workspace, size_t workspace_bytes, ngp_stream_t stream);
 
 #define NGP_FF_INPUT_PLANAR 1u
 #define NGP_FF_DX_PLANAR 2u
@@ -212,6 +220,10 @@
                            uint32_t output_dim, uint32_t hidden_dim, uint32_t num_layers, uint32_t activation,
                            uint32_t output_activation, void* inference_buffer, void* outputs, uint32_t flags,
                            ngp_stream_t stream);
+int ngp_ffmlp_inference_rows(const void* inputs, const void* weights, uint32_t B, uint32_t input_dim,
+                             uint32_t output_dim, uint32_t hidden_dim, uint32_t num_layers, uint32_t activation,
+                             uint32_t output_activation, void* inference_buffer, void* outputs, uint32_t flags,
+                             const uint32_t* rows_dev, ngp_stream_t stream);
 int ngp_ffmlp_backward_ex(const void* grad, const void* inputs, const void* weights, const void* forward_buffer,
                           uint32_t B, uint32_t input_dim, uint32_t output_dim, uint32_t hidden_dim, uint32_t num_layers,
                           uint32_t activation, uint32_t output_activation, int calc_grad_inputs, void* backward_buffer,
diff --git a/torch-ngp_amd/_ngp_capi.py b/torch-ngp_amd/_ngp_capi.py
--- a/torch-ngp_amd/_ngp_capi.py
+++ b/torch-ngp_amd/_ngp_capi.py
@@ -82,6 +82,9 @@
     'ngp_grid_encode_backward_checked_slabs': [_vp, _vp, _vp, _vp, _vp, _u32, _u32, _u32, _u32, _f32, _u32, _vp, _vp, _u32, _i32, _u32, _i32, _f32,
                                                _vp, _vp, _sz, _vp, _vp, _vp],
     'ngp_density_grid_update': [_vp, _vp, _u32, _f32, _f32, _vp, _u32, _vp, _f32, _vp, _vp, _vp, _vp],
+    'ngp_density_grid_update_rows': [_vp, _vp, _u32, _vp, _u32, _vp, _f32, _f32, _vp, _u32, _vp, _f32, _vp, _vp, _vp, _vp],
+    'ngp_refresh_select': [_vp, _vp, _u32, _u32, _vp, _vp, _vp, _vp, _sz, _vp],
+    'ngp_ffmlp_inference_rows': [_vp, _vp, _u32, _u32, _u32, _u32, _u32, _u32, _u32, _vp, _vp, _u32, _vp, _vp],
     'ngp_ffmlp_forward_ex': [_vp, _vp, _u32, _u32, _u32, _u32, _u32, _u32, _u32, _vp, _vp, _u32, _vp],
     'ngp_ffmlp_inference_ex': [_vp, _vp, _u32, _u32, _u32, _u32, _u32, _u32, _u32, _vp, _vp, _u32, _vp],
     'ngp_ffmlp_backward_ex': [_vp, _vp, _vp, _vp, _u32, _u32, _u32, _u32, _u32, _u32, _u32, _i32, _vp, _vp, _vp, _u32, _vp],
@@ -189,6 +192,8 @@
 lib.ngp_density_grid_update_workspace_bytes.restype = _sz
 lib.ngp_sdf_sigmas_workspace_bytes.argtypes = [_u32]
 lib.ngp_sdf_sigmas_workspace_bytes.restype = _sz
+lib.ngp_refresh_select_workspace_bytes.argtypes = [_u32]
+lib.ngp_refresh_select_workspace_bytes.restype = _sz
 
 if lib.ngp_abi_version() != ABI_VERSION:
     raise ImportError(f"{LIB_PATH}: ABI version {lib.ngp_abi_version()} != expected {ABI_VERSION}; rebuild the extension")
@@ -199,7 +204,7 @@
                                        'ngp_ffmlp_backward_slab_count', 'ngp_density_grid_update_workspace_bytes', 'ngp_grid_forward_work_lists', 'ngp_coarse_occupancy_bytes',
                                        'ngp_grid_table_adam_prefix', 'ngp_linear_stack_flat_size',
                                        'ngp_grid_backward_backward_workspace_bytes', 'ngp_ffmlp_backward_backward_workspace_bytes',
-                                       'ngp_grid_ordered_workspace_bytes', 'ngp_sdf_sigmas_workspace_bytes'])
+                                       'ngp_grid_ordered_workspace_bytes', 'ngp_sdf_sigmas_workspace_bytes', 'ngp_refresh_select_workspace_bytes'])
 
 
 def check(rc):
diff --git a/torch-ngp_amd/csrc/ffmlp.hip b/torch-ngp_amd/csrc/ffmlp.hip
--- a/torch-ngp_amd/csrc/ffmlp.hip
+++ b/torch-ngp_amd/csrc/ffmlp.hip
@@ -229,12 +229,14 @@
 template <int WIDTH, bool TRAIN, bool PLAIN >
 __device__ __forceinline__ void ffmlp_forward_body(const half_t* __restrict__ inputs, const half_t* __restrict__ weights,
                                                    half_t* __restrict__ forward_buffer, half_t* __restrict__ outputs, uint32_t n_tiles,
-                                                   uint32_t in_dim, uint32_t num_layers, uint32_t act, uint32_t out_act, bool in_planar) {
+                                                   uint32_t in_dim, uint32_t num_layers, uint32_t act, uint32_t out_act, bool in_planar,
+                                                   const uint32_t* __restrict__ rows_dev) {
     constexpr int NIB = Shape<WIDTH>::NIB, NKB = Shape<WIDTH>::NKB;
     extern __shared__ __attribute__((aligned(16))) unsigned char smem[];
     half8_t* img = reinterpret_cast<half8_t*>(smem);
     build_forward_image<WIDTH>(img, weights, in_dim, num_layers);
     const size_t rows = (size_t)n_tiles * FF_TILE;
+    const uint32_t n_work = rows_dev ? min(n_tiles, (rows_dev[0] + (uint32_t)FF_TILE - 1u) / (uint32_t)FF_TILE) : n_tiles;
     __syncthreads();
 
     const int lane = threadIdx.x & 63, wid = threadIdx.x >> 6;
@@ -245,7 +247,7 @@
     const half8_t* img_out = img_hid + (size_t)(num_layers - 1) * NIB * NKB * 64;
     const size_t layer_stride = (size_t)n_tiles * NKB * 64;
 
-    for (uint32_t tile = blockIdx.x * FF_WAVES + wid; tile < n_tiles; tile += gridDim.x * FF_WAVES) {
+    for (uint32_t tile = blockIdx.x * FF_WAVES + wid; tile < n_work; tile += gridDim.x * FF_WAVES) {
         const size_t srow = (size_t)tile * FF_TILE + n;
         float16_t acc[NIB];
 #pragma unroll
@@ -300,14 +302,14 @@
 template <int WIDTH, bool TRAIN, bool PLAIN>
 __global__ __launch_bounds__(FF_THREADS) __attribute__((amdgpu_waves_per_eu(4, 4))) void k_ffmlp_forward(
     const half_t* __restrict__ inputs, const half_t* __restrict__ weights, half_t* __restrict__ forward_buffer, half_t* __restrict__ outputs,
-    uint32_t n_tiles, uint32_t in_dim, uint32_t num_layers, uint32_t act, uint32_t out_act, bool in_planar) {
-    ffmlp_forward_body<WIDTH, TRAIN, PLAIN>(inputs, weights, forward_buffer, outputs, n_tiles, in_dim, num_layers, act, out_act, in_planar);
+    uint32_t n_tiles, uint32_t in_dim, uint32_t num_layers, uint32_t act, uint32_t out_act, bool in_planar, const uint32_t* __restrict__ rows_dev) {
+    ffmlp_forward_body<WIDTH, TRAIN, PLAIN>(inputs, weights, forward_buffer, outputs, n_tiles, in_dim, num_layers, act, out_act, in_planar, rows_dev);
 }
 template <int WIDTH, bool TRAIN, bool PLAIN>
 __global__ __launch_bounds__(FF_THREADS) __attribute__((amdgpu_waves_per_eu(2, 2))) void k_ffmlp_forward_wide(
     const half_t* __restrict__ inputs, const half_t* __restrict__ weights, half_t* __restrict__ forward_buffer, half_t* __restrict__ outputs,
-    uint32_t n_tiles, uint32_t in_dim, uint32_t num_layers, uint32_t act, uint32_t out_act, bool in_planar) {
-    ffmlp_forward_body<WIDTH, TRAIN, PLAIN>(inputs, weights, forward_buffer, outputs, n_tiles, in_dim, num_layers, act, out_act, in_planar);
+    uint32_t n_tiles, uint32_t in_dim, uint32_t num_layers, uint32_t act, uint32_t out_act, bool in_planar, const uint32_t* __restrict__ rows_dev) {
+    ffmlp_forward_body<WIDTH, TRAIN, PLAIN>(inputs, weights, forward_buffer, outputs, n_tiles, in_dim, num_layers, act, out_act, in_planar, rows_dev);
 }
 
 
@@ -1688,16 +1690,21 @@
 
 template <int WIDTH, bool TRAIN>
 static int launch_forward(const void* inputs, const void* weights, uint32_t B, uint32_t in_dim, uint32_t num_layers, uint32_t act,
-                          uint32_t out_act, void* fwd, void* outputs, uint32_t flags, hipStream_t st) {
+                          uint32_t out_act, void* fwd, void* outputs, uint32_t flags, hipStream_t st,
+                          const uint32_t* rows_dev = nullptr ) {
     const uint32_t n_tiles = B / FF_TILE;
     const size_t lds = forward_image_bytes<WIDTH>(in_dim, num_layers);
-    if (WIDTH > 128 || lds > 152 * 1024 || (flags & NGP_FF_LAYERED))
+    const bool layered = WIDTH > 128 || lds > 152 * 1024 || (flags & NGP_FF_LAYERED);
+    NGP_REQUIRE(!(rows_dev && layered), NGP_ERR_INVALID, "ffmlp_inference_rows: the row count needs the register-resident kernel (widths up to "
+                "128 whose weight image fits the LDS, no NGP_FF_LAYERED)");
+    if (layered)
         return launch_forward_layered<WIDTH, TRAIN>(inputs, weights, B, in_dim, num_layers, act, out_act, fwd, outputs, flags, st);
     if constexpr (WIDTH > 128) {
         return NGP_ERR_INVALID;
     } else {
     const bool plain = act == ACT_RELU && out_act == ACT_NONE;
-    using forward_kernel_t = void (*)(const half_t*, const half_t*, half_t*, half_t*, uint32_t, uint32_t, uint32_t, uint32_t, uint32_t, bool);
+    using forward_kernel_t = void (*)(const half_t*, const half_t*, half_t*, half_t*, uint32_t, uint32_t, uint32_t, uint32_t, uint32_t, bool,
+                                      const uint32_t*);
     forward_kernel_t kern;
     if constexpr (WIDTH > 64) kern = plain ? k_ffmlp_forward_wide<WIDTH, TRAIN, true> : k_ffmlp_forward_wide<WIDTH, TRAIN, false>;
     else kern = plain ? k_ffmlp_forward<WIDTH, TRAIN, true> : k_ffmlp_forward<WIDTH, TRAIN, false>;
@@ -1708,7 +1715,7 @@
     const uint32_t need = cdiv(n_tiles, FF_WAVES);
     if (blocks > need) blocks = need;
     const hipError_t e = NGP_LAUNCH_STATUS(kern, dim3(blocks), dim3(FF_THREADS), lds, st, (const half_t*)inputs, (const half_t*)weights, (half_t*)fwd,
-                                           (half_t*)outputs, n_tiles, in_dim, num_layers, act, out_act, (flags & NGP_FF_INPUT_PLANAR) != 0);
+                                           (half_t*)outputs, n_tiles, in_dim, num_layers, act, out_act, (flags & NGP_FF_INPUT_PLANAR) != 0, rows_dev);
     NGP_REQUIRE(e == hipSuccess, NGP_ERR_LAUNCH, "ffmlp: kernel launch failed: %s", hipGetErrorString(e));
     return check_launch(TRAIN ? "ffmlp_forward" : "ffmlp_inference");
     }
@@ -1918,12 +1925,19 @@
 extern "C" int ngp_ffmlp_inference_ex(const void* inputs, const void* weights, uint32_t B, uint32_t input_dim, uint32_t output_dim,
                                       uint32_t hidden_dim, uint32_t num_layers, uint32_t activation, uint32_t output_activation,
                                       void* inference_buffer, void* outputs, uint32_t flags, ngp_stream_t stream) {
+    return ngp_ffmlp_inference_rows(inputs, weights, B, input_dim, output_dim, hidden_dim, num_layers, activation, output_activation,
+                                    inference_buffer, outputs, flags, nullptr, stream);
+}
+
+extern "C" int ngp_ffmlp_inference_rows(const void* inputs, const void* weights, uint32_t B, uint32_t input_dim, uint32_t output_dim,
+                                        uint32_t hidden_dim, uint32_t num_layers, uint32_t activation, uint32_t output_activation,
+                                        void* inference_buffer, void* outputs, uint32_t flags, const uint32_t* rows_dev, ngp_stream_t stream) {
     int rc = check_ff_args("ffmlp_inference", B, input_dim, output_dim, hidden_dim, num_layers);
     if (rc) return rc;
     if (B == 0) return NGP_OK;
     NGP_REQUIRE(inputs && weights && outputs, NGP_ERR_INVALID, "ffmlp_inference: NULL tensor");
     hipStream_t st = as_stream(stream);
-#define FF_INF(W) launch_forward<W, false>(inputs, weights, B, input_dim, num_layers, activation, output_activation, inference_buffer, outputs, flags, st)
+#define FF_INF(W) launch_forward<W, false>(inputs, weights, B, input_dim, num_layers, activation, output_activation, inference_buffer, outputs, flags, st, rows_dev)
     FF_WIDTHS(FF_INF)
 #undef FF_INF
 }
diff --git a/torch-ngp_amd/csrc/raymarching.hip b/torch-ngp_amd/csrc/raymarching.hip
--- a/torch-ngp_amd/csrc/raymarching.hip
+++ b/torch-ngp_amd/csrc/raymarching.hip
@@ -114,6 +114,151 @@
     if (i >= n) return;
     const uint64_t c = (uint64_t)cells[i];
     if (c < n_cells) scratch[c] = sigmas[i] * scale;
+}
+
+template <bool H16>
+__global__ __launch_bounds__(RM_THREADS) void k_density_scatter_rows(const float* __restrict__ sigmas, const _Float16* __restrict__ h16,
+                                                                       uint32_t stride, const int64_t* __restrict__ cells, uint32_t n,
+                                                                       const uint32_t* __restrict__ rows, float scale,
+                                                                       float* __restrict__ scratch, uint32_t n_cells) {
+    const uint32_t i = blockIdx.x * RM_THREADS + threadIdx.x;
+    const uint32_t live = rows ? min(n, rows[0]) : n;
+    if (i >= live) return;
+    const uint64_t c = (uint64_t)cells[i];
+    if (c >= n_cells) return;
+    if (H16) scratch[c] = expf((float)h16[(size_t)i * stride]) * scale;
+    else scratch[c] = sigmas[i] * scale;
+}
+
+constexpr int RS_THREADS = 256, RS_ITEMS = 4;
+struct RefreshSelectWs {
+    uint32_t* ticket; uint32_t* last_src; uint32_t* block_count; uint32_t* block_last; uint32_t* flags;
+    __host__ __device__ RefreshSelectWs(void* ws, uint32_t blocks)
+        : ticket((uint32_t*)ws), last_src((uint32_t*)ws + 1), block_count((uint32_t*)ws + 2), block_last((uint32_t*)ws + 2 + blocks),
+          flags((uint32_t*)ws + 2 + 2 * (size_t)blocks) {}
+};
+
+__device__ __forceinline__ uint32_t rs_block_exclusive(uint32_t v, uint32_t* wave_sums , uint32_t& total) {
+    const int lane = threadIdx.x & 63, w = threadIdx.x >> 6;
+    uint32_t inc = v;
+#pragma unroll
+    for (int o = 1; o < 64; o <<= 1) {
+        const uint32_t t = __shfl_up(inc, o, 64);
+        if (lane >= o) inc += t;
+    }
+    __syncthreads();
+    if (lane == 63) wave_sums[w] = inc;
+    __syncthreads();
+    uint32_t before = 0, all = 0;
+#pragma unroll
+    for (int k = 0; k < RS_THREADS / 64; k++) {
+        const uint32_t s = wave_sums[k];
+        if (k < w) before += s;
+        all += s;
+    }
+    total = all;
+    return before + inc - v;
+}
+
+__global__ __launch_bounds__(RS_THREADS) void k_refresh_flag(const int64_t* __restrict__ ids, uint32_t T, uint32_t run_len, void* ws,
+                                                               uint32_t* __restrict__ live_out) {
+    const RefreshSelectWs w(ws, gridDim.x);
+    const uint32_t i0 = (blockIdx.x * RS_THREADS + threadIdx.x) * RS_ITEMS;
+    uint32_t flags = 0, count = 0, last = 0;
+#pragma unroll
+    for (int k = 0; k < RS_ITEMS; k++) {
+        const uint32_t i = i0 + k;
+        if (i >= T) break;
+        const int64_t id = ids[i];
+        const uint32_t run = i / run_len, pos = i - run * run_len;
+        bool keep = pos == 0 || ids[i - 1] != id;
+        if (keep && (run & 1u)) {
+            const int64_t* u = ids + (size_t)(run - 1u) * run_len;
+            uint32_t lo = 0, hi = run_len;
+            while (lo < hi) {
+                const uint32_t mid = lo + ((hi - lo) >> 1);
+                if (u[mid] < id) lo = mid + 1; else hi = mid;
+            }
+            keep = !(lo < run_len && u[lo] == id);
+        }
+        if (keep) { flags |= 1u << k; count++; last = i + 1u; }
+    }
+    if (i0 < T) w.flags[blockIdx.x * RS_THREADS + threadIdx.x] = flags;
+
+    __shared__ uint32_t part_count[RS_THREADS / 64], part_last[RS_THREADS / 64];
+    __shared__ uint32_t wave_sums[RS_THREADS / 64 + 1];
+    __shared__ bool is_last;
+#pragma unroll
+    for (int o = 32; o > 0; o >>= 1) {
+        count += __shfl_xor(count, o, 64);
+        last = max(last, (uint32_t)__shfl_xor(last, o, 64));
+    }
+    if ((threadIdx.x & 63) == 0) { part_count[threadIdx.x >> 6] = count; part_last[threadIdx.x >> 6] = last; }
+    __syncthreads();
+    if (threadIdx.x == 0) {
+        uint32_t c = 0, l = 0;
+#pragma unroll
+        for (int k = 0; k < RS_THREADS / 64; k++) { c += part_count[k]; l = max(l, part_last[k]); }
+        __hip_atomic_store(&w.block_count[blockIdx.x], c, __ATOMIC_RELAXED, __HIP_MEMORY_SCOPE_AGENT);
+        __hip_atomic_store(&w.block_last[blockIdx.x], l, __ATOMIC_RELAXED, __HIP_MEMORY_SCOPE_AGENT);
+        asm volatile("s_waitcnt vmcnt(0)" ::: "memory");
+        is_last = __hip_atomic_fetch_add(w.ticket, 1u, __ATOMIC_RELAXED, __HIP_MEMORY_SCOPE_AGENT) == gridDim.x - 1u;
+    }
+    __syncthreads();
+    if (!is_last) return;
+    const uint32_t per = (gridDim.x + RS_THREADS - 1u) / RS_THREADS;
+    const uint32_t b0 = min(threadIdx.x * per, gridDim.x), b1 = min(b0 + per, gridDim.x);
+    uint32_t sum = 0, hi_last = 0;
+    for (uint32_t b = b0; b < b1; b++) {
+        sum += __hip_atomic_load(&w.block_count[b], __ATOMIC_RELAXED, __HIP_MEMORY_SCOPE_AGENT);
+        hi_last = max(hi_last, __hip_atomic_load(&w.block_last[b], __ATOMIC_RELAXED, __HIP_MEMORY_SCOPE_AGENT));
+    }
+    uint32_t total;
+    uint32_t run = rs_block_exclusive(sum, wave_sums, total);
+    for (uint32_t b = b0; b < b1; b++) {
+        const uint32_t c = __hip_atomic_load(&w.block_count[b], __ATOMIC_RELAXED, __HIP_MEMORY_SCOPE_AGENT);
+        w.block_count[b] = run;
+        run += c;
+    }
+#pragma unroll
+    for (int o = 32; o > 0; o >>= 1) hi_last = max(hi_last, (uint32_t)__shfl_xor(hi_last, o, 64));
+    __syncthreads();
+    if ((threadIdx.x & 63) == 0) part_last[threadIdx.x >> 6] = hi_last;
+    __syncthreads();
+    if (threadIdx.x == 0) {
+        uint32_t l = 0;
+#pragma unroll
+        for (int k = 0; k < RS_THREADS / 64; k++) l = max(l, part_last[k]);
+        live_out[0] = total;
+        w.last_src[0] = l - 1u;
+        __hip_atomic_store(w.ticket, 0u, __ATOMIC_RELAXED, __HIP_MEMORY_SCOPE_AGENT);
+    }
+}
+
+__global__ __launch_bounds__(RS_THREADS) void k_refresh_compact(const int64_t* __restrict__ ids, const float* __restrict__ pts, uint32_t T,
+                                                                  const void* ws, const uint32_t* __restrict__ live_in,
+                                                                  int64_t* __restrict__ ids_out, float* __restrict__ pts_out) {
+    const RefreshSelectWs w(const_cast<void*>(ws), gridDim.x);
+    __shared__ uint32_t wave_sums[RS_THREADS / 64 + 1];
+    const uint32_t slot = blockIdx.x * RS_THREADS + threadIdx.x, i0 = slot * RS_ITEMS;
+    const uint32_t flags = i0 < T ? w.flags[slot] : 0u;
+    uint32_t total;
+    uint32_t at = w.block_count[blockIdx.x] + rs_block_exclusive((uint32_t)__builtin_popcount(flags), wave_sums, total);
+    const uint32_t live = live_in[0], src = w.last_src[0];
+#pragma unroll
+    for (int k = 0; k < RS_ITEMS; k++) {
+        const uint32_t i = i0 + k;
+        if (i >= T) break;
+        if (flags & (1u << k)) {
+            ids_out[at] = ids[i];
+            pts_out[(size_t)at * 3] = pts[(size_t)i * 3]; pts_out[(size_t)at * 3 + 1] = pts[(size_t)i * 3 + 1]; pts_out[(size_t)at * 3 + 2] = pts[(size_t)i * 3 + 2];
+            at++;
+        }
+        if (i >= live) {
+            ids_out[i] = ids[src];
+            pts_out[(size_t)i * 3] = pts[(size_t)src * 3]; pts_out[(size_t)i * 3 + 1] = pts[(size_t)src * 3 + 1]; pts_out[(size_t)i * 3 + 2] = pts[(size_t)src * 3 + 2];
+        }
+    }
 }
 
 constexpr int DM_THREADS = 256, DM_PER_THREAD = 32;
@@ -1597,17 +1742,25 @@
     return sizeof(double) * (size_t)cdiv(n_cells, DM_THREADS * DM_PER_THREAD) + 64;
 }
 
-extern "C" int ngp_density_grid_update(const float* sigmas, const int64_t* cells, uint32_t n, float density_scale, float decay, float* density_grid,
-                                       uint32_t n_cells, float* scratch, float density_thresh, float* mean_out, uint8_t* bitfield, void* workspace,
-                                       ngp_stream_t stream) {
+static int density_grid_update_impl(const float* sigmas, const _Float16* h16, uint32_t h16_stride, const int64_t* cells, uint32_t n,
+                                    const uint32_t* rows_dev, float density_scale, float decay, float* density_grid, uint32_t n_cells,
+                                    float* scratch, float density_thresh, float* mean_out, uint8_t* bitfield, void* workspace,
+                                    ngp_stream_t stream) {
     NGP_REQUIRE(density_grid && scratch && mean_out && bitfield && workspace, NGP_ERR_INVALID, "density_grid_update: NULL tensor");
     NGP_REQUIRE(n_cells >= 8 && n_cells % 8 == 0, NGP_ERR_INVALID, "density_grid_update: the grid must hold a multiple of 8 cells (got %u)", n_cells);
     NGP_REQUIRE(((reinterpret_cast<uintptr_t>(density_grid) | reinterpret_cast<uintptr_t>(scratch)) & 15) == 0, NGP_ERR_INVALID,
                 "density_grid_update: grid and scratch must be 16-byte aligned");
     hipStream_t st = as_stream(stream);
     if (n) {
-        NGP_REQUIRE(sigmas && cells, NGP_ERR_INVALID, "density_grid_update: NULL tensor");
-        RM_LAUNCH_1D(k_density_scatter, n, st, sigmas, cells, n, density_scale, scratch, n_cells);
+        NGP_REQUIRE((sigmas || h16) && cells, NGP_ERR_INVALID, "density_grid_update: NULL tensor");
+        if (h16) {
+            NGP_REQUIRE(!sigmas && h16_stride >= 1, NGP_ERR_INVALID, "density_grid_update_rows: give sigmas or h16 (with its row stride), not both");
+            RM_LAUNCH_1D(k_density_scatter_rows<true>, n, st, sigmas, h16, h16_stride, cells, n, rows_dev, density_scale, scratch, n_cells);
+        } else if (rows_dev) {
+            RM_LAUNCH_1D(k_density_scatter_rows<false>, n, st, sigmas, h16, h16_stride, cells, n, rows_dev, density_scale, scratch, n_cells);
+        } else {
+            RM_LAUNCH_1D(k_density_scatter, n, st, sigmas, cells, n, density_scale, scratch, n_cells);
+        }
     }
     const uint32_t blocks = cdiv(n_cells, DM_THREADS * DM_PER_THREAD);
     double* partials = reinterpret_cast<double*>(workspace);
@@ -1615,6 +1768,47 @@
     NGP_LAUNCH(k_density_apply_mean, dim3(blocks), dim3(DM_THREADS), 0, st, density_grid, scratch, n_cells, decay, partials, ticket, mean_out);
     RM_LAUNCH_1D(k_packbits, n_cells / 8, st, (const float*)density_grid, n_cells / 8, density_thresh, (const float*)mean_out, bitfield);
     return check_launch("density_grid_update");
+}
+
+extern "C" int ngp_density_grid_update(const float* sigmas, const int64_t* cells, uint32_t n, float density_scale, float decay, float* density_grid,
+                                       uint32_t n_cells, float* scratch, float density_thresh, float* mean_out, uint8_t* bitfield, void* workspace,
+                                       ngp_stream_t stream) {
+    return density_grid_update_impl(sigmas, nullptr, 0, cells, n, nullptr, density_scale, decay, density_grid, n_cells, scratch, density_thresh,
+                                    mean_out, bitfield, workspace, stream);
+}
+
+extern "C" int ngp_density_grid_update_rows(const float* sigmas, const void* h16, uint32_t h16_stride, const int64_t* cells, uint32_t n,
+                                            const uint32_t* rows_dev, float density_scale, float decay, float* density_grid, uint32_t n_cells,
+                                            float* scratch, float density_thresh, float* mean_out, uint8_t* bitfield, void* workspace,
+                                            ngp_stream_t stream) {
+    return density_grid_update_impl(sigmas, reinterpret_cast<const _Float16*>(h16), h16_stride, cells, n, rows_dev, density_scale, decay,
+                                    density_grid, n_cells, scratch, density_thresh, mean_out, bitfield, workspace, stream);
+}
+
+extern "C" size_t ngp_refresh_select_workspace_bytes(uint32_t T) {
+    const size_t blocks = cdiv(T, RS_THREADS * RS_ITEMS);
+    return sizeof(uint32_t) * (2 + 2 * blocks + blocks * RS_THREADS) + 64;
+}
+
+extern "C" int ngp_refresh_select(const int64_t* ids, const float* pts, uint32_t run_len, uint32_t n_runs, int64_t* ids_out, float* pts_out,
+                                  uint32_t* live_out, void* workspace, size_t workspace_bytes, ngp_stream_t stream) {
+    NGP_REQUIRE(live_out && workspace, NGP_ERR_INVALID, "refresh_select: NULL tensor");
+    NGP_REQUIRE((uint64_t)run_len * n_runs <= 0xfffff000ull, NGP_ERR_INVALID, "refresh_select: %u runs of %u elements exceed 32-bit indexing", n_runs, run_len);
+    const uint32_t T = run_len * n_runs;
+    NGP_REQUIRE(workspace_bytes >= ngp_refresh_select_workspace_bytes(T), NGP_ERR_INVALID,
+                "refresh_select: workspace of %zu bytes, ngp_refresh_select_workspace_bytes(%u) asks for %zu", workspace_bytes, T,
+                ngp_refresh_select_workspace_bytes(T));
+    hipStream_t st = as_stream(stream);
+    if (T == 0) {
+        NGP_REQUIRE(memset_async(live_out, 0, sizeof(uint32_t), st) == hipSuccess, NGP_ERR_LAUNCH, "refresh_select: memset failed");
+        return NGP_OK;
+    }
+    NGP_REQUIRE(ids && pts && ids_out && pts_out, NGP_ERR_INVALID, "refresh_select: NULL tensor");
+    NGP_REQUIRE(ids != ids_out && pts != pts_out, NGP_ERR_INVALID, "refresh_select: the outputs must not be the inputs");
+    const uint32_t blocks = cdiv(T, RS_THREADS * RS_ITEMS);
+    NGP_LAUNCH(k_refresh_flag, dim3(blocks), dim3(RS_THREADS), 0, st, ids, T, run_len, workspace, live_out);
+    NGP_LAUNCH(k_refresh_compact, dim3(blocks), dim3(RS_THREADS), 0, st, ids, pts, T, (const void*)workspace, (const uint32_t*)live_out, ids_out, pts_out);
+    return check_launch("refresh_select");
 }
 
 extern "C" size_t ngp_march_rays_train_workspace_bytes(uint32_t N) {
diff --git a/torch-ngp_amd/fused.py b/torch-ngp_amd/fused.py
--- a/torch-ngp_amd/fused.py
+++ b/torch-ngp_amd/fused.py
@@ -39,10 +39,11 @@
         return super().__new__(cls, lams[0], lams[1], target_depth, depth_weight)
 
 
-def _grid_forward(x, emb16, offsets, enc, M, L, S, H, gridtype, align, interp, bound, costs, st):
+def _grid_forward(x, emb16, offsets, enc, M, L, S, H, gridtype, align, interp, bound, costs, st, rows=None):
     sel = getattr(emb16, '_ngp_sel', None)
-    if sel is not None:
-        capi.check(capi.lib.ngp_grid_encode_forward_sel(x.data_ptr(), emb16.data_ptr(), sel[0].data_ptr(), sel[1].data_ptr(), None, offsets.data_ptr(),
+    if sel is not None or rows is not None:
+        alt, parity = (None, None) if sel is None else (sel[0].data_ptr(), sel[1].data_ptr())
+        capi.check(capi.lib.ngp_grid_encode_forward_sel(x.data_ptr(), emb16.data_ptr(), alt, parity, capi.ptr(rows), offsets.data_ptr(),
                                                          enc.data_ptr(), M, 3, 2, L, S, H, gridtype, align, interp, capi.NGP_F16, float(bound), costs, st))
     else:
         capi.check(capi.lib.ngp_grid_encode_forward_sched(x.data_ptr(), emb16.data_ptr(), offsets.data_ptr(), enc.data_ptr(), M, 3, 2, L, S, H,
@@ -552,6 +553,12 @@
 
 @torch.no_grad()
 def fused_density(x, encoder, sigma_net, bound):
+    h16 = fused_density_h16(x, encoder, sigma_net, bound)
+    return torch.exp(h16[:, 0].float()), h16[:, 1:]
+
+
+@torch.no_grad()
+def fused_density_h16(x, encoder, sigma_net, bound, rows=None):
     M = x.shape[0]
     dev = x.device
     st = capi.stream()
@@ -561,11 +568,11 @@
     S, H = float(np.log2(encoder.per_level_scale)), int(encoder.base_resolution)
     costs = None if density_point_spacing is None else capi.ray_level_costs(L, S, H, float(density_point_spacing))
     _grid_forward(x.contiguous(), emb16, encoder.offsets, enc, M, L, S, H, int(encoder.gridtype_id), int(bool(encoder.align_corners)),
-                  int(encoder.interp_id), bound, costs, st)
+                  int(encoder.interp_id), bound, costs, st, rows)
     h16 = torch.empty(M, 16, device=dev, dtype=torch.half)
-    capi.check(capi.lib.ngp_ffmlp_inference_ex(enc.data_ptr(), w16.data_ptr(), M, 32, 16, 64, int(sigma_net.num_layers), 0, 6, None, h16.data_ptr(),
-                                                _PLANAR_IN, st))
-    return torch.exp(h16[:, 0].float()), h16[:, 1:]
+    capi.check(capi.lib.ngp_ffmlp_inference_rows(enc.data_ptr(), w16.data_ptr(), M, 32, 16, 64, int(sigma_net.num_layers), 0, 6, None, h16.data_ptr(),
+                                                  _PLANAR_IN, capi.ptr(rows), st))
+    return h16
 
 
 def inference_weights(model, x):
diff --git a/torch-ngp_amd/graph.py b/torch-ngp_amd/graph.py
--- a/torch-ngp_amd/graph.py
+++ b/torch-ngp_amd/graph.py
@@ -621,9 +621,13 @@
             gc.collect()
             torch.cuda.synchronize()
             m = self.model
-            if getattr(m, 'fused_refresh', True) and getattr(m, 'density_grid', None) is not None and m.density_grid.is_cuda:
+            if getattr(m, 'density_grid', None) is not None and m.density_grid.is_cuda:
                 import raymarching
-                raymarching.density_grid_state(m.density_grid, m.__dict__.setdefault('_refresh_state', {}))
+                state = m.__dict__.setdefault('_refresh_state', {})
+                if getattr(m, 'fused_refresh', True):
+                    raymarching.density_grid_state(m.density_grid, state)
+                if not full and getattr(m, 'refresh_select', True) and hasattr(m, '_select_samples'):
+                    raymarching.refresh_select_state(m.cascade * 2 * (m.grid_size ** 3 // 4), m.density_grid.device, state)
             if self.la is not None and hasattr(m, 'refresh_sample'):
                 gs, ga = torch.cuda.CUDAGraph(), torch.cuda.CUDAGraph()
                 if self._sample_pool is None:
diff --git a/torch-ngp_amd/nerf/network_ff.py b/torch-ngp_amd/nerf/network_ff.py
--- a/torch-ngp_amd/nerf/network_ff.py
+++ b/torch-ngp_amd/nerf/network_ff.py
@@ -3,7 +3,7 @@
 from activation import trunc_exp
 from encoding import get_encoder
 from ffmlp import FFMLP
-from fused import fused_density, fused_ngp
+from fused import fused_density, fused_density_h16, fused_ngp
 from gridencoder import GridEncoder
 from shencoder import SHEncoder
 
@@ -65,6 +65,11 @@
         sigma, geo_feat = self._density_head(x)
         return {'sigma': sigma, 'geo_feat': geo_feat}
 
+    def density_h16(self, x, rows=None):
+        if not torch.is_grad_enabled() and x.dim() == 2 and self._fused_ok(x, x):
+            return fused_density_h16(x, self.encoder, self.sigma_net, self.bound, rows)
+        return None
+
     def color(self, x, d, mask=None, geo_feat=None, **kwargs):
         if mask is None:
             return self._color_head(d, geo_feat)
diff --git a/torch-ngp_amd/nerf/renderer.py b/torch-ngp_amd/nerf/renderer.py
--- a/torch-ngp_amd/nerf/renderer.py
+++ b/torch-ngp_amd/nerf/renderer.py
@@ -36,6 +36,30 @@
     alphas = 1 - torch.exp(-deltas * density_scale * sigma)
     trans = torch.cumprod(torch.cat([torch.ones_like(alphas[..., :1]), 1 - alphas + 1e-15], -1), -1)[..., :-1]
     return deltas, alphas * trans
+
+
+class RefreshSamples(list):
+
+    def __init__(self, build):
+        super().__init__()
+        self._build = build
+
+    def _fill(self):
+        if self._build is not None:
+            build, self._build = self._build, None
+            super().extend(build())
+
+    def __iter__(self):
+        self._fill()
+        return super().__iter__()
+
+    def __len__(self):
+        self._fill()
+        return super().__len__()
+
+    def __getitem__(self, i):
+        self._fill()
+        return super().__getitem__(i)
 
 
 class NeRFRenderer(nn.Module):
@@ -347,6 +371,31 @@
         self._mean_density, self._mean_density_dev = float(value), None
 
     @torch.no_grad()
+    def _select_samples(self, samples):
+        cells = self.grid_size ** 3
+        n = samples[0][1].shape[0] // 2
+        if len(samples) == 1 and samples[0][0] == 0:
+            ids, pts = samples[0][1], samples[0][2]
+        else:
+            ids = torch.cat([cell_ids + cas * cells for cas, cell_ids, _ in samples], 0)
+            pts = torch.cat([p for _, _, p in samples], 0)
+        state = self.__dict__.setdefault('_refresh_state', {})
+        sel_ids, sel_pts, live = raymarching.refresh_select(ids, pts, n, state)
+        cascades = [cas for cas, _, _ in samples]
+
+        def triples():
+            if len(cascades) == 1:
+                return [(cascades[0], sel_ids - cascades[0] * cells, sel_pts)]
+            out = []
+            for k, cas in enumerate(cascades):
+                own = torch.div(sel_ids, cells, rounding_mode='floor') == cas
+                out.append((cas, torch.where(own, sel_ids, ids[2 * n * k]) - cas * cells, torch.where(own[:, None], sel_pts, pts[2 * n * k])))
+            return out
+        out = RefreshSamples(triples)
+        out.live, out.ids, out.pts = live, sel_ids, sel_pts
+        return out
+
+    @torch.no_grad()
     def refresh_sample(self, S=128, full=None):
         dev = self.density_bitfield.device
         full = (self.iter_density < 16) if full is None else full
@@ -379,19 +428,27 @@
                 cell_ids = torch.cat([rand_ids, occ_ids], 0)
                 coords = torch.cat([rand_coords, occ_coords], 0)
                 samples.append((cas, cell_ids, self._cascade_points(coords, cas)))
+            if getattr(self, 'refresh_select', True) and self.density_grid.is_cuda:
+                samples = self._select_samples(samples)
         return samples
 
     @torch.no_grad()
     def refresh_apply(self, samples, decay=0.95):
         cells = self.grid_size ** 3
         if getattr(self, 'fused_refresh', True) and self.density_grid.is_cuda and self.density_grid.is_contiguous():
-            if len(samples) == 1 and samples[0][0] == 0:
+            ordered = getattr(samples, 'live', None) is not None
+            if ordered:
+                mean = self._refresh_apply_live(samples, decay)
+                if mean is not None:
+                    return mean
+                ids, pts = samples.ids, samples.pts
+            elif len(samples) == 1 and samples[0][0] == 0:
                 ids, pts = samples[0][1], samples[0][2]
             else:
                 ids = torch.cat([cell_ids + cas * cells for cas, cell_ids, _ in samples], 0)
                 pts = torch.cat([p for _, _, p in samples], 0)
             import fused as _fused
-            _fused.density_point_spacing = 1.6 / self.grid_size if len(samples) == self.cascade and len(samples[0][1]) < cells else None
+            _fused.density_point_spacing = 1.6 / self.grid_size if ordered or (len(samples) == self.cascade and len(samples[0][1]) < cells) else None
             try:
                 chunk = int(getattr(self, 'refresh_chunk', 1 << 22))
                 if pts.shape[0] <= chunk:
@@ -411,6 +468,24 @@
         mean = torch.mean(self.density_grid.clamp(min=0))
         raymarching.packbits_capped(self.density_grid, self.density_thresh, mean, self.density_bitfield)
         return mean
+
+    def _refresh_apply_live(self, samples, decay):
+        density_h16 = getattr(self, 'density_h16', None)
+        if density_h16 is None or samples.pts.shape[0] > int(getattr(self, 'refresh_chunk', 1 << 22)):
+            return None
+        import fused as _fused
+        _fused.density_point_spacing = 1.6 / self.grid_size
+        try:
+            h16 = density_h16(samples.pts, samples.live)
+        finally:
+            _fused.density_point_spacing = None
+        if h16 is None:
+            return None
+        state = self.__dict__.setdefault('_refresh_state', {})
+        if not getattr(self, 'refresh_fold', True):
+            h16 = torch.exp(h16[:, 0].float())
+        return raymarching.update_density_grid_rows(h16, samples.ids, samples.live, self.density_scale, decay, self.density_grid,
+                                                    self.density_thresh, self.density_bitfield, state).reshape(())
 
     @torch.no_grad()
     def refresh_occupancy(self, decay=0.95, S=128, full=None):
diff --git a/torch-ngp_amd/raymarching/backend.py b/torch-ngp_amd/raymarching/backend.py
--- a/torch-ngp_amd/raymarching/backend.py
+++ b/torch-ngp_amd/raymarching/backend.py
@@ -79,6 +79,44 @@
 
 def density_grid_update_workspace_bytes(n_cells):
     return int(capi.lib.ngp_density_grid_update_workspace_bytes(n_cells))
+
+
+def density_grid_update_rows(values, cells, n, rows_dev, density_scale, decay, density_grid, n_cells, scratch, density_thresh, mean_out, bitfield,
+                             workspace):
+    _f32(density_grid, 'density_grid'); _f32(scratch, 'scratch'); _f32(mean_out, 'mean_out')
+    capi.dense(cells, 'cells')
+    if cells.dtype != torch.int64:
+        raise RuntimeError("cells must be an int64 tensor")
+    if rows_dev is not None and (rows_dev.dtype not in (torch.int32, torch.uint32) or not rows_dev.is_cuda):
+        raise RuntimeError("rows_dev must be a 32-bit integer tensor on the device")
+    if values.dtype == torch.float16:
+        if values.dim() != 2 or values.stride(1) != 1 or not values.is_cuda:
+            raise RuntimeError("h16 must be a [n, k] float16 device tensor with unit column stride")
+        sig, h16, stride = None, capi.ptr(values), int(values.stride(0))
+    else:
+        sig, h16, stride = capi.ptr(_f32(values, 'sigmas')), None, 0
+    capi.check(capi.lib.ngp_density_grid_update_rows(sig, h16, stride, capi.ptr(cells), n, capi.ptr(rows_dev), float(density_scale), float(decay),
+                                                     capi.ptr(density_grid), n_cells, capi.ptr(scratch), float(density_thresh),
+                                                     capi.ptr(mean_out), capi.ptr(bitfield), capi.ptr(workspace), capi.stream()))
+
+
+def refresh_select_workspace_bytes(T):
+    return int(capi.lib.ngp_refresh_select_workspace_bytes(T))
+
+
+def refresh_select(ids, pts, run_len, n_runs, ids_out, pts_out, live_out, workspace):
+    for t, n in ((ids, 'ids'), (ids_out, 'ids_out')):
+        capi.dense(t, n)
+        if t.dtype != torch.int64:
+            raise RuntimeError(f"{n} must be an int64 tensor")
+    _f32(pts, 'pts'); _f32(pts_out, 'pts_out')
+    T = run_len * n_runs
+    if ids.numel() != T or ids_out.numel() != T or pts.numel() != 3 * T or pts_out.numel() != 3 * T:
+        raise RuntimeError(f"refresh_select: ids / pts must hold {n_runs} runs of {run_len} elements")
+    if live_out.dtype not in (torch.int32, torch.uint32) or not live_out.is_cuda:
+        raise RuntimeError("live_out must be a 32-bit integer tensor on the device")
+    capi.check(capi.lib.ngp_refresh_select(capi.ptr(ids), capi.ptr(pts), run_len, n_runs, capi.ptr(ids_out), capi.ptr(pts_out), capi.ptr(live_out),
+                                           capi.ptr(workspace), workspace.numel() * workspace.element_size(), capi.stream()))
 
 
 def march_rays_train(rays_o, rays_d, grid, bound, dt_gamma, max_steps, N, C, H, M, nears, fars, xyzs, dirs, deltas, rays,
diff --git a/torch-ngp_amd/raymarching/raymarching.py b/torch-ngp_amd/raymarching/raymarching.py
--- a/torch-ngp_amd/raymarching/raymarching.py
+++ b/torch-ngp_amd/raymarching/raymarching.py
@@ -13,7 +13,7 @@
 
 __all__ = ['near_far_from_aabb', 'sph_from_ray', 'morton3D', 'morton3D_invert', 'packbits', 'packbits_capped', 'march_rays_train',
            'composite_rays_train', 'composite_rays_train_geo', 'composite_rays_train_features', 'sample_ts', 'ray_points', 'march_rays', 'composite_rays', 'composite_rays_features', 'compact_rays', 'update_density_grid', 'density_grid_state',
-           'sdf_sigmas']
+           'update_density_grid_rows', 'refresh_select', 'refresh_select_state', 'sdf_sigmas']
 
 _f32_fwd = custom_fwd(device_type='cuda', cast_inputs=torch.float32)
 
@@ -124,6 +124,36 @@
     _backend.density_grid_update(sigmas, cells, sigmas.numel(), float(density_scale), float(decay), density_grid, n_cells, state['scratch'],
                                  float(density_thresh), state['mean'], bitfield, state['workspace'])
     return state['mean']
+
+
+def update_density_grid_rows(values, cells, rows, density_scale, decay, density_grid, density_thresh, bitfield, state):
+    n_cells = density_grid.numel()
+    density_grid_state(density_grid, state)
+    if values.dtype != torch.float16:
+        values = values.reshape(-1).float().contiguous()
+    cells = cells.reshape(-1).contiguous()
+    _geo.density_grid_update_rows(values, cells, cells.numel(), rows, float(density_scale), float(decay), density_grid, n_cells, state['scratch'],
+                                  float(density_thresh), state['mean'], bitfield, state['workspace'])
+    return state['mean']
+
+
+def refresh_select_state(T, device, state):
+    if state.get('select_T') != T or state.get('select_device') != device:
+        if device.type == 'cuda' and torch.cuda.is_current_stream_capturing():
+            raise RuntimeError('refresh_select_state: the selection buffers must be created outside stream capture (call '
+                               'raymarching.refresh_select_state(T, device, state) -- or run one refresh eagerly -- before capturing)')
+        state.update(select_T=T, select_device=device, select_ids=torch.zeros(T, dtype=torch.int64, device=device),
+                     select_pts=torch.zeros(T, 3, dtype=torch.float32, device=device), select_live=torch.zeros(1, dtype=torch.int32, device=device),
+                     select_ws=torch.zeros(_geo.refresh_select_workspace_bytes(T), dtype=torch.uint8, device=device))
+    return state
+
+
+def refresh_select(ids, pts, run_len, state):
+    T = ids.numel()
+    refresh_select_state(T, ids.device, state)
+    _geo.refresh_select(ids.contiguous(), pts.float().contiguous(), run_len, T // run_len, state['select_ids'], state['select_pts'],
+                        state['select_live'], state['select_ws'])
+    return state['select_ids'], state['select_pts'], state['select_live']
 
 
 class _march_rays_train(Function):
```

Result: no change. 669.4 million (-0.7%).
